# acerbilab/pyvbmc

Measured on AMD Instinct MI355X. Metric: ELBO+entropy evals/sec at D=10, K=50, N=400, Ns=1e6 (1e6-sample-equivalent evals/s), higher is better.
Workload: dtype f64; 1 GPU; BASELINE config 3 per GPU: D=10 K=50 N=400 S=1, Ns=1000000 MC samples per GPU (job Ns=1000000), value+grad _neg_elcbo with soft bounds, eps=philox; parallelism=single GPU

## Files before the change

include/vbmc_hip.h:

```cpp
#ifndef VBMC_HIP_H
#define VBMC_HIP_H

#include <stddef.h>
#include <stdint.h>

#ifdef __cplusplus
extern "C" {
#endif

typedef struct vbmc_ctx vbmc_ctx;

enum {
  VBMC_OK = 0,
  VBMC_E_ARG = -1,
  VBMC_E_HIP = -2,
  VBMC_E_RCCL = -3,
  VBMC_E_NODEV = -4,
  VBMC_E_UNSUP = -5,
  VBMC_E_NONFINITE = -6,
  VBMC_E_NOMEM = -7,
  VBMC_E_NOTPD = -8,
  VBMC_W_GP_CHANGED = 1,
  VBMC_W_NOT_FUSED = 2
};

enum { VBMC_MEAN_ZERO = 0, VBMC_MEAN_CONST = 1, VBMC_MEAN_NEGQUAD = 2 };

enum {
  VBMC_EPS_RESIDENT = 0,
  VBMC_EPS_PHILOX = 1
};


int vbmc_abi_version(void);

int vbmc_device_count(int* n_out);

int vbmc_ctx_create(int device_id, vbmc_ctx** out);
void vbmc_ctx_destroy(vbmc_ctx* ctx);

int vbmc_host_affinity(const vbmc_ctx* ctx, int* bound_out, int* n_cpus_out);

const char* vbmc_last_error(const vbmc_ctx* ctx);

int vbmc_device_info(const vbmc_ctx* ctx, char* name, int name_len, int* cu_count,
                     int* clock_khz, uint64_t* hbm_bytes);

int vbmc_synchronize(vbmc_ctx* ctx);

int vbmc_set_timing(vbmc_ctx* ctx, int on);

int vbmc_last_kernel_ms(vbmc_ctx* ctx, int which, double* ms_out);

int vbmc_last_host_us(const vbmc_ctx* ctx, double out[5]);
int vbmc_last_step_marks(const vbmc_ctx* ctx, double out[4]);
int vbmc_set_release_callback(vbmc_ctx* ctx, void (*fn)(void*), void* user);

int vbmc_set_option(vbmc_ctx* ctx, const char* key, int value);

int vbmc_last_entmc_plan(const vbmc_ctx* ctx, int out[4]);

int vbmc_ws_span_layout(int cus, int pb, int front, int nb, int pad, int K, int64_t* part_lo, int* first_part,
                        int* rows_per_component);

int vbmc_host_checksum(const double* const* ptrs, const int64_t* lens, int n, uint64_t* out);

int vbmc_set_gp_watch(vbmc_ctx* ctx, const double* const* ptrs, const int64_t* lens, int n, uint64_t expected);

int vbmc_armed_stats(const vbmc_ctx* ctx, uint64_t out[6]);

int vbmc_last_elbo_raw(const vbmc_ctx* ctx, double* out, int n);


int vbmc_set_mixture(vbmc_ctx* ctx, int D, int K, const double* mu_KxD,
                     const double* sigma_K, const double* lambd_D, const double* w_K,
                     const double* eta_K);

int vbmc_set_mixture_dk(vbmc_ctx* ctx, int D, int K, const double* mu_DxK,
                        const double* sigma_K, const double* lambd_D, const double* w_K,
                        const double* eta_K);

int vbmc_theta_to_mixture(vbmc_ctx* ctx, const double* theta, int n_theta,
                          int optimize_mask, double* mu_KxD, double* sigma_K,
                          double* lambd_D, double* w_K, double* eta_K);


int vbmc_mixture_pdf(vbmc_ctx* ctx, int64_t n, const double* x_nxD, int log_flag,
                     int grad_flag, double df, double* y_n, double* dy_nxD);


int vbmc_set_eps(vbmc_ctx* ctx, int K, int64_t n_half, int D, const double* eps_half,
                 int64_t row_begin, int64_t row_count);

int vbmc_mt19937_randn(uint32_t* key, int* pos, int* has_gauss, double* gauss, double* out,
                       int64_t n, int n_threads);

int vbmc_mt19937_randn_dev(vbmc_ctx* ctx, uint32_t* key, int* pos, int* has_gauss, double* gauss, double* out,
                           int64_t n);
int vbmc_randn_dev_info(const vbmc_ctx* ctx, int* window_reused);
int vbmc_mt_jump_host(const uint32_t* key_in, uint64_t n_words, uint32_t* key_out);
int vbmc_mt_jump_polys(uint64_t stride_words, int count, uint32_t* out);

int vbmc_set_eps_numpy(vbmc_ctx* ctx, uint32_t* key, int* pos, int* has_gauss, double* gauss, int K,
                       int64_t n_half, int D, int64_t row_begin, int64_t row_count, int n_threads);

int vbmc_entmc(vbmc_ctx* ctx, int64_t ns_per_comp, int eps_mode, uint64_t seed,
               int64_t row_begin, int64_t row_count, int grad_flags, int jacobian_flag,
               double* H, double* dH, double* raw_out);

int vbmc_philox_normals(vbmc_ctx* ctx, int K, int64_t n_half, int D, uint64_t seed, int64_t row_begin,
                        int64_t row_count, double* out);

int vbmc_entmc_finalize(vbmc_ctx* ctx, const double* raw, int grad_flags,
                        int jacobian_flag, double* H, double* dH);

int vbmc_entlb(vbmc_ctx* ctx, int grad_flags, int jacobian_flag, double* H, double* dH);


int vbmc_set_gp(vbmc_ctx* ctx, int N, int D, int S, int P, int mean_kind,
                const double* X_NxD, const double* hyp_SxP, const double* alpha_SxN,
                const double* L_SxNxN, const int32_t* L_chol_S, const double* sW_SxN,
                const double* sn2_mult_S);

int vbmc_gp_posterior(vbmc_ctx* ctx, int N, int D, int S, int P, int mean_kind, const double* X_NxD,
                      const double* y_N, const double* sn2_SxN, const double* sn2_div_S, const double* hyp_SxP,
                      double* alpha_SxN, double* L_SxNxN);

int vbmc_gp_append(vbmc_ctx* ctx, const double* x_D, double y, double* alpha_SxN1, double* L_SxN1xN1);

int vbmc_gp_append_noisy(vbmc_ctx* ctx, const double* x_D, double y, const double* sn2_new_S, double* alpha_SxN1,
                         double* L_SxN1xN1);

int vbmc_gp_fetch(vbmc_ctx* ctx, double* alpha_SxN, double* L_SxNxN);

int vbmc_gp_lml(vbmc_ctx* ctx, int N, int D, int B, int P, int mean_kind, const double* X_NxD, const double* y_N,
                const double* sn2_BxN, const double* sn2_div_B, const double* dsn2_B, const double* hyp_BxP, int want_grad,
                double* lml_B, double* dlml_BxP, int32_t* status_B);

int vbmc_gp_hyp_sample(vbmc_ctx* ctx, int N, int D, int P, int mean_kind, const double* X_NxD, const double* y_N,
                       const double* s2_N, int C, const double* x0_CxP, const double* widths_P, const double* lb_P,
                       const double* ub_P, const double* prior_mu_P, const double* prior_sigma_P, const double* prior_df_P,
                       int n, int thin, int burn_in, uint64_t seed, double* hyp_CxnxP, double* logpost_Cxn,
                       double* logprior_Cxn, int64_t* stats_Cx4, int32_t* invalid_C);

int vbmc_gp_hyp_optimize(vbmc_ctx* ctx, int N, int D, int P, int mean_kind, const double* X_NxD, const double* y_N,
                         const double* s2_N, int R, const double* x0_RxP, const double* lb_P, const double* ub_P,
                         const double* prior_mu_P, const double* prior_sigma_P, const double* prior_df_P, int max_iter, int m,
                         double tol_g, double tol_f, int trace_cap, double* hyp_RxP, double* logpost_R, double* grad_RxP,
                         int64_t* stats_Rx4, int32_t* invalid_R, double* trace_iter, double* trace_eval);

int vbmc_gp_fit(vbmc_ctx* ctx, int N, int D, int P, int mean_kind, const double* X_NxD, const double* y_N,
                const double* s2_N, int H, const double* hyp0_HxP, int init_N, const double* dlb_P, const double* dub_P,
                const double* lb_P, const double* ub_P, const double* prior_mu_P, const double* prior_sigma_P,
                const double* prior_df_P, int opts_N, int max_iter, int m, double tol_g, double tol_f, int n_samples,
                const double* widths_P, int thin, int burn_in, uint64_t seed, double* cand_BxP, double* score_B,
                int32_t* starts_R, double* opt_hyp_RxP, double* opt_logpost_R, int64_t* opt_stats_Rx4,
                int32_t* opt_invalid_R, double* best_P, double* best_logpost, double* hyp_SxP, double* logpost_S,
                double* logprior_S, int64_t* stats_Sx4, double* noise_S, int32_t* status, double* alpha_SxN,
                double* L_SxNxN);


int vbmc_gp_log_joint(vbmc_ctx* ctx, int grad_flags, int avg_flag, int jacobian_flag,
                      int compute_var, double* G, double* dG, double* varG,
                      double* var_ss, double* I_SxK, double* J_SxKxK);


int vbmc_gp_predict(vbmc_ctx* ctx, int64_t M, const double* xs_MxD, int add_noise,
                    int separate_samples, double* fmu, double* fs2);


typedef struct {
  int64_t ns_per_comp;
  int eps_mode;
  uint64_t seed;
  int compute_grad;
  int optimize_mask;
  int64_t row_begin;
  int64_t row_count;
  const double* bnd_lb;
  const double* bnd_ub;
  int n_bnd;
  double tol_con;
  double weight_threshold;
  double weight_penalty;
} vbmc_elbo_opts;

int vbmc_neg_elcbo(vbmc_ctx* ctx, double* theta, int n_theta, const vbmc_elbo_opts* opts,
                   double* F, double* dF, double* G, double* H, double* mu_KxD,
                   double* sigma_K, double* lambd_D, double* w_K, double* eta_K);

typedef struct vbmc_elbo_call {
  double* theta;
  int n_theta;
  const vbmc_elbo_opts* opts;
  double* F;
  double* dF;
  double* G;
  double* H;
  double* mu_KxD;
  double* sigma_K;
  double* lambd_D;
  double* w_K;
  double* eta_K;
} vbmc_elbo_call;
int vbmc_neg_elcbo_call(vbmc_ctx* ctx, const vbmc_elbo_call* c);


int vbmc_neg_elcbo_batch(vbmc_ctx* ctx, const double* thetas_BxN, int B, int n_theta,
                         const vbmc_elbo_opts* opts, double* F_B, double* G_B, double* H_B);


int vbmc_adam_begin(vbmc_ctx* ctx, const double* theta0, int n_theta, const vbmc_elbo_opts* opts,
                    const double* lb, const double* ub, int max_iter, double master_min,
                    double master_max, double master_decay);
int vbmc_adam_run_auto(vbmc_ctx* ctx, int max_iters, double tol_fun, int* n_done, double* y_tab_out,
                       double* x_tab_out, double* G_out, double* H_out);
int vbmc_adam_run(vbmc_ctx* ctx, int n_iters, double* y_tab_out, double* x_tab_out,
                  double* G_out, double* H_out);
int vbmc_adam_end(vbmc_ctx* ctx, double* theta_out, double* mu_KxD, double* sigma_K,
                  double* lambd_D, double* w_K, double* eta_K, int* iterations);


// ... 173 lines not shown
```

pyvbmc_amd/_lib.py:

```python
import ctypes as C
import os
import sys
import threading
from pathlib import Path

import numpy as np

_HERE = Path(__file__).resolve().parent
LIB_PATH = Path(os.environ.get("VBMC_HIP_LIB", _HERE / "libvbmc_hip.so"))

EPS_RESIDENT, EPS_PHILOX = 0, 1
MEAN_ZERO, MEAN_CONST, MEAN_NEGQUAD = 0, 1, 2
E_ARG, E_HIP, E_RCCL, E_NODEV, E_UNSUP, E_NONFINITE = -1, -2, -3, -4, -5, -6
E_NOTPD = -8
W_GP_CHANGED = 1
W_NOT_FUSED = 2
T_ENTMC, T_GLJ, T_PDF, T_PREDICT, T_ELBO, T_PREDICT_VAR, T_GP_POST, T_IS_MCMC, T_GP_LML = range(9)
T_SEARCH_FILL, T_SEARCH_EVAL, T_SEARCH_SORT = 9, 10, 11
T_GP_HYP = 12
T_SEARCH_CMAES = 13
T_GP_OPT = 14
T_SIEVE_FILL, T_SIEVE_SCORE, T_SIEVE_RANK = 15, 16, 17


class VbmcHipError(RuntimeError):
    def __init__(self, code, msg):
        super().__init__(f"libvbmc_hip error {code}: {msg}")
        self.code = code


class NoDeviceError(VbmcHipError):
    pass


class UnsupportedShape(NotImplementedError):
    """VBMC_E_UNSUP: a shape the kernels do not cover (D > 32, a GP too large for the LDS plans ...).  A
    ``NotImplementedError`` -- there is no CPU fallback inside this package -- that ``pyvbmc_amd.patch`` recognises:
    under the drop-in such a call goes back to the reference callable it replaced (pyvbmc_amd/dropin.py)."""


_dp = C.POINTER(C.c_double)
_vp = C.c_void_p


class ElboOpts(C.Structure):
    _fields_ = [
        ("ns_per_comp", C.c_int64),
        ("eps_mode", C.c_int),
        ("seed", C.c_uint64),
        ("compute_grad", C.c_int),
        ("optimize_mask", C.c_int),
        ("row_begin", C.c_int64),
        ("row_count", C.c_int64),
        ("bnd_lb", _dp),
        ("bnd_ub", _dp),
        ("n_bnd", C.c_int),
        ("tol_con", C.c_double),
        ("weight_threshold", C.c_double),
        ("weight_penalty", C.c_double),
    ]


class ElboCall(C.Structure):

    _fields_ = [
        ("theta", _dp),
        ("n_theta", C.c_int),
        ("opts", C.POINTER(ElboOpts)),
        ("F", _dp),
        ("dF", _dp),
        ("G", _dp),
        ("H", _dp),
        ("mu_KxD", _dp),
        ("sigma_K", _dp),
        ("lambd_D", _dp),
        ("w_K", _dp),
        ("eta_K", _dp),
    ]


MTV_HOST, MTV_MIX1, MTV_MIX2 = 0, 1, 2
KDE_SCOTT, KDE_DEGENERATE, KDE_ROOT_STUCK = 1, 4, 8


class MtvSide(C.Structure):

    _fields_ = [
        ("source", C.c_int),
        ("n", C.c_int64),
        ("x_NxD", _dp),
        ("seed", C.c_uint64),
        ("lb_D", _dp),
        ("ub_D", _dp),
    ]


SRC_COPY, SRC_TRANSFORM, SRC_MIXTURE, SRC_AFFINE, SRC_BOX = range(5)
ACQ_IS = 4


class SearchSource(C.Structure):

    _fields_ = [
        ("kind", C.c_int),
        ("rows", C.c_int64),
        ("data", _dp),
        ("df", C.c_double),
        ("seed", C.c_uint64),
    ]


class SieveFillArgs(C.Structure):

    _fields_ = [
        ("D", C.c_int),
        ("K", C.c_int),
        ("K_new", C.c_int),
        ("optimize_mask", C.c_int),
        ("n1", C.c_int64),
        ("n2", C.c_int64),
        ("n3", C.c_int64),
        ("mu0_KxD", _dp),
        ("sigma0_K", _dp),
        ("lambd0_D", _dp),
        ("w0_K", _dp),
        ("mu2_KnxD", _dp),
        ("sigma2_Kn", _dp),
        ("lambd_s_D", _dp),
        ("N_star", C.c_int64),
        ("X_star_NxD", _dp),
        ("v3", C.c_double),
        ("Z_BxS", _dp),
        ("n_slot", C.c_int),
        ("I_BxKn", C.POINTER(C.c_int32)),
        ("seed", C.c_uint64),
    ]


class CmaesOpts(C.Structure):

    _fields_ = [
        ("lam", C.c_int),
        ("max_fevals", C.c_int64),
        ("tol_fun", C.c_double),
        ("tol_x", C.c_double),
        ("seed", C.c_uint64),
    ]


SIGNATURES = {
    "vbmc_abi_version": (C.c_int, []),
    "vbmc_device_count": (C.c_int, [C.POINTER(C.c_int)]),
    "vbmc_ctx_create": (C.c_int, [C.c_int, C.POINTER(_vp)]),
    "vbmc_ctx_destroy": (None, [_vp]),
    "vbmc_last_error": (C.c_char_p, [_vp]),
    "vbmc_device_info": (
        C.c_int,
        [_vp, C.c_char_p, C.c_int, C.POINTER(C.c_int), C.POINTER(C.c_int), C.POINTER(C.c_uint64)],
    ),
    "vbmc_host_affinity": (C.c_int, [_vp, C.POINTER(C.c_int), C.POINTER(C.c_int)]),
    "vbmc_synchronize": (C.c_int, [_vp]),
    "vbmc_set_option": (C.c_int, [_vp, C.c_char_p, C.c_int]),
    "vbmc_last_entmc_plan": (C.c_int, [_vp, C.POINTER(C.c_int)]),
    "vbmc_ws_span_layout": (C.c_int, [C.c_int, C.c_int, C.c_int, C.c_int, C.c_int, C.c_int, C.POINTER(C.c_int64),
                                      C.POINTER(C.c_int), C.POINTER(C.c_int)]),
    "vbmc_last_elbo_raw": (C.c_int, [_vp, _dp, C.c_int]),
    "vbmc_armed_stats": (C.c_int, [_vp, C.POINTER(C.c_uint64)]),
    "vbmc_set_gp_watch": (C.c_int, [_vp, C.POINTER(C.c_void_p), C.POINTER(C.c_int64), C.c_int, C.c_uint64]),
    "vbmc_host_checksum": (C.c_int, [C.POINTER(C.c_void_p), C.POINTER(C.c_int64), C.c_int, C.POINTER(C.c_uint64)]),
    "vbmc_set_timing": (C.c_int, [_vp, C.c_int]),
    "vbmc_last_kernel_ms": (C.c_int, [_vp, C.c_int, _dp]),
    "vbmc_last_host_us": (C.c_int, [_vp, _dp]),
    "vbmc_last_step_marks": (C.c_int, [_vp, _dp]),
    "vbmc_set_release_callback": (C.c_int, [_vp, C.c_void_p, C.c_void_p]),
    "vbmc_set_mixture": (C.c_int, [_vp, C.c_int, C.c_int, _dp, _dp, _dp, _dp, _dp]),
    "vbmc_set_mixture_dk": (C.c_int, [_vp, C.c_int, C.c_int, _dp, _dp, _dp, _dp, _dp]),
    "vbmc_theta_to_mixture": (C.c_int, [_vp, _dp, C.c_int, C.c_int, _dp, _dp, _dp, _dp, _dp]),
    "vbmc_mixture_pdf": (C.c_int, [_vp, C.c_int64, _dp, C.c_int, C.c_int, C.c_double, _dp, _dp]),
    "vbmc_set_eps": (C.c_int, [_vp, C.c_int, C.c_int64, C.c_int, _dp, C.c_int64, C.c_int64]),
    "vbmc_mt19937_randn": (
        C.c_int,
        [C.POINTER(C.c_uint32), C.POINTER(C.c_int), C.POINTER(C.c_int), _dp, _dp, C.c_int64, C.c_int],
    ),
    "vbmc_randn_dev_info": (C.c_int, [_vp, C.POINTER(C.c_int)]),
    "vbmc_mt19937_randn_dev": (
        C.c_int,
        [_vp, C.POINTER(C.c_uint32), C.POINTER(C.c_int), C.POINTER(C.c_int), _dp, _dp, C.c_int64],
    ),
    "vbmc_mt_jump_host": (C.c_int, [C.POINTER(C.c_uint32), C.c_uint64, C.POINTER(C.c_uint32)]),
    "vbmc_mt_jump_polys": (C.c_int, [C.c_uint64, C.c_int, C.POINTER(C.c_uint32)]),
    "vbmc_set_eps_numpy": (
        C.c_int,
        [_vp, C.POINTER(C.c_uint32), C.POINTER(C.c_int), C.POINTER(C.c_int), _dp, C.c_int, C.c_int64, C.c_int,
         C.c_int64, C.c_int64, C.c_int],
    ),
    "vbmc_entmc": (
        C.c_int,
        [_vp, C.c_int64, C.c_int, C.c_uint64, C.c_int64, C.c_int64, C.c_int, C.c_int, _dp, _dp, _dp],
    ),
    "vbmc_philox_normals": (C.c_int, [_vp, C.c_int, C.c_int64, C.c_int, C.c_uint64, C.c_int64, C.c_int64, _dp]),
    "vbmc_entmc_finalize": (C.c_int, [_vp, _dp, C.c_int, C.c_int, _dp, _dp]),
    "vbmc_entlb": (C.c_int, [_vp, C.c_int, C.c_int, _dp, _dp]),
    "vbmc_set_gp": (
        C.c_int,
        [_vp, C.c_int, C.c_int, C.c_int, C.c_int, C.c_int, _dp, _dp, _dp, _dp,
         C.POINTER(C.c_int32), _dp, _dp],
    ),
    "vbmc_gp_posterior": (
        C.c_int,
        [_vp, C.c_int, C.c_int, C.c_int, C.c_int, C.c_int, _dp, _dp, _dp, _dp, _dp, _dp, _dp],
    ),
    "vbmc_gp_append": (C.c_int, [_vp, _dp, C.c_double, _dp, _dp]),
    "vbmc_gp_append_noisy": (C.c_int, [_vp, _dp, C.c_double, _dp, _dp, _dp]),
    "vbmc_gp_fetch": (C.c_int, [_vp, _dp, _dp]),
    "vbmc_gp_lml": (
        C.c_int,
        [_vp, C.c_int, C.c_int, C.c_int, C.c_int, C.c_int, _dp, _dp, _dp, _dp, _dp, _dp, C.c_int, _dp, _dp,
         C.POINTER(C.c_int32)],
    ),
    "vbmc_gp_hyp_sample": (
        C.c_int,
        [_vp, C.c_int, C.c_int, C.c_int, C.c_int, _dp, _dp, _dp, C.c_int, _dp, _dp, _dp, _dp, _dp, _dp, _dp, C.c_int, C.c_int,
         C.c_int, C.c_uint64, _dp, _dp, _dp, C.POINTER(C.c_int64), C.POINTER(C.c_int32)],
    ),
    "vbmc_gp_hyp_optimize": (
        C.c_int,
        [_vp, C.c_int, C.c_int, C.c_int, C.c_int, _dp, _dp, _dp, C.c_int, _dp, _dp, _dp, _dp, _dp, _dp, C.c_int, C.c_int,
         C.c_double, C.c_double, C.c_int, _dp, _dp, _dp, C.POINTER(C.c_int64), C.POINTER(C.c_int32), _dp, _dp],
    ),
    "vbmc_gp_fit": (
        C.c_int,
        [_vp, C.c_int, C.c_int, C.c_int, C.c_int, _dp, _dp, _dp, C.c_int, _dp, C.c_int, _dp, _dp, _dp, _dp, _dp, _dp, _dp,
         C.c_int, C.c_int, C.c_int, C.c_double, C.c_double, C.c_int, _dp, C.c_int, C.c_int, C.c_uint64, _dp, _dp,
         C.POINTER(C.c_int32), _dp, _dp, C.POINTER(C.c_int64), C.POINTER(C.c_int32), _dp, _dp, _dp, _dp, _dp,
         C.POINTER(C.c_int64), _dp, C.POINTER(C.c_int32), _dp, _dp],
    ),
    "vbmc_gp_log_joint": (
        C.c_int,
        [_vp, C.c_int, C.c_int, C.c_int, C.c_int, _dp, _dp, _dp, _dp, _dp, _dp],
    ),
    "vbmc_gp_predict": (C.c_int, [_vp, C.c_int64, _dp, C.c_int, C.c_int, _dp, _dp]),
    "vbmc_neg_elcbo": (
        C.c_int,
        [_vp, _dp, C.c_int, C.POINTER(ElboOpts), _dp, _dp, _dp, _dp, _dp, _dp, _dp, _dp, _dp],
    ),
    "vbmc_neg_elcbo_call": (C.c_int, [_vp, C.POINTER(ElboCall)]),
    "vbmc_neg_elcbo_batch": (
        C.c_int,
        [_vp, _dp, C.c_int, C.c_int, C.POINTER(ElboOpts), _dp, _dp, _dp],
    ),
    "vbmc_adam_begin": (
        C.c_int,
        [_vp, _dp, C.c_int, C.POINTER(ElboOpts), _dp, _dp, C.c_int, C.c_double, C.c_double, C.c_double],
    ),
    "vbmc_adam_run": (C.c_int, [_vp, C.c_int, _dp, _dp, _dp, _dp]),
    "vbmc_adam_run_auto": (C.c_int, [_vp, C.c_int, C.c_double, C.POINTER(C.c_int), _dp, _dp, _dp, _dp]),
    "vbmc_adam_end": (C.c_int, [_vp, _dp, _dp, _dp, _dp, _dp, _dp, C.POINTER(C.c_int)]),
    "vbmc_acq_eval": (
        C.c_int,
        [_vp, C.c_int64, _dp, C.c_int, C.c_double, C.c_double, _dp, _dp, _dp, _dp],
    ),
    "vbmc_acq_is_set": (C.c_int, [_vp, C.c_int64, _dp, C.c_int, _dp, _dp, _dp]),
    "vbmc_acq_is_eval": (C.c_int, [_vp, C.c_int64, _dp, _dp, C.c_double, _dp, _dp]),
    "vbmc_is_proposal": (C.c_int, [_vp, C.c_int64, _dp, C.c_int, _dp, _dp, _dp, _dp, C.c_double, _dp, C.c_int, _dp, _dp,
                                   C.POINTER(C.c_int)]),
    "vbmc_is_box_sample": (C.c_int, [_vp, C.c_int64, C.c_uint64, _dp, _dp]),
    "vbmc_acq_is_build": (C.c_int, [_vp, C.c_int64, _dp, C.c_int, _dp, _dp, _dp, _dp]),
    "vbmc_is_mcmc": (C.c_int, [_vp, C.c_int, C.c_double, _dp, _dp, _dp, _dp, C.c_int, C.c_int, C.c_int, C.c_uint64, _dp, _dp,
                               _dp, _dp, C.POINTER(C.c_int64), C.POINTER(C.c_int)]),
    "vbmc_sq_dist": (C.c_int, [_vp, C.c_int64, C.c_int64, C.c_int, _dp, _dp, _dp, C.POINTER(C.c_int64)]),
    "vbmc_search_fill": (C.c_int, [_vp, C.c_int, C.c_int, C.POINTER(SearchSource), _dp, _dp, C.c_uint32, C.c_int, _dp]),
    "vbmc_search_put": (C.c_int, [_vp, C.c_int64, C.c_int, _dp, C.c_uint32, C.c_int]),
    "vbmc_search_eval": (C.c_int, [_vp, C.c_int, C.c_double, C.c_double, C.c_double, C.c_int64, _dp, _dp, _dp, C.c_int, _dp,
                                   _dp, _dp, C.POINTER(C.c_int64), _dp]),
    "vbmc_search_cmaes": (C.c_int, [_vp, C.c_int, C.c_double, C.c_double, C.c_double, C.c_int64, _dp, _dp, _dp, C.c_int, _dp,
                                    _dp, C.c_int, _dp, _dp, _dp, _dp, C.c_uint32, C.POINTER(CmaesOpts), _dp, _dp, _dp, _dp,
                                    _dp, _dp, C.POINTER(C.c_int64)]),
    "vbmc_sieve_fill": (C.c_int, [_vp, C.POINTER(SieveFillArgs), _dp]),
    "vbmc_sieve_put": (C.c_int, [_vp, C.c_int64, C.c_int, _dp]),
    "vbmc_sieve_eval": (C.c_int, [_vp, C.POINTER(ElboOpts), _dp, _dp, _dp, C.POINTER(C.c_int64), _dp]),
    "vbmc_elcbo_full": (C.c_int, [_vp, _dp, C.c_int, C.c_int, C.c_int64, C.c_int, C.c_uint64, C.c_int, _dp, _dp, _dp]),
    "vbmc_elcbo_prune_trial": (C.c_int, [_vp, C.c_int, C.c_int64, C.c_int, C.c_uint64, _dp]),
    "vbmc_elcbo_prune_accept": (C.c_int, [_vp]),
    "vbmc_elcbo_put": (C.c_int, [_vp, C.c_int, C.c_int, _dp, _dp]),
    "vbmc_elcbo_record_info": (C.c_int, [_vp, C.POINTER(C.c_int64), C.POINTER(C.c_int32)]),
    "vbmc_mixture_sample": (C.c_int, [_vp, C.c_int64, C.c_uint64, C.c_int, _dp, C.POINTER(C.c_int32)]),
    "vbmc_mixture_sample_t": (C.c_int, [_vp, C.c_int64, C.c_uint64, C.c_int, C.c_double, _dp, C.POINTER(C.c_int32)]),
    "vbmc_kl_div_mc": (C.c_int, [_vp, C.c_int64, C.c_uint64, C.c_int, _dp, _dp, _dp, _dp, _dp]),
    "vbmc_set_transformer": (C.c_int, [_vp, C.c_int, C.c_int, _dp, _dp, _dp, _dp, _dp, _dp, _dp]),
    "vbmc_clear_transformer": (C.c_int, [_vp, C.c_int]),
    "vbmc_transform": (C.c_int, [_vp, C.c_int64, C.c_int, _dp, _dp]),
    "vbmc_mixture_sample_orig": (C.c_int, [_vp, C.c_int64, C.c_uint64, C.c_int, C.c_double, _dp, C.POINTER(C.c_int32)]),
    "vbmc_mixture_pdf_orig": (C.c_int, [_vp, C.c_int64, _dp, C.c_int, C.c_int, C.c_double, _dp, _dp]),
    "vbmc_mixture_moments_orig": (C.c_int, [_vp, C.c_int64, C.c_uint64, C.c_int, _dp, _dp]),
    "vbmc_kl_div_mc_orig": (C.c_int, [_vp, C.c_int64, C.c_uint64, C.c_int, _dp, _dp, _dp, _dp, _dp]),
    "vbmc_kde_1d": (C.c_int, [_vp, C.c_int, C.c_int64, _dp, C.c_int, _dp, _dp, _dp, _dp, _dp, C.POINTER(C.c_int64)]),
    "vbmc_mtv": (C.c_int, [_vp, C.c_int, C.POINTER(MtvSide), C.POINTER(MtvSide), C.c_int, _dp, _dp, _dp, _dp, _dp,
                           C.POINTER(C.c_int64)]),
    "vbmc_mixture_mode": (C.c_int, [_vp, C.c_int, C.c_int, C.c_int64, _dp, C.c_uint64, C.c_int, C.c_double, _dp, _dp,
                                    _dp, _dp, _dp]),
    "vbmc_warp_points": (C.c_int, [_vp, C.c_int, C.c_int64, C.c_int, _dp, _dp, _dp, _dp]),
    "vbmc_warp_unscent": (C.c_int, [_vp, C.c_int, C.c_int64, _dp, C.c_int64, _dp, _dp, _dp, _dp]),
    "vbmc_warp_gp": (C.c_int, [_vp, C.c_int, C.c_int, C.c_int, C.c_int, _dp, _dp, _dp, _dp, _dp]),
    "vbmc_warp_box": (C.c_int, [_vp, C.c_int, C.c_int64, C.c_int, _dp, _dp, _dp, C.c_uint64, C.c_int, _dp, _dp]),
    "vbmc_comm_unique_id": (C.c_int, [C.POINTER(C.c_uint8)]),
    "vbmc_comm_init": (C.c_int, [_vp, C.POINTER(C.c_uint8), C.c_int, C.c_int]),
    "vbmc_comm_destroy": (C.c_int, [_vp]),
    "vbmc_comm_info": (C.c_int, [_vp, C.POINTER(C.c_int), C.POINTER(C.c_int)]),
    "vbmc_comm_allreduce_max": (C.c_int, [_vp, _dp]),
    "vbmc_comm_barrier": (C.c_int, [_vp]),
}

_lib = None
_lib_lock = threading.Lock()


def load():
    global _lib
    with _lib_lock:
        if _lib is None:
            if not LIB_PATH.exists():
                raise ImportError(
                    f"{LIB_PATH} not found: build it with `python -m pyvbmc_amd.build` "
                    "(hipcc, gfx950).  pyvbmc_amd has no CPU fallback."
                )
            lib = C.CDLL(str(LIB_PATH), mode=C.RTLD_GLOBAL)
            for name, (res, args) in SIGNATURES.items():
                fn = getattr(lib, name)
                fn.restype = res
                fn.argtypes = args
            _lib = lib
    return _lib


def device_count():
    n = C.c_int(0)
    load().vbmc_device_count(C.byref(n))
    return n.value


def f64(a):
    return np.ascontiguousarray(a, dtype=np.float64)


def ptr(a):
    if a is None:
        return None
    assert a.dtype == np.float64 and a.flags["C_CONTIGUOUS"]
    return a.ctypes.data_as(_dp)


def flags_to_bits(flags):
    if np.isscalar(flags):
        return 15 if flags else 0
    return sum((1 << i) for i, f in enumerate(flags) if f)


class Context:

    def __init__(self, device=None):
        lib = load()
        if device is None:
            device = int(os.environ.get("VBMC_HIP_DEVICE", os.environ.get("LOCAL_RANK", "0")))
        h = _vp()
        rc = lib.vbmc_ctx_create(int(device), C.byref(h))
        if rc != 0:
            msg = (lib.vbmc_last_error(None) or b"").decode()
            raise (NoDeviceError if rc == E_NODEV else VbmcHipError)(rc, msg)
        self._h = h
        self._lib = lib
        self.device = int(device)
        self.rank, self.world = 0, 1

    def close(self):
        if getattr(self, "_h", None):
            self.__dict__.pop("_fused_last", None)
            self.__dict__.pop("_fused_cache", None)
            vo = sys.modules.get(__package__ + ".variational_optimization")
            if vo is not None:
                fs = vo._fast_last[0]
                if fs is not None and fs.ctx is self:
                    vo._fast_last[0] = None
            self._lib.vbmc_ctx_destroy(self._h)
            self._h = None

    def __del__(self):
        try:
            self.close()
        except Exception:
            pass

    def check(self, rc):
        if rc != 0:
            msg = (self._lib.vbmc_last_error(self._h) or b"").decode()
            if rc == E_UNSUP:
                raise UnsupportedShape(msg)
            if rc == E_ARG:
                raise ValueError(msg)
            if rc == E_NODEV:
                raise NoDeviceError(rc, msg)
            if rc == E_NOTPD:
                raise np.linalg.LinAlgError(msg)
            raise VbmcHipError(rc, msg)

    def device_info(self):
        name = C.create_string_buffer(256)
        cu, clk, mem = C.c_int(), C.c_int(), C.c_uint64()
        self.check(self._lib.vbmc_device_info(self._h, name, 256, C.byref(cu), C.byref(clk), C.byref(mem)))
        return {"name": name.value.decode(), "cu_count": cu.value, "clock_khz": clk.value,
                "hbm_bytes": mem.value}

    def host_affinity(self):
        b, n = C.c_int(), C.c_int()
        self.check(self._lib.vbmc_host_affinity(self._h, C.byref(b), C.byref(n)))
        return bool(b.value), n.value

    def synchronize(self):
        self.check(self._lib.vbmc_synchronize(self._h))

    def set_timing(self, on):
        self.check(self._lib.vbmc_set_timing(self._h, int(on) if on else 0))

    def set_option(self, key, value):
        self.check(self._lib.vbmc_set_option(self._h, key.encode(), int(value)))

    def last_entmc_plan(self):
        out = (C.c_int * 4)()
        self.check(self._lib.vbmc_last_entmc_plan(self._h, out))
        return {"kernel": ("valu", "ws", "small", "mfma", "adam_fused", "ws", "ws")[out[0]] if out[0] >= 0 else None, "rg": out[1],
                "chunks": out[2], "resident_draws": bool(out[3] & 1), "roles": bool(out[3] & 2), "span": out[0] in (5, 6), "adam_tail": out[0] == 6}

    def philox_normals(self, K, n_half, D, seed, row_begin=0, row_count=None):
        row_count = n_half - row_begin if row_count is None else row_count
        out = np.empty((K, row_count, D))
        self.check(self._lib.vbmc_philox_normals(self._h, K, n_half, D, C.c_uint64(seed), row_begin, row_count, ptr(out)))
        return out

    def armed_stats(self):
        out = (C.c_uint64 * 6)()
        self.check(self._lib.vbmc_armed_stats(self._h, out))
        return dict(zip(("hits", "cancels", "late", "ident_checked", "ident_bad", "lost"), (int(v) for v in out)))

    def last_elbo_raw(self, D, K):
        out = np.empty(1 + D * K + 2 * K + D)
        self.check(self._lib.vbmc_last_elbo_raw(self._h, ptr(out), out.size))
        return out

    def last_kernel_ms(self, which=T_ENTMC):
        v = C.c_double()
        self.check(self._lib.vbmc_last_kernel_ms(self._h, which, C.byref(v)))
        return v.value

    def last_host_us(self):
        out = np.zeros(5)
        self.check(self._lib.vbmc_last_host_us(self._h, ptr(out)))
        return out

    def last_step_marks(self):
        out = np.zeros(4)
        self.check(self._lib.vbmc_last_step_marks(self._h, ptr(out)))
        return {"gp_word_us": out[0], "entropy_word_us": out[1],
                "gp_sums_in": ("prep launch", "finish launch", "entropy launch")[int(out[2])]}

    def set_mixture(self, mu_DK, sigma, lambd, w, eta):
        mu_DK = np.asarray(mu_DK, dtype=np.float64)
        D, K = mu_DK.shape
        mu_kd = f64(mu_DK.T)
        s, l, ww = f64(np.ravel(sigma)), f64(np.ravel(lambd)), f64(np.ravel(w))
        e = f64(np.ravel(eta)) if eta is not None and np.size(eta) == K else None
        if s.size != K or l.size != D or ww.size != K:
            raise ValueError("mixture attribute shapes do not match (D, K)")
        self.check(self._lib.vbmc_set_mixture(self._h, D, K, ptr(mu_kd), ptr(s), ptr(l), ptr(ww), ptr(e)))
        self.D, self.K = D, K

    def mixture_changed(self, D, K):
        self.__dict__["_vp_args"] = None
        self.D, self.K = int(D), int(K)
        vo = sys.modules.get(__package__ + ".variational_optimization")
        if vo is not None:
            vo.clear_fast_path()

    def set_eps(self, eps_half, row_begin=0, row_count=None):
        eps_half = f64(eps_half)
        K, h, D = eps_half.shape
        if row_count is None:
            row_count = h - row_begin
        self.check(self._lib.vbmc_set_eps(self._h, K, h, D, ptr(eps_half), row_begin, row_count))

    def set_eps_numpy(self, K, n_half, D, row_begin=0, row_count=None, threads=0, view=None):
        if row_count is None:
            row_count = n_half - row_begin
        with NP_STREAM_LOCK:
            left = self.__dict__.get("_np_left")
            fp = view() if view is not None and left is not None else None
            if fp is not None and fp == left and view._words is not None:
                bg, words = view._bg, view._words
                has_gauss, gauss = C.c_int(0), C.c_double(0.0)
                with bg.lock:
                    addr = C.addressof(words)
                    rc = self._lib.vbmc_set_eps_numpy(self._h, C.cast(addr, C.POINTER(C.c_uint32)),
                                                      C.cast(addr + 624 * 4, C.POINTER(C.c_int)), C.byref(has_gauss),
                                                      C.byref(gauss), K, n_half, D, row_begin, row_count,
                                                      threads or host_threads())
                    if has_gauss.value:
                        key = np.array(words[:624], dtype=np.uint32)
                        pos = int(words[624])
                if has_gauss.value:
                    np.random.set_state(("MT19937", key, pos, has_gauss.value, gauss.value))
                    self.__dict__["_np_left"] = None
                else:
                    self.__dict__["_np_left"] = view()
                self.check(rc)
                return True
            st = np.random.get_state(legacy=True)
            if not isinstance(st, tuple) or st[0] != "MT19937":
                return False
            key = np.array(st[1], dtype=np.uint32)
            pos, has_gauss, gauss = C.c_int(int(st[2])), C.c_int(int(st[3])), C.c_double(float(st[4]))
            rc = self._lib.vbmc_set_eps_numpy(self._h, key.ctypes.data_as(C.POINTER(C.c_uint32)), C.byref(pos),
                                              C.byref(has_gauss), C.byref(gauss), K, n_half, D, row_begin, row_count,
                                              threads or host_threads())
            np.random.set_state(("MT19937", key, pos.value, has_gauss.value, gauss.value))
            self.__dict__["_np_left"] = view() if view is not None and has_gauss.value == 0 else None
        self.check(rc)
        return True

    def comm_init(self, uid_bytes, rank, world):
        buf = (C.c_uint8 * 128).from_buffer_copy(uid_bytes)
        self.check(self._lib.vbmc_comm_init(self._h, buf, rank, world))
        self.rank, self.world = rank, world

    def comm_info(self):
        r, w = C.c_int(), C.c_int()
        self.check(self._lib.vbmc_comm_info(self._h, C.byref(r), C.byref(w)))
        return r.value, w.value

    def comm_barrier(self):
        self.check(self._lib.vbmc_comm_barrier(self._h))

    def comm_max(self, value):
        v = C.c_double(value)
        self.check(self._lib.vbmc_comm_allreduce_max(self._h, C.byref(v)))
        return v.value


def comm_unique_id():
    buf = (C.c_uint8 * 128)()
    rc = load().vbmc_comm_unique_id(buf)
    if rc != 0:
        raise VbmcHipError(rc, (load().vbmc_last_error(None) or b"").decode())
    return bytes(buf)


NP_STREAM_LOCK = threading.Lock()


def host_threads():
    try:
        n = len(os.sched_getaffinity(0))
    except (AttributeError, OSError):
        n = os.cpu_count() or 1
    return max(1, min(64, n))


_default_ctx = None


def default_context():
    global _default_ctx
    if _default_ctx is None:
        _default_ctx = Context()
    return _default_ctx


def set_default_context(ctx):
    global _default_ctx
    _default_ctx = ctx
```

pyvbmc_amd/csrc/api_elbo.hip:

```cpp
#include <algorithm>
#include <chrono>
#include <cstdlib>
#include <cmath>
#include <cstring>

#include "common.h"
#include "entropy_args.h"

static double soft_bound_loss(const std::vector<double>& x, const double* lb, const double* ub,
                              double tol_con, std::vector<double>* dy) {
  double y = 0.0;
  if (dy) dy->assign(x.size(), 0.0);
  for (size_t i = 0; i < x.size(); ++i) {
    if (x[i] >= lb[i] && x[i] <= ub[i]) continue;
    const double ell = (ub[i] - lb[i]) * tol_con;
    if (x[i] < lb[i]) {
      const double t = (lb[i] - x[i]) / ell;
      y += 0.5 * t * t;
      if (dy) (*dy)[i] = (x[i] - lb[i]) / (ell * ell);
    }
    if (x[i] > ub[i]) {
      const double t = (x[i] - ub[i]) / ell;
      y += 0.5 * t * t;
      if (dy) (*dy)[i] = (x[i] - ub[i]) / (ell * ell);
// ... 17 lines not shown
  memcpy(out, g_host_stamps, sizeof(g_host_stamps));
  return (int)(g_host_n & 63);
}
extern "C" int vbmc_debug_clock_pair(vbmc_ctx* ctx, int64_t* host_before, int64_t* host_after, unsigned long long* gpu) {
  volatile unsigned long long* f = (volatile unsigned long long*)(ctx->h_done + 6);
  *f = 0;
  (void)hipStreamSynchronize(ctx->stream);
  *host_before = host_ns();
  hipLaunchKernelGGL(clock_stamp_kernel, dim3(1), dim3(64), 0, ctx->stream, (unsigned long long*)(ctx->hd_done + 6));
  while (*f == 0) __builtin_ia32_pause();
  *host_after = host_ns();
  *gpu = *f;
  return 0;
}
#define HSTAMP(i) g_host_stamps[g_host_n & 63][i] = host_ns()
#else
#define HSTAMP(i) (void)0
#endif

static inline uint64_t* ctl_word(vbmc_ctx* ctx, uint64_t seq) { return ctx->d_ctl + (seq & 7); }

void spec_disarm(vbmc_ctx* ctx) {
  vbmc_ctx::ArmedEval& sp = ctx->spec;
  if (!sp.armed) return;
  *(volatile uint64_t*)ctl_word(ctx, sp.seq) = ~(uint64_t)0;
  __builtin_ia32_sfence();
  sp.armed = false;
  ++sp.cancels;
  ctx->gen_cur = sp.gen_cur_before;
  ctx->ahead.valid = sp.ahead_before_valid;
  ctx->ahead.seed = sp.ahead_before_seed;
  ctx->ahead.buf = sp.ahead_before_buf;
  ctx->ahead.frac = sp.ahead_before_frac;
}

extern "C" int vbmc_neg_elcbo(vbmc_ctx* ctx, double* theta, int n_theta,
                              const vbmc_elbo_opts* opts, double* F, double* dF, double* G,
                              double* H, double* mu_KxD, double* sigma_K, double* lambd_D,
                              double* w_K, double* eta_K) {
  if (!ctx || !theta || !opts) return VBMC_E_ARG;
  struct KeepArmed {
    vbmc_ctx* c;
    explicit KeepArmed(vbmc_ctx* c_) : c(c_) { c->spec.keep = true; }
    ~KeepArmed() { c->spec.keep = false; }
  } keep_armed(ctx);
  NEED_DEVICE(ctx);
  if (!ctx->mix_set) return vbmc_fail(ctx, VBMC_E_ARG, "neg_elcbo: mixture (D,K) not set");
  if (!ctx->gp.set) return vbmc_fail(ctx, VBMC_E_ARG, "neg_elcbo: GP not set");
  if (ctx->gp.D != ctx->D) return vbmc_fail(ctx, VBMC_E_ARG, "neg_elcbo: GP/mixture D mismatch");
  using clk = std::chrono::steady_clock;
  const auto t_begin = clk::now();
  HSTAMP(0);
  auto us_since = [](clk::time_point a) {
    return std::chrono::duration<double, std::micro>(clk::now() - a).count();
  };
  const int D = ctx->D, K = ctx->K;
  const int mask = opts->optimize_mask;
  const ThetaMap tm(D, K, mask, n_theta);
  ctx->defer_mix_upload = true;
  int rc = vbmc_theta_to_mixture(ctx, theta, n_theta, mask, mu_KxD, sigma_K, lambd_D, w_K, eta_K);
  ctx->defer_mix_upload = false;
  if (rc) return rc;
  if (tm.o_w()) {
    double* e = theta + (n_theta - K);
    double mx = e[0];
    for (int k = 1; k < K; ++k) mx = e[k] > mx ? e[k] : mx;
    for (int k = 0; k < K; ++k) e[k] -= mx;
  }
  const int grad_flags = opts->compute_grad ? mask : 0;
  const GpState& g = ctx->gp;
  const int S = g.S;
  const int st = 1 + 2 * D;
  const size_t n_res = (size_t)S * K * st;
  const int n_raw = raw_len(D, K);
  const bool mc = opts->ns_per_comp > 0;
  const bool lb_dev = !mc && K > 1;

  int64_t row_begin = opts->row_begin, row_count = opts->row_count;
  if (mc) {
    if (opts->ns_per_comp & 1)
      return vbmc_fail(ctx, VBMC_E_ARG, "neg_elcbo: ns_per_comp must be even");
    rc = resolve_row_slice(ctx, opts, "neg_elcbo", &row_begin, &row_count);
    if (rc) return rc;
  }

  rc = ensure_pinned(ctx, n_res + (size_t)n_raw);
  if (rc) return rc;
  double* hp_dev = ctx->hp_dev;
  double* res_out = hp_dev;
  double* raw_host = hp_dev + n_res;
  const bool multi = ctx_is_multi(ctx);
  double* raw_out = raw_host;
  if (multi && mc) {
    rc = ensure_dev(ctx, &ctx->d_out, &ctx->d_out_cap, (size_t)n_raw);
    if (rc) return rc;
    raw_out = ctx->d_out;
  }

  ctx->host_us[0] = us_since(t_begin);
  const auto t_launch = clk::now();
  const bool can_poll = mc;
  double* stage = nullptr;
  if (can_poll) {
    rc = ensure_dev(ctx, &ctx->d_stage, &ctx->d_stage_cap, n_res + (size_t)n_raw);
    if (rc) return rc;
    stage = ctx->d_stage;
  }
  vbmc_ctx::ArmedEval& sp = ctx->spec;
  constexpr double ARM_MAX_EVAL_US = 1000.0, ARM_LIMIT_MS = 0.3, ARM_DEVICE_WAIT_MS = 0.5;
  const bool arm_allowed = ctx->opt_elbo_arm >= 2 || (ctx->opt_elbo_arm == 1 && vbmc_live_contexts_on(ctx->device) <= 1);
  const bool arm_next = can_poll && !multi && arm_allowed && ctx->opt_mix_bar && !ctx->timing &&
                        opts->eps_mode == VBMC_EPS_PHILOX && ctx->host_us[4] <= ARM_MAX_EVAL_US;
  constexpr double ARM_LATE_SLACK_MS = 0.15;
  const double arm_limit_ms = 1e-3 * ctx->host_us[4] + ARM_LIMIT_MS;
  static_assert(ARM_LIMIT_MS + ARM_LATE_SLACK_MS < ARM_DEVICE_WAIT_MS, "the host's cut-off must come before the device's");

  bool polled = false;
  uint64_t cur_seq = 0;
  bool ident_out_flag = false;
  auto issue = [&](uint64_t seed, bool spin, bool& polled_out, uint64_t& seq_out) -> int {
    int rc2;
    PrepArgs pa;
    glj_fill_prep(ctx, grad_flags != 0, res_out, nullptr, pa);
    EntPlan plan;
    if (mc) {
      rc2 = entmc_plan(ctx, opts->ns_per_comp, opts->eps_mode, seed, row_begin, row_count, grad_flags != 0, plan,
                       pa.n_glj);
      if (rc2) return rc2;
      entmc_fill_prep(ctx, plan, pa);
      rc2 = entmc_pregen(ctx, plan, pa);
      if (rc2) return rc2;
    }
    const bool ahead_ok = can_poll && opts->eps_mode == VBMC_EPS_PHILOX && ctx->opt_elbo_ahead &&
                          plan.a.eps != nullptr && plan.a.eps == ctx->d_epsgen[ctx->gen_cur];
    const bool ws_form = plan.kernel == EntKernel::Ws || plan.kernel == EntKernel::WsSpan || plan.kernel == EntKernel::Mfma;
    if (spin && !(ahead_ok && plan.pregen_hit && ws_form))
      return -1000;
    if (can_poll) {
      pa.done.cnt = ctx->d_done_cnt + 8;
      pa.done.flag = ctx->hd_done + 4;
      pa.done.seq = ++ctx->done_seq;
      pa.done.host_out = res_out;
      pa.done.host_n = (int)n_res;
      pa.res = stage;
    }
    seq_out = ctx->done_seq;
    ident_out_flag = false;
    ctx->gp_where = 0;
    double* fg = nullptr;
    if (can_poll && ctx->opt_mix_bar) fg = spin ? ctx->d_mix_fg : write_pack_to_device(ctx);
    if (spin && !fg) return -1000;
    const bool ident = fg != nullptr && mc;
    if (ident) pa.ident_out = (uint64_t*)(ctx->d_done_cnt + 12);
    if (fg) {
      PrepArgs gp_tail = pa;
      gp_tail.n_table = 0;
      gp_tail.gen = GenSlice();
      gp_tail.mix = ctx->d_mix;
      if (entmc_take_gp(ctx, plan, gp_tail)) {
        pa.n_glj = 0;
        ctx->gp_where = 2;
      }
      if (mc && pa.n_glj > 0 && pa.done.flag != nullptr && ctx->opt_gp_ship && plan.kernel == EntKernel::Mfma) {
        plan.a.ship_src = pa.res;
        plan.a.ship_dst = pa.done.host_out;
        plan.a.ship_n = pa.done.host_n;
        plan.a.ship_flag = pa.done.flag;
        plan.a.ship_seq = pa.done.seq;
        pa.done = DoneSignal();
      }
      pa.mix = fg;
      pa.mix_copy = ctx->d_mix;
      pa.mix_copy_n = ctx->ml.total;
    } else {
      rc2 = upload_packed_mixture(ctx);
      if (rc2) return rc2;
    }
    uint64_t* ctl = nullptr;
    if (spin) {
      ctl = ctl_word(ctx, seq_out);
      *(volatile uint64_t*)ctl = 0;
      __builtin_ia32_sfence();
      pa.go = ctl;
      pa.go_seq = seq_out;
      pa.go_timeout = (uint64_t)(ARM_DEVICE_WAIT_MS * 1e5);
      pa.dead = ctx->hd_done + 5;
      plan.a.cancel = ctl;
    }
    HSTAMP(1);
    rc2 = launch_prep(ctx, pa);
    if (rc2) return rc2;
    polled_out = false;
    if (mc) {
      rc2 = entmc_launch_main(ctx, plan);
      if (rc2) return rc2;
      GenSlice ahead_gen;
      DoneSignal done;
      if (can_poll) {
        if (ahead_ok) ahead_gen = entmc_ahead_slice(ctx, plan);
        done.cnt = ctx->d_done_cnt;
        done.sub = ctx->d_done_sub;
        {
          static const int sub_min = [] { const char* e = getenv("VBMC_FIN_SUB_MIN"); return e ? atoi(e) : 256; }();
          done.sub_min = sub_min;
        }
        done.flag = ctx->hd_done;
        done.seq = seq_out;
        done.host_out = raw_out;
        done.host_n = n_raw;
        done.cancel = ctl;
        if (ident) {
          done.ident_src = (const uint64_t*)(ctx->d_done_cnt + 12);
          done.ident_dst = ctx->hd_done + 1;
          done.ident_seed = seed;
        }
        polled_out = true;
        ident_out_flag = ident;
      }
      const GenSlice* gen_here = ahead_gen.n_blocks > 0 ? &ahead_gen : nullptr;
      if (!multi) {
        rc2 = entmc_launch_finish(ctx, plan, polled_out ? stage + n_res : raw_out, gen_here, polled_out ? &done : nullptr);
        if (rc2) return rc2;
      } else {
        rc2 = entmc_launch_finish(ctx, plan, raw_out, nullptr, nullptr);
        if (rc2) return rc2;
        rc2 = comm_allreduce_sum(ctx, raw_out, n_raw);
        if (rc2) return rc2;
        if (polled_out) {
          done.host_out = raw_host;
          rc2 = entmc_launch_publish(ctx, raw_out, done, gen_here);
          if (rc2) return rc2;
        } else {
          HIP_TRY(ctx, hipMemcpyAsync(ctx->h_pinned + n_res, raw_out, sizeof(double) * n_raw,
                                      hipMemcpyDeviceToHost, ctx->stream));
        }
      }
    } else if (lb_dev) {
      rc2 = launch_entlb(ctx, raw_host);
      if (rc2) return rc2;
    }
    return 0;
  };

  uint64_t want_ck = 0;
  bool check_ident = false;
  bool used_armed = false;
  if (sp.armed) {
    const bool match = can_poll && sp.seed == opts->seed && sp.n_theta == n_theta && sp.mask == mask &&
                       sp.grad_flags == grad_flags && sp.eps_mode == opts->eps_mode &&
                       sp.ns_per_comp == opts->ns_per_comp && sp.row_begin == row_begin && sp.row_count == row_count &&
                       !ctx->timing &&
                       std::chrono::duration<double, std::milli>(clk::now() - sp.t_armed).count() < sp.limit_ms;
    if (match) {
      memcpy(ctx->d_mix_fg, ctx->h_pack, sizeof(double) * (size_t)ctx->ml.total);
      __builtin_ia32_sfence();
      *(volatile uint64_t*)ctl_word(ctx, sp.seq) = sp.seq;
      __builtin_ia32_sfence();
      ctx->pack_valid = true;
      sp.armed = false;
      const bool force_late = ctx->opt_arm_late_test > 0 && --ctx->opt_arm_late_test == 0;
      if (!force_late && std::chrono::duration<double, std::milli>(clk::now() - sp.t_armed).count() < sp.limit_ms + ARM_LATE_SLACK_MS) {
        ++sp.hits;
        used_armed = true;
        polled = true;
        cur_seq = sp.seq;
        check_ident = sp.ident;
        HSTAMP(1);
      } else {
        *(volatile uint64_t*)ctl_word(ctx, sp.seq) = ~(uint64_t)0;
        __builtin_ia32_sfence();
        HIP_TRY(ctx, stream_wait(ctx));
        HIP_TRY(ctx, hipMemsetAsync(ctx->d_done_cnt, 0, sizeof(int) * 16, ctx->stream));
        HIP_TRY(ctx, hipMemsetAsync(ctx->d_done_sub, 0, sizeof(int) * 16 * 64, ctx->stream));
        ctx->gen_cur = sp.gen_cur_before;
        ctx->ahead.valid = sp.ahead_before_valid;
        ctx->ahead.seed = sp.ahead_before_seed;
        ctx->ahead.buf = sp.ahead_before_buf;
        ctx->ahead.frac = sp.ahead_before_frac;
        ++sp.cancels;
        ++sp.late;
      }
    } else {
      spec_disarm(ctx);
    }
  }
  if (!used_armed) {
    rc = issue(opts->seed, false, polled, cur_seq);
    if (rc) return rc;
    check_ident = polled && ident_out_flag;
  }
  if (mc && can_poll && ctx->opt_mix_bar) want_ck = pack_checksum(ctx->h_pack, (size_t)ctx->ml.total);
  ctx->step_marks[2] = (double)ctx->gp_where;
  if (polled && arm_next && ctx->d_ctl && ctx->d_mix_fg) {
    sp.gen_cur_before = ctx->gen_cur;
    sp.ahead_before_valid = ctx->ahead.valid;
    sp.ahead_before_seed = ctx->ahead.seed;
    sp.ahead_before_buf = ctx->ahead.buf;
    sp.ahead_before_frac = ctx->ahead.frac;
    const uint64_t seq_before = ctx->done_seq;
    bool p2 = false;
    uint64_t seq2 = 0;
    const auto t_arm0 = clk::now();
    const int rc2 = issue(opts->seed + 1, true, p2, seq2);
    if (rc2 == 0 && p2) {
      sp.armed = true;
      sp.ident = ident_out_flag;
      sp.limit_ms = arm_limit_ms;
      sp.t_armed = t_arm0;
      sp.seq = seq2;
      sp.seed = opts->seed + 1;
      sp.n_theta = n_theta;
      sp.mask = mask;
      sp.grad_flags = grad_flags;
      sp.eps_mode = opts->eps_mode;
      sp.ns_per_comp = opts->ns_per_comp;
      sp.row_begin = row_begin;
      sp.row_count = row_count;
    } else if (rc2 == -1000) {
      ctx->done_seq = seq_before;
      ctx->gen_cur = sp.gen_cur_before;
      ctx->ahead.valid = sp.ahead_before_valid;
      ctx->ahead.seed = sp.ahead_before_seed;
      ctx->ahead.buf = sp.ahead_before_buf;
      ctx->ahead.frac = sp.ahead_before_frac;
    } else if (rc2 != 0) {
      return rc2;
    }
  }
  if (ctx->release_cb && !ctx->ident_retry) ctx->release_cb(ctx->release_cb_user);
  ElboScratch& sc = ctx->elbo;
  const bool has_bnd = opts->bnd_lb && opts->bnd_ub;
  double F_bnd = 0.0;
  std::vector<double>& dFb = sc.dFb;
  if (has_bnd && grad_flags) dFb.assign((size_t)n_theta, 0.0);
  if (has_bnd) {
    if (tm.n_bnd() != opts->n_bnd)
      return vbmc_fail(ctx, VBMC_E_ARG, "neg_elcbo: bounds length %d != %d", opts->n_bnd, tm.n_bnd());
    std::vector<double>& ext = sc.ext;
    ext.resize((size_t)tm.n_bnd());
    const int sc0 = tm.p_sg;
    for (int i = 0; i < tm.n_bnd(); ++i) ext[i] = tm.bound_coord(i, theta, ctx->sigma.data(), ctx->lambd.data());
    std::vector<double>& dL = sc.dL;
    const double L = soft_bound_loss(ext, opts->bnd_lb, opts->bnd_ub, opts->tol_con,
                                     grad_flags ? &dL : nullptr);
    F_bnd += L;
    if (grad_flags) {
      if (tm.o_mu())
        for (int i = 0; i < D * K; ++i) dFb[i] += dL[i];
      if (tm.o_sg())
        for (int k = 0; k < K; ++k) {
          double a = 0.0;
          for (int d = 0; d < D; ++d) a += dL[sc0 + d * K + k];
          dFb[tm.p_sg + k] += a;
        }
      if (tm.o_lm())
        for (int d = 0; d < D; ++d) {
          double a = 0.0;
          for (int k = 0; k < K; ++k) a += dL[sc0 + d * K + k];
          dFb[tm.p_lm + d] += a;
        }
      if (tm.o_w())
        for (int k = 0; k < K; ++k) dFb[tm.p_w + k] += dL[dL.size() - K + k];
    }
    if (tm.o_w()) {
      const double th = opts->weight_threshold, pen = opts->weight_penalty;
      double a = 0.0;
      std::vector<double>& wg = sc.wpen;
      wg.resize(K);
      for (int k = 0; k < K; ++k) {
        const bool small = ctx->w[k] < th;
        a += small ? ctx->w[k] : th;
        wg[k] = small ? pen : 0.0;
      }
      F_bnd += a * pen;
      if (grad_flags) {
        std::vector<double>& jw = sc.jw;
        jw.resize(K);
        softmax_jacobian_apply(ctx, wg.data(), jw.data());
        for (int k = 0; k < K; ++k) dFb[n_theta - K + k] += jw[k];
      }
    }
  }
  bool gp_changed = false;
  if (!ctx->gp_watch_ptrs.empty()) {
    uint64_t ck = 0;
    vbmc_host_checksum(ctx->gp_watch_ptrs.data(), ctx->gp_watch_lens.data(), (int)ctx->gp_watch_ptrs.size(), &ck);
    gp_changed = ck != ctx->gp_watch_ck;
  }
  ctx->host_us[1] = us_since(t_launch);
  HSTAMP(2);
  const auto t_wait = clk::now();
  auto spin_on = [&](const volatile uint64_t* f, uint64_t want) -> int {
    const volatile uint64_t* dead = ctx->h_done + 5;
    unsigned spins = 0;
    for (;;) {
      if (*f == want) break;
      if (*dead == want) return 1;
      __builtin_ia32_pause();
      if ((++spins & 0xFFFF) == 0 && us_since(t_wait) > 5e6) return 2;
    }
    __atomic_thread_fence(__ATOMIC_ACQUIRE);
    return 0;
  };
  auto redo_unarmed = [&](const char* why) -> int {
    HIP_TRY(ctx, stream_wait(ctx));
    HIP_TRY(ctx, hipMemsetAsync(ctx->d_done_cnt, 0, sizeof(int) * 16, ctx->stream));
        HIP_TRY(ctx, hipMemsetAsync(ctx->d_done_sub, 0, sizeof(int) * 16 * 64, ctx->stream));
    ctx->ahead.valid = false;
    if (ctx->ident_retry) return vbmc_fail(ctx, VBMC_E_HIP, "neg_elcbo: %s, twice in a row", why);
    ctx->ident_retry = true;
    const int arm_was = ctx->opt_elbo_arm;
    ctx->opt_elbo_arm = 0;
    const int rc3 = vbmc_neg_elcbo(ctx, theta, n_theta, opts, F, dF, G, H, mu_KxD, sigma_K, lambd_D, w_K, eta_K);
    ctx->opt_elbo_arm = arm_was;
    ctx->ident_retry = false;
    ctx->spec.keep = true;
    return rc3;
  };
  GljHost& o = sc.glj;
  double Gv = 0.0;
  std::vector<double>&dGv = sc.dG, &dHv = sc.dH;
  auto finalize_gp = [&]() -> int {
    glj_finalize(ctx, ctx->h_pinned, grad_flags != 0, o);
    for (int s = 0; s < S; ++s) Gv += o.G[s];
    Gv /= S;
    dGv.assign((size_t)n_theta, 0.0);
    if (grad_flags) {
      std::vector<double>&mu = sc.mu, &sg = sc.sg, &lm = sc.lm, &wg = sc.wg;
      mu.assign((size_t)K * D, 0.0);
      sg.assign(K, 0.0);
      lm.assign(D, 0.0);
      wg.assign(K, 0.0);
      for (int s = 0; s < S; ++s) {
        for (int i = 0; i < K * D; ++i) mu[i] += o.mu[(size_t)s * K * D + i] / S;
        for (int k = 0; k < K; ++k) sg[k] += o.sigma[(size_t)s * K + k] / S;
        for (int d = 0; d < D; ++d) lm[d] += o.lambd[(size_t)s * D + d] / S;
        for (int k = 0; k < K; ++k) wg[k] += o.w[(size_t)s * K + k] / S;
      }
      const int n = glj_pack(ctx, mu.data(), sg.data(), lm.data(), wg.data(), grad_flags, 1, dGv.data());
      if (n != n_theta) return vbmc_fail(ctx, VBMC_E_ARG, "neg_elcbo: gradient length %d != n_theta %d", n, n_theta);
    }
    return 0;
  };
  bool gp_done = false;
  if (polled) {
    int st_w = spin_on(ctx->h_done + 4, cur_seq);
    HSTAMP(3);
    ctx->step_marks[0] = us_since(t_begin);
    if (st_w == 0) {
      rc = finalize_gp();
      if (rc) return rc;
      gp_done = true;
      st_w = spin_on(ctx->h_done, cur_seq);
    }
    if (st_w != 0) {
      ++sp.lost;
      return redo_unarmed(st_w == 1 ? "the armed launches gave up before the go word reached them"
                                    : "no completion word from the device after 5 s");
    }
    if (check_ident) {
      const volatile uint64_t* id = ctx->h_done + 1;
      ++sp.ident_checked;
      const bool force_bad = ctx->opt_ident_test > 0 && --ctx->opt_ident_test == 0;
      if (force_bad || id[0] != want_ck || id[1] != opts->seed) {
        ++sp.ident_bad;
        return redo_unarmed("the result block does not identify as this evaluation");
      }
    }
  } else {
    HIP_TRY(ctx, stream_wait(ctx));
  }
  ctx->pack_in_flight = false;
  ctx->step_marks[1] = us_since(t_begin);
  if (!polled) ctx->step_marks[0] = ctx->step_marks[1];
  ctx->host_us[2] = us_since(t_wait);
  HSTAMP(4);
  const auto t_fin = clk::now();
  if (!gp_done) {
    rc = finalize_gp();
    if (rc) return rc;
  }
  dHv.assign((size_t)n_theta, 0.0);
  double Hv = 0.0;
  if (mc || lb_dev) {
    const double* r = ctx->h_pinned + n_res;
    entropy_pack(ctx, r[0], r + 1, r + 1 + D * K, r + 1 + D * K + K, r + 1 + D * K + K + D,
                 grad_flags, 1, &Hv, grad_flags ? dHv.data() : nullptr);
  } else {
    rc = vbmc_entlb(ctx, grad_flags, 1, &Hv, grad_flags ? dHv.data() : nullptr);
    if (rc) return rc;
  }
  ctx->last_raw_off = n_res;
  ctx->last_raw_n = mc ? n_raw : 0;
  double Fv = -Gv - Hv;
  std::vector<double>& dFv = sc.dF;
  dFv.assign((size_t)n_theta, 0.0);
  if (grad_flags)
    for (int i = 0; i < n_theta; ++i) dFv[i] = -dGv[i] - dHv[i];

  Fv += F_bnd;
  if (grad_flags && has_bnd)
    for (int i = 0; i < n_theta; ++i) dFv[i] += dFb[i];
  ctx->host_us[3] = us_since(t_fin);
  ctx->host_us[4] = us_since(t_begin);
#ifdef FIN_TIMES
  HSTAMP(5);
  ++g_host_n;
#endif
  if (F) *F = Fv;
  if (G) *G = Gv;
  if (H) *H = Hv;
  if (dF && grad_flags) memcpy(dF, dFv.data(), sizeof(double) * n_theta);
  return gp_changed ? VBMC_W_GP_CHANGED : VBMC_OK;
}

extern "C" int vbmc_neg_elcbo_call(vbmc_ctx* ctx, const vbmc_elbo_call* c) {
  if (!c) return VBMC_E_ARG;
  return vbmc_neg_elcbo(ctx, c->theta, c->n_theta, c->opts, c->F, c->dF, c->G, c->H, c->mu_KxD, c->sigma_K, c->lambd_D, c->w_K,
                        c->eta_K);
}

extern "C" int vbmc_armed_stats(const vbmc_ctx* ctx, uint64_t out[6]) {
  if (!ctx || !out) return VBMC_E_ARG;
  const vbmc_ctx::ArmedEval& sp = ctx->spec;
  out[0] = sp.hits;
  out[1] = sp.cancels;
  out[2] = sp.late;
  out[3] = sp.ident_checked;
  out[4] = sp.ident_bad;
  out[5] = sp.lost;
  return VBMC_OK;
}

extern "C" int vbmc_last_elbo_raw(const vbmc_ctx* ctx, double* out, int n) {
  if (!ctx || !out || ctx->last_raw_n <= 0 || n != ctx->last_raw_n || !ctx->h_pinned) return VBMC_E_ARG;
  memcpy(out, ctx->h_pinned + ctx->last_raw_off, sizeof(double) * (size_t)n);
  return VBMC_OK;
}

extern "C" int vbmc_set_release_callback(vbmc_ctx* ctx, void (*fn)(void*), void* user) {
  if (!ctx) return VBMC_E_ARG;
  ctx->release_cb = fn;
  ctx->release_cb_user = user;
  return VBMC_OK;
}

extern "C" int vbmc_last_step_marks(const vbmc_ctx* ctx, double out[4]) {
  if (!ctx || !out) return VBMC_E_ARG;
  for (int i = 0; i < 4; ++i) out[i] = ctx->step_marks[i];
  return VBMC_OK;
}

extern "C" int vbmc_last_host_us(const vbmc_ctx* ctx, double out[5]) {
  if (!ctx || !out) return VBMC_E_ARG;
  for (int i = 0; i < 5; ++i) out[i] = ctx->host_us[i];
  return VBMC_OK;
}
```

pyvbmc_amd/csrc/common.h:

```cpp
#pragma once
#include <hip/hip_runtime.h>
#include <chrono>

#include <cstdint>
#include <cstdio>
#include <string>
#include <vector>

#include "../../include/vbmc_hip.h"
#include "gp_cand_host.h"
#include "gp_fit_host.h"
#include "scratch.h"
#include "transform.h"

struct ncclComm;

struct MixLayout {
  int D = 0, K = 0;
  int o_mup = 0;
  int o_mu = 0;
  int o_is2 = 0;
  int o_wc = 0;
  int o_rc = 0;
  int o_lrc = 0;
  int o_sig = 0;
  int o_w = 0;
  int o_lam = 0;
  int o_ilam = 0;
  int total = 0;
  void plan(int D_, int K_) {
    D = D_;
    K = K_;
    int o = 0;
    o_mup = o; o += K * D;
    o_mu = o; o += K * D;
    o_is2 = o; o += K;
    o_wc = o; o += K;
    o_rc = o; o += K;
    o_lrc = o; o += K;
    o_sig = o; o += K;
    o_w = o; o += K;
    o_lam = o; o += D;
    o_ilam = o; o += D;
    total = o;
  }
};

struct ThetaMap {
  int D, K;
  int mask;
  __host__ __device__ bool o_mu() const { return mask & 1; }
  __host__ __device__ bool o_sg() const { return mask & 2; }
  __host__ __device__ bool o_lm() const { return mask & 4; }
  __host__ __device__ bool o_w() const { return mask & 8; }
  int p_sg, p_lm, p_w;
  int n_sc;
  __host__ __device__ ThetaMap(int D_, int K_, int mask_) : ThetaMap(D_, K_, mask_, 0) { p_w = n_theta() - K; }
  __host__ __device__ ThetaMap(int D_, int K_, int mask_, int n_theta_)
      : D(D_), K(K_), mask(mask_), p_sg((mask_ & 1) ? D_ * K_ : 0), p_lm(p_sg + ((mask_ & 2) ? K_ : 0)), p_w(n_theta_ - K_),
        n_sc((mask_ & 6) ? D_ * K_ : 0) {}
  __host__ __device__ int n_theta() const { return p_lm + (o_lm() ? D : 0) + (o_w() ? K : 0); }
  __host__ __device__ int n_bnd() const { return p_sg + n_sc + (o_w() ? K : 0); }
  __host__ __device__ bool in_mu(int i) const { return o_mu() && i < D * K; }
  __host__ __device__ bool in_sg(int i) const { return o_sg() && i >= p_sg && i < p_sg + K; }
  __host__ __device__ bool in_lm(int i) const { return o_lm() && i >= p_lm && i < p_lm + D; }
  __host__ __device__ int raw_w() const { return 1 + D * K + K + D; }
  __host__ __device__ int raw_index(int i) const {
    if (o_w() && i >= p_w) return raw_w() + (i - p_w);
    if (o_lm() && i >= p_lm) return 1 + D * K + K + (i - p_lm);
    if (o_sg() && i >= p_sg) return 1 + D * K + (i - p_sg);
    return 1 + i;
  }
  __host__ __device__ double bound_coord(int i, const double* theta, const double* sigma, const double* lambda) const {
    double x;
    if (i < p_sg) {
      x = theta[i];
    } else if (i < p_sg + n_sc) {
      const int q = i - p_sg, k = q / D, d = q - k * D;
      const double ls = o_sg() ? theta[p_sg + k] : log(sigma[k]);
      const double ll = o_lm() ? theta[p_lm + d] : log(lambda[d]);
      x = ll + ls;
    } else {
      x = theta[p_w + (i - p_sg - n_sc)];
    }
    return x;
  }
};

struct GpState {
  bool set = false;
  int N = 0, D = 0, S = 0, P = 0, mean_kind = 0;
  std::vector<double> hyp;
  std::vector<int32_t> L_chol;
  std::vector<double> sn2_eff;
  std::vector<double> sn2_mult;
  double* d_X = nullptr;
  double* d_XT = nullptr;
  double* d_alpha = nullptr;
  double* d_L = nullptr;
  double* d_Linv = nullptr;
  double* d_LinvP = nullptr;
  double* d_sW = nullptr;
  double* d_hyp = nullptr;
  double* d_xc = nullptr;
  double* d_smeta = nullptr;
  size_t cap_X = 0, cap_XT = 0, cap_alpha = 0, cap_L = 0, cap_Linv = 0, cap_LinvP = 0, cap_sW = 0, cap_hyp = 0, cap_xc = 0, cap_smeta = 0;
  std::vector<double> h_small;
  std::vector<double> h_XT;
  bool dev_built = false;
  bool homo = false;
  double* d_y = nullptr;
  double* d_r = nullptr;
  double* d_sn2 = nullptr;
  double* d_sl = nullptr;
  size_t cap_y = 0, cap_r = 0, cap_sn2 = 0, cap_sl = 0;
  std::vector<double> h_X, h_y, h_sl;
  std::vector<double> h_sn2;
};

struct GljHost {
  std::vector<double> G;
  std::vector<double> I_sk;
  std::vector<double> mu;
  std::vector<double> sigma;
  std::vector<double> lambd;
  std::vector<double> w;
};

struct ElboScratch {
  GljHost glj;
  std::vector<double> dG, dH, dF, dFb, mu, sg, lm, wg, ext, dL, wpen, jw;
};

enum TimingPair { T_ENTMC = 0, T_GLJ, T_PDF, T_PREDICT, T_ELBO, T_PREDICT_VAR, T_GP_POST, T_IS_MCMC, T_GP_LML, T_SEARCH_FILL,
                  T_SEARCH_EVAL, T_SEARCH_SORT, T_GP_HYP, T_SEARCH_CMAES, T_GP_OPT, T_SIEVE_FILL, T_SIEVE_SCORE, T_SIEVE_RANK, T_COUNT };

struct vbmc_ctx {
  int device = 0;
  hipStream_t stream = nullptr;
  hipEvent_t ev[2 * T_COUNT] = {};
  bool ev_valid[T_COUNT] = {};
  std::string err;
  hipDeviceProp_t prop;

  bool mix_set = false;
  int D = 0, K = 0;
  std::vector<double> mu, sigma, lambd, w, eta;
  MixLayout ml;
  double* d_mix = nullptr;
  struct ArmedEval {
    bool armed = false;
    bool keep = false;
    uint64_t seq = 0;
    uint64_t seed = 0;
    int n_theta = 0, mask = 0, grad_flags = 0, eps_mode = 0;
    int64_t ns_per_comp = 0, row_begin = 0, row_count = 0;
    int gen_cur_before = 0;
    bool ahead_before_valid = false;
    uint64_t ahead_before_seed = 0;
    int ahead_before_buf = 0;
    double ahead_before_frac = 1.0;
    uint64_t hits = 0, cancels = 0, late = 0, ident_checked = 0, ident_bad = 0, lost = 0;
    bool ident = false;
    double limit_ms = 1.0;
    std::chrono::steady_clock::time_point t_armed;
  } spec;
  uint64_t* d_ctl = nullptr;
  double* d_stage = nullptr;
  size_t d_stage_cap = 0;
  double* d_mix_fg = nullptr;
  std::vector<double> mu_scratch;
  std::vector<double> t2m_mu, t2m_sg, t2m_lm, t2m_w, t2m_eta;
  double* d_acq_fg = nullptr;
  bool acq_fg_failed = false;
  uint64_t acq_seq = 0;
  size_t d_mix_fg_cap = 0;
  bool mix_fg_failed = false;
  size_t d_mix_cap = 0;

  double* d_epsgen[2] = {nullptr, nullptr};
  size_t d_epsgen_cap[2] = {0, 0};
  int gen_cur = 0;
  struct AheadDraws {
    bool valid = false;
    uint64_t seed = 0;
    int K = 0, D = 0, buf = 0;
    int64_t rows = 0, n_half = 0, row_begin = 0;
    double frac = 1.0;
  } ahead;
  uint64_t* h_done = nullptr;
  uint64_t* hd_done = nullptr;
  int* d_done_cnt = nullptr;
  int* d_done_sub = nullptr;
  uint64_t done_seq = 0;

  double* d_eps = nullptr;
  size_t d_eps_cap = 0;
  int eps_K = 0, eps_D = 0;
  int64_t eps_rows = 0, eps_row_begin = 0, eps_n_half = 0;

  double* d_scratch = nullptr;
  size_t d_scratch_cap = 0;
  double* d_out = nullptr;
  size_t d_out_cap = 0;
  double* d_ptick = nullptr;
  size_t d_ptick_cap = 0;
  double* h_pinned = nullptr;
  double* h_eps = nullptr;
  size_t h_eps_cap = 0;
  size_t h_pinned_cap = 0;
  double* h_pack = nullptr;
  size_t h_pack_cap = 0;
  bool pack_in_flight = false;
  bool pack_valid = false;
  bool defer_mix_upload = false;
  double* hp_dev = nullptr;
  int timing = 0;
  double host_us[5] = {0, 0, 0, 0, 0};
  double step_marks[4] = {0, 0, 0, 0};
  int gp_where = 0;
  int opt_entmc_valu = 0;
  int opt_gp_ship = 1;
  int opt_entmc_mfma = 1;
  int opt_elbo_pregen = 1;
  int opt_elbo_ahead = 1;
  int opt_predict_dma = 1;
  int opt_predict_fused = 1;
  int opt_arm_late_test = 0;
  int opt_acq_poll = 1;
  int opt_is_mcmc_threads = 512;
  int opt_gp_lml_chunk = 0;
  int opt_gp_hyp_rounds = 4;
  int opt_gp_opt_rounds = 4;
  int opt_cmaes_rounds = 8;
  void (*release_cb)(void*) = nullptr;
  void* release_cb_user = nullptr;
  int opt_adam_fused = 1;
  int opt_adam_tail = 1;
  int opt_ident_test = 0;
  bool ident_retry = false;
  int opt_elbo_arm = 1;
  bool counted = false;
  int opt_ws_span = 1;
  int opt_ws_front = 0;
  int opt_ws_pad = -1;
  int opt_ws_roles = 1;
  int opt_mix_bar = 1;
  double* h_pack_dev = nullptr;
  double* h_pack_dev_of = nullptr;
  std::vector<double> exp_eta;
  double exp_eta_sum = 0.0;
  bool exp_eta_valid = false;
  int last_plan[4] = {-1, 0, 0, 0};
  size_t last_raw_off = 0;
  int last_raw_n = 0;

  GpState gp;
  GpState gp_next;
  double* d_post_ws = nullptr;
  size_t d_post_ws_cap = 0;

  ncclComm* comm = nullptr;
  int rank = 0, world = 1;

  std::vector<const double*> gp_watch_ptrs;
  std::vector<int64_t> gp_watch_lens;
  uint64_t gp_watch_ck = 0;

  ElboScratch elbo;
  void* adam = nullptr;
  void* acq_is = nullptr;
  bool host_bound = false;
  int host_cpus = 0;
  void* randn_dev = nullptr;
  int randn_last_reused = 0;
  int opt_randn_dev = 1;
  void* xf = nullptr;
  void* search = nullptr;
  void* sieve = nullptr;
  void* elcbo = nullptr;
  uint64_t stream_waits = 0;
  uint64_t gp_launches = 0;
};
inline int ctx_cus(const vbmc_ctx* ctx) { return ctx->prop.multiProcessorCount > 0 ? ctx->prop.multiProcessorCount : 256; }
int vbmc_live_contexts_on(int device);
void adam_free(vbmc_ctx* ctx);
void acq_is_free(vbmc_ctx* ctx);
void randn_dev_free(vbmc_ctx* ctx);
void xf_free(vbmc_ctx* ctx);
void search_free(vbmc_ctx* ctx);
void sieve_free(vbmc_ctx* ctx);
void elcbo_free(vbmc_ctx* ctx);
int randn_device(vbmc_ctx* ctx, uint32_t* key, int* pos, int* has_gauss, double* gauss, double* d_out, int64_t n);

int vbmc_fail(vbmc_ctx* ctx, int code, const char* fmt, ...);
extern thread_local std::string g_create_err;

#define HIP_TRY(ctx, call)                                                            \
  do {                                                                                \
    hipError_t e_ = (call);                                                           \
    if (e_ != hipSuccess)                                                             \
      return vbmc_fail((ctx), VBMC_E_HIP, "%s failed: %s (%s:%d)", #call,             \
                       hipGetErrorString(e_), __FILE__, __LINE__);                    \
  } while (0)

#define VBMC_DISPATCH_DP(D, CALL)   \
  do {                              \
    if ((D) <= 2) CALL(2);          \
    else if ((D) <= 4) CALL(4);     \
    else if ((D) <= 6) CALL(6);     \
    else if ((D) <= 8) CALL(8);     \
    else if ((D) <= 10) CALL(10);   \
    else if ((D) <= 12) CALL(12);   \
    else if ((D) <= 16) CALL(16);   \
    else if ((D) <= 20) CALL(20);   \
    else if ((D) <= 24) CALL(24);   \
    else CALL(32);                  \
  } while (0)

void spec_disarm(vbmc_ctx* ctx);
#define NEED_DEVICE(ctx)                                                                     \
  do {                                                                                       \
    if ((ctx)->device < 0)                                                                   \
      return vbmc_fail((ctx), VBMC_E_NODEV,                                                  \
                       "host-only context: this entry point needs a gfx950 device "          \
                       "(libvbmc_hip has no CPU fallback)");                                 \
    if ((ctx)->spec.armed && !(ctx)->spec.keep) spec_disarm(ctx);                            \
  } while (0)

void write_mixture_pack(const MixLayout& ml, const double* mu_KxD, const double* sigma,
                        const double* lambd, const double* w, double* p);
int make_mixture2(vbmc_ctx* ctx, const char* who, int err, int D, int K2, const double* mu2_KxD, const double* sigma2_K,
                  const double* lambd2_D, const double* w2_K, MixLayout& ml2, std::vector<double>& pack2);
int theta_to_arrays(int D, int K, const double* theta, int n_theta, int optimize_mask, double* mu,
                    double* sg, double* lm, double* w, double* eta);
void ctx_pack_aux(const vbmc_ctx* ctx, double* dst);
void ctx_unpack_aux(vbmc_ctx* ctx, const double* src);
int resolve_row_slice(vbmc_ctx* ctx, const vbmc_elbo_opts* opts, const char* who, int64_t* row_begin, int64_t* row_count);
int upload_packed_mixture(vbmc_ctx* ctx);
double* write_pack_to_device(vbmc_ctx* ctx);
int set_mixture_host(vbmc_ctx* ctx, int D, int K, const double* mu_KxD, const double* sigma_K,
                     const double* lambd_D, const double* w_K, const double* eta_K, bool skip_if_same);

int ensure_dev(vbmc_ctx* ctx, double** p, size_t* cap, size_t n_doubles);
int ensure_pinned(vbmc_ctx* ctx, size_t n_doubles);
int reserve_in(vbmc_ctx* ctx, double** p, size_t* cap, Scratch& sc);
int reserve(vbmc_ctx* ctx, Scratch& sc);
int download_chunked(vbmc_ctx* ctx, const double* d_src, double* dst, size_t n);
int fetch_vectors(vbmc_ctx* ctx, int k, const double* const* d_src, double* const* dst, size_t count, size_t stride, size_t o);
int randn_with_progress(uint32_t* key, int* pos, int* has_gauss, double* gauss, double* out, int64_t n, int n_threads,
                        void (*progress)(void*, int64_t), void* user);

static inline int raw_len(int D, int K) { return 1 + D * K + 2 * K + D; }

struct DoneSignal {
  int* cnt = nullptr;
  int* sub = nullptr;
  int sub_min = 256;
  uint64_t* flag = nullptr;
  uint64_t seq = 0;
  double* host_out = nullptr;
  int host_n = 0;
  const uint64_t* cancel = nullptr;
  const uint64_t* ident_src = nullptr;
  uint64_t* ident_dst = nullptr;
  uint64_t ident_seed = 0;
  int dev = 0;
};

__host__ __device__ inline uint64_t pack_ck_term(double v, uint32_t i) {
  uint64_t b;
  __builtin_memcpy(&b, &v, 8);
  return b * (0x9E3779B97F4A7C15ull + 2ull * i);
}
inline uint64_t pack_checksum(const double* p, size_t n) {
  uint64_t s0 = 0, s1 = 0, s2 = 0, s3 = 0;
  size_t i = 0;
  for (; i + 4 <= n; i += 4) {
    s0 += pack_ck_term(p[i], (uint32_t)i);
    s1 += pack_ck_term(p[i + 1], (uint32_t)i + 1);
    s2 += pack_ck_term(p[i + 2], (uint32_t)i + 2);
    s3 += pack_ck_term(p[i + 3], (uint32_t)i + 3);
  }
  for (; i < n; ++i) s0 += pack_ck_term(p[i], (uint32_t)i);
  return (s0 + s1) + (s2 + s3);
}

#ifdef __HIPCC__
__device__ __forceinline__ void staged_copy_to_host(const double* __restrict__ src, double* __restrict__ dst, int n) {
  for (int base = 0; base < n; base += 256 * 8) {
    double v[8];
#pragma unroll
    for (int u = 0; u < 8; ++u) {
// ... 354 lines not shown
```

pyvbmc_amd/csrc/ctx.hip:

```cpp
#include <algorithm>
#include <cmath>
#include <cstdarg>
#include <cstdlib>
#include <cstring>

#include <sched.h>

#include <cctype>
#include <cstdio>

#include "common.h"

thread_local std::string g_create_err;

int vbmc_fail(vbmc_ctx* ctx, int code, const char* fmt, ...) {
  char buf[1024];
  va_list ap;
  va_start(ap, fmt);
  vsnprintf(buf, sizeof buf, fmt, ap);
  va_end(ap);
  if (ctx)
    ctx->err = buf;
  else
    g_create_err = buf;
  return code;
}

int ensure_dev(vbmc_ctx* ctx, double** p, size_t* cap, size_t n) {
  if (*cap >= n && *p) return 0;
  if (*p) {
    HIP_TRY(ctx, stream_wait(ctx));
    HIP_TRY(ctx, hipFree(*p));
    *p = nullptr;
    *cap = 0;
  }
  size_t want = n + n / 4 + 64;
  HIP_TRY(ctx, hipMalloc((void**)p, want * sizeof(double)));
  *cap = want;
  return 0;
}

int ensure_pinned(vbmc_ctx* ctx, size_t n) {
  if (ctx->h_pinned_cap >= n && ctx->h_pinned) return 0;
  if (ctx->h_pinned) {
    HIP_TRY(ctx, stream_wait(ctx));
    HIP_TRY(ctx, hipHostFree(ctx->h_pinned));
    ctx->h_pinned = nullptr;
    ctx->h_pinned_cap = 0;
  }
  size_t want = n + n / 4 + 64;
  HIP_TRY(ctx, hipHostMalloc((void**)&ctx->h_pinned, want * sizeof(double), hipHostMallocDefault));
  ctx->h_pinned_cap = want;
  HIP_TRY(ctx, hipHostGetDevicePointer((void**)&ctx->hp_dev, ctx->h_pinned, 0));
  return 0;
}

int reserve_in(vbmc_ctx* ctx, double** p, size_t* cap, Scratch& sc) {
  const int rc = ensure_dev(ctx, p, cap, sc.total);
  if (rc) return rc;
  sc.base = *p;
  return 0;
}
int reserve(vbmc_ctx* ctx, Scratch& sc) { return reserve_in(ctx, &ctx->d_scratch, &ctx->d_scratch_cap, sc); }

int download_chunked(vbmc_ctx* ctx, const double* d_src, double* dst, size_t n) {
  const size_t chunk = (size_t)1 << 20;
  int rc = ensure_pinned(ctx, n < chunk ? n : chunk);
  if (rc) return rc;
  for (size_t o = 0; o < n; o += chunk) {
    const size_t m = (n - o) < chunk ? (n - o) : chunk;
    HIP_TRY(ctx, hipMemcpyAsync(ctx->h_pinned, d_src + o, sizeof(double) * m, hipMemcpyDeviceToHost, ctx->stream));
    HIP_TRY(ctx, stream_wait(ctx));
    memcpy(dst + o, ctx->h_pinned, sizeof(double) * m);
  }
  return 0;
}

int fetch_vectors(vbmc_ctx* ctx, int k, const double* const* d_src, double* const* dst, size_t count, size_t stride, size_t o) {
  for (int i = 0; i < k; ++i)
    if (!dst || dst[i])
      HIP_TRY(ctx, hipMemcpyAsync(ctx->h_pinned + i * stride, d_src[i], sizeof(double) * count, hipMemcpyDeviceToHost, ctx->stream));
  HIP_TRY(ctx, stream_wait(ctx));
  for (int i = 0; dst && i < k; ++i)
    if (dst[i]) memcpy(dst[i] + o, ctx->h_pinned + i * stride, sizeof(double) * count);
  return 0;
}

#include <atomic>
static std::atomic<int> g_live_ctx[64];
int vbmc_live_contexts_on(int device) { return device >= 0 && device < 64 ? g_live_ctx[device].load() : 2; }

static void options_from_env(vbmc_ctx* c) {
  const char* e = getenv("VBMC_ENTMC_KERNEL");
  c->opt_entmc_valu = (e && e[0] == 'v') ? 1 : 0;
  e = getenv("VBMC_ELBO_PREGEN");
  c->opt_elbo_pregen = !(e && e[0] == '0');
  e = getenv("VBMC_ELBO_AHEAD");
  c->opt_elbo_ahead = !(e && e[0] == '0');
  e = getenv("VBMC_ELBO_ARM");
  c->opt_elbo_arm = e ? atoi(e) : 1;
  e = getenv("VBMC_ACQ_POLL");
  c->opt_acq_poll = !(e && e[0] == '0');
  e = getenv("VBMC_ADAM_FUSED");
  c->opt_adam_fused = e ? atoi(e) : 1;
  e = getenv("VBMC_RANDN_DEVICE");
  c->opt_randn_dev = e ? (e[0] == '0' ? 0 : e[0] == '2' ? 2 : 1) : 1;
  e = getenv("VBMC_ADAM_TAIL");
  c->opt_adam_tail = e ? atoi(e) : 1;
  e = getenv("VBMC_WS_SPAN");
  c->opt_ws_span = !(e && e[0] == '0');
  e = getenv("VBMC_WS_FRONT");
  if (e) c->opt_ws_front = atoi(e);
  e = getenv("VBMC_WS_PAD");
  if (e) c->opt_ws_pad = atoi(e);
  e = getenv("VBMC_WS_ROLES");
  c->opt_ws_roles = !(e && e[0] == '0');
  e = getenv("VBMC_MIX_BAR");
  c->opt_mix_bar = !(e && e[0] == '0');
  e = getenv("VBMC_PREDICT_DMA");
  c->opt_predict_dma = !(e && e[0] == '0');
  e = getenv("VBMC_PREDICT_FUSED_FINISH");
  if (e) c->opt_predict_fused = atoi(e);
  e = getenv("VBMC_GP_SHIP");
  c->opt_gp_ship = !(e && e[0] == '0');
}

extern "C" {

int vbmc_abi_version(void) { return 2; }

int vbmc_device_count(int* n_out) {
  int n = 0;
  hipError_t e = hipGetDeviceCount(&n);
  if (e != hipSuccess) {
    n = 0;
    (void)hipGetLastError();
  }
  if (n_out) *n_out = n;
  return VBMC_OK;
}

}

static void bind_host_thread(vbmc_ctx* ctx) {
  const char* e = getenv("VBMC_HOST_AFFINITY");
  if (e && e[0] == '0') return;
  char bus[64] = {0};
  if (hipDeviceGetPCIBusId(bus, (int)sizeof(bus) - 1, ctx->device) != hipSuccess) {
    (void)hipGetLastError();
    return;
  }
  for (char* c = bus; *c; ++c) *c = (char)tolower((unsigned char)*c);
  char path[160];
  snprintf(path, sizeof(path), "/sys/bus/pci/devices/%s/local_cpulist", bus);
  FILE* f = fopen(path, "r");
  if (!f) return;
  char list[1024] = {0};
  const bool got = fgets(list, sizeof(list), f) != nullptr;
  fclose(f);
  if (!got) return;
  cpu_set_t local, cur, both;
  CPU_ZERO(&local);
  for (char* p = list; *p;) {
    char* end = nullptr;
    const long a = strtol(p, &end, 10);
    if (end == p) break;
    long b = a;
    p = end;
    if (*p == '-') {
      b = strtol(p + 1, &end, 10);
      if (end == p + 1) break;
      p = end;
    }
    for (long c = a; c <= b && c < CPU_SETSIZE; ++c)
      if (c >= 0) CPU_SET((int)c, &local);
    while (*p == ',' || *p == ' ' || *p == '\n') ++p;
  }
  if (CPU_COUNT(&local) == 0 || sched_getaffinity(0, sizeof(cur), &cur) != 0) return;
  CPU_AND(&both, &cur, &local);
  const int n_both = CPU_COUNT(&both), n_cur = CPU_COUNT(&cur);
  ctx->host_cpus = n_cur;
  if (n_both == 0 || n_both == n_cur) return;
  if (sched_setaffinity(0, sizeof(both), &both) == 0) {
    ctx->host_bound = true;
    ctx->host_cpus = n_both;
  }
}

extern "C" {

int vbmc_host_affinity(const vbmc_ctx* ctx, int* bound_out, int* n_cpus_out) {
  if (!ctx) return VBMC_E_ARG;
  if (bound_out) *bound_out = ctx->host_bound ? 1 : 0;
  if (n_cpus_out) *n_cpus_out = ctx->host_cpus;
  return VBMC_OK;
}

int vbmc_ctx_create(int device_id, vbmc_ctx** out) {
  if (!out) return vbmc_fail(nullptr, VBMC_E_ARG, "vbmc_ctx_create: out is NULL");
  *out = nullptr;
  if (device_id == -1) {
    vbmc_ctx* h = new vbmc_ctx();
    h->device = -1;
    options_from_env(h);
    *out = h;
    return VBMC_OK;
  }
  int n = 0;
  hipError_t e = hipGetDeviceCount(&n);
  if (e != hipSuccess || n <= 0) {
    (void)hipGetLastError();
    return vbmc_fail(nullptr, VBMC_E_NODEV,
                     "no HIP device visible (%s); libvbmc_hip has no CPU fallback",
                     e == hipSuccess ? "device count 0" : hipGetErrorString(e));
  }
  if (device_id < 0 || device_id >= n)
    return vbmc_fail(nullptr, VBMC_E_ARG, "device_id %d out of range [0,%d)", device_id, n);
  vbmc_ctx* ctx = new vbmc_ctx();
  ctx->device = device_id;
  options_from_env(ctx);
  e = hipSetDevice(device_id);
  if (e == hipSuccess) e = hipGetDeviceProperties(&ctx->prop, device_id);
  if (e == hipSuccess) bind_host_thread(ctx);
  if (e == hipSuccess) e = hipStreamCreateWithFlags(&ctx->stream, hipStreamNonBlocking);
  for (int i = 0; i < 2 * T_COUNT && e == hipSuccess; ++i) e = hipEventCreate(&ctx->ev[i]);
  if (e == hipSuccess) e = hipHostMalloc((void**)&ctx->h_done, 64, hipHostMallocDefault);
  if (e == hipSuccess) {
    for (int i = 0; i < 8; ++i) ctx->h_done[i] = 0;
    e = hipHostGetDevicePointer((void**)&ctx->hd_done, ctx->h_done, 0);
  }
  if (e == hipSuccess) e = hipMalloc((void**)&ctx->d_done_cnt, 64);
  if (e == hipSuccess) e = hipMemset(ctx->d_done_cnt, 0, 64);
  if (e == hipSuccess) e = hipMalloc((void**)&ctx->d_done_sub, 16 * 64 * sizeof(int));
  if (e == hipSuccess) e = hipMemset(ctx->d_done_sub, 0, 16 * 64 * sizeof(int));
  if (e != hipSuccess) {
    int rc = vbmc_fail(nullptr, VBMC_E_HIP, "context setup failed: %s", hipGetErrorString(e));
    delete ctx;
    return rc;
  }
  if (strncmp(ctx->prop.gcnArchName, "gfx950", 6) != 0) {
    int rc = vbmc_fail(nullptr, VBMC_E_NODEV, "device %d is %s; this library is built for gfx950 only",
                       device_id, ctx->prop.gcnArchName);
    vbmc_ctx_destroy(ctx);
    return rc;
  }
  if (device_id < 64) g_live_ctx[device_id].fetch_add(1);
  ctx->counted = true;
  *out = ctx;
  return VBMC_OK;
}

void vbmc_ctx_destroy(vbmc_ctx* ctx) {
  if (!ctx) return;
  if (ctx->device < 0) {
    delete ctx;
    return;
  }
  if (ctx->counted && ctx->device < 64) g_live_ctx[ctx->device].fetch_sub(1);
  (void)hipSetDevice(ctx->device);
  spec_disarm(ctx);
  if (getenv("VBMC_DEBUG_ARM")) fprintf(stderr, "[vbmc] armed evaluations: %llu used, %llu cancelled\n", (unsigned long long)ctx->spec.hits, (unsigned long long)ctx->spec.cancels);
  if (ctx->stream) (void)hipStreamSynchronize(ctx->stream);
  if (ctx->d_ctl) (void)hipFree(ctx->d_ctl);
  vbmc_comm_destroy(ctx);
  adam_free(ctx);
  acq_is_free(ctx);
  randn_dev_free(ctx);
  xf_free(ctx);
  search_free(ctx);
  sieve_free(ctx);
  elcbo_free(ctx);
  gp_post_free(ctx);
  double* bufs[] = {ctx->d_mix, ctx->d_mix_fg, ctx->d_acq_fg, ctx->d_stage, ctx->d_eps, ctx->d_scratch, ctx->d_out, ctx->d_ptick, ctx->gp.d_X, ctx->gp.d_XT,
                    ctx->gp.d_alpha, ctx->gp.d_L, ctx->gp.d_Linv, ctx->gp.d_LinvP, ctx->gp.d_sW, ctx->gp.d_hyp,
                    ctx->gp.d_xc, ctx->gp.d_smeta};
  for (double* b : bufs)
    if (b) (void)hipFree(b);
  for (double* b : ctx->d_epsgen)
    if (b) (void)hipFree(b);
  if (ctx->h_done) (void)hipHostFree(ctx->h_done);
  if (ctx->d_done_cnt) (void)hipFree(ctx->d_done_cnt);
  if (ctx->d_done_sub) (void)hipFree(ctx->d_done_sub);
  if (ctx->h_pinned) (void)hipHostFree(ctx->h_pinned);
  if (ctx->h_eps) (void)hipHostFree(ctx->h_eps);
  if (ctx->h_pack) (void)hipHostFree(ctx->h_pack);

  for (hipEvent_t e : ctx->ev)
    if (e) (void)hipEventDestroy(e);
  if (ctx->stream) (void)hipStreamDestroy(ctx->stream);
  delete ctx;
}

const char* vbmc_last_error(const vbmc_ctx* ctx) {
  return ctx ? ctx->err.c_str() : g_create_err.c_str();
}

int vbmc_device_info(const vbmc_ctx* ctx, char* name, int name_len, int* cu_count,
                     int* clock_khz, uint64_t* hbm_bytes) {
  if (!ctx) return VBMC_E_ARG;
  if (ctx->device < 0) return vbmc_fail(const_cast<vbmc_ctx*>(ctx), VBMC_E_NODEV, "host-only context");
  if (name && name_len > 0) {
    snprintf(name, (size_t)name_len, "%s (%s)", ctx->prop.name, ctx->prop.gcnArchName);
  }
  if (cu_count) *cu_count = ctx->prop.multiProcessorCount;
  if (clock_khz) *clock_khz = ctx->prop.clockRate;
  if (hbm_bytes) *hbm_bytes = (uint64_t)ctx->prop.totalGlobalMem;
  return VBMC_OK;
}

int vbmc_synchronize(vbmc_ctx* ctx) {
  if (!ctx) return VBMC_E_ARG;
  if (ctx->device < 0) return VBMC_OK;
  HIP_TRY(ctx, hipSetDevice(ctx->device));
  HIP_TRY(ctx, stream_wait(ctx));
  return VBMC_OK;
}

int vbmc_set_option(vbmc_ctx* ctx, const char* key, int value) {
  if (!ctx || !key) return VBMC_E_ARG;
  if (!strcmp(key, "arm_late_test")) {
    ctx->opt_arm_late_test = value;
    return VBMC_OK;
  }
  if (!strcmp(key, "ident_test")) {
    ctx->opt_ident_test = value;
    return VBMC_OK;
  }
  spec_disarm(ctx);
  if (!strcmp(key, "entmc_kernel")) ctx->opt_entmc_valu = value == 1;
  else if (!strcmp(key, "entmc_mfma")) ctx->opt_entmc_mfma = value != 0;
  else if (!strcmp(key, "gp_ship")) ctx->opt_gp_ship = value != 0;
  else if (!strcmp(key, "elbo_pregen")) ctx->opt_elbo_pregen = value != 0;
  else if (!strcmp(key, "elbo_ahead")) ctx->opt_elbo_ahead = value != 0;
  else if (!strcmp(key, "predict_dma")) ctx->opt_predict_dma = value != 0;
  else if (!strcmp(key, "predict_fused")) ctx->opt_predict_fused = value < 0 ? 0 : value > 2 ? 2 : value;
  else if (!strcmp(key, "mix_bar")) ctx->opt_mix_bar = value != 0;
  else if (!strcmp(key, "ws_span")) ctx->opt_ws_span = value != 0;
  else if (!strcmp(key, "ws_roles")) ctx->opt_ws_roles = value != 0;
  else if (!strcmp(key, "ws_pad")) ctx->opt_ws_pad = value > 8 ? 8 : value;
  else if (!strcmp(key, "ws_front")) ctx->opt_ws_front = value < 0 ? 0 : value > 990 ? 990 : value;
  else if (!strcmp(key, "elbo_arm")) ctx->opt_elbo_arm = value < 0 ? 0 : value > 2 ? 2 : value;
  else if (!strcmp(key, "acq_poll")) ctx->opt_acq_poll = value != 0;
  else if (!strcmp(key, "is_mcmc_threads")) ctx->opt_is_mcmc_threads = value <= 256 ? 256 : value >= 768 ? 768 : 512;
  else if (!strcmp(key, "gp_lml_chunk")) ctx->opt_gp_lml_chunk = value < 0 ? 0 : value;
  else if (!strcmp(key, "gp_hyp_rounds")) ctx->opt_gp_hyp_rounds = value < 1 ? 4 : value > 4096 ? 4096 : value;
  else if (!strcmp(key, "gp_opt_rounds")) ctx->opt_gp_opt_rounds = value < 1 ? 4 : value > 4096 ? 4096 : value;
  else if (!strcmp(key, "cmaes_rounds")) ctx->opt_cmaes_rounds = value < 1 ? 8 : value > 4096 ? 4096 : value;
  else if (!strcmp(key, "randn_device")) ctx->opt_randn_dev = value < 0 ? 0 : value > 3 ? 3 : value;
  else if (!strcmp(key, "adam_tail")) ctx->opt_adam_tail = value;
  else if (!strcmp(key, "adam_fused")) ctx->opt_adam_fused = value;
  else return vbmc_fail(ctx, VBMC_E_ARG, "vbmc_set_option: unknown key '%s'", key);
  return VBMC_OK;
}

int vbmc_set_gp_watch(vbmc_ctx* ctx, const double* const* ptrs, const int64_t* lens, int n, uint64_t expected) {
  if (!ctx || n < 0 || (n > 0 && (!ptrs || !lens))) return VBMC_E_ARG;
  ctx->gp_watch_ptrs.assign(ptrs, ptrs + n);
  ctx->gp_watch_lens.assign(lens, lens + n);
  ctx->gp_watch_ck = expected;
  return VBMC_OK;
}

int vbmc_host_checksum(const double* const* ptrs, const int64_t* lens, int n, uint64_t* out) {
  if (!ptrs || !lens || n < 0 || !out) return VBMC_E_ARG;
  uint64_t s = 0;
  for (int a = 0; a < n; ++a) {
    if (!ptrs[a] || lens[a] < 0) return VBMC_E_ARG;
    s += (pack_checksum(ptrs[a], (size_t)lens[a]) + (uint64_t)lens[a]) * (0xD1B54A32D192ED03ull + 2ull * (uint64_t)a);
  }
  *out = s;
  return VBMC_OK;
}

int vbmc_last_entmc_plan(const vbmc_ctx* ctx, int out[4]) {
  if (!ctx || !out) return VBMC_E_ARG;
  for (int i = 0; i < 4; ++i) out[i] = ctx->last_plan[i];
  return VBMC_OK;
}

int vbmc_set_timing(vbmc_ctx* ctx, int on) {
  if (!ctx) return VBMC_E_ARG;
  ctx->timing = on < 0 ? 0 : on > 2 ? 2 : on;
  return VBMC_OK;
}

int vbmc_last_kernel_ms(vbmc_ctx* ctx, int which, double* ms_out) {
  if (!ctx || which < 0 || which >= T_COUNT || !ms_out) return VBMC_E_ARG;
  NEED_DEVICE(ctx);
  if (!ctx->ev_valid[which])
    return vbmc_fail(ctx, VBMC_E_ARG, which == T_PREDICT_VAR ? "no timed launch recorded for 5 (gp_predict's product alone is timed at vbmc_set_timing(ctx, 2) only)"
                                                 : "no timed launch recorded for %d", which);
  HIP_TRY(ctx, hipEventSynchronize(ctx->ev[2 * which + 1]));
  float ms = 0.f;
  HIP_TRY(ctx, hipEventElapsedTime(&ms, ctx->ev[2 * which], ctx->ev[2 * which + 1]));
  *ms_out = (double)ms;
  return VBMC_OK;
}

}

void write_mixture_pack(const MixLayout& ml, const double* mu_KxD, const double* sigma,
                        const double* lambd, const double* w, double* p) {
  const int D = ml.D, K = ml.K;
  double prod_lam = 1.0;
  for (int d = 0; d < D; ++d) prod_lam *= lambd[d];
  const double nconst = 1.0 / std::pow(2.0 * M_PI, 0.5 * D) / prod_lam;
  const double l2n = std::log2(nconst);
  for (int k = 0; k < K; ++k) {
    for (int d = 0; d < D; ++d) {
      p[ml.o_mu + k * D + d] = mu_KxD[(size_t)k * D + d];
      p[ml.o_mup + k * D + d] = mu_KxD[(size_t)k * D + d] / lambd[d];
    }
    const double s = sigma[k];
    double sD = 1.0, b = s;
    for (int e = D; e > 0; e >>= 1) {
      if (e & 1) sD *= b;
      b *= b;
    }
    p[ml.o_is2 + k] = 1.0 / (s * s);
    p[ml.o_rc + k] = nconst / sD;
    p[ml.o_lrc + k] = l2n - D * std::log2(s);
    p[ml.o_wc + k] = w[k] * nconst / sD;
    p[ml.o_sig + k] = s;
    p[ml.o_w + k] = w[k];
  }
  for (int d = 0; d < D; ++d) {
    p[ml.o_lam + d] = lambd[d];
    p[ml.o_ilam + d] = 1.0 / lambd[d];
  }
}

int make_mixture2(vbmc_ctx* ctx, const char* who, int err, int D, int K2, const double* mu2_KxD, const double* sigma2_K,
                  const double* lambd2_D, const double* w2_K, MixLayout& ml2, std::vector<double>& pack2) {
  for (int k = 0; k < K2; ++k)
    if (!(sigma2_K[k] > 0.0) || !std::isfinite(sigma2_K[k]))
      return vbmc_fail(ctx, err, "%s: sigma2[%d] must be finite and > 0", who, k);
  ml2.plan(D, K2);
  pack2.resize((size_t)ml2.total);
  write_mixture_pack(ml2, mu2_KxD, sigma2_K, lambd2_D, w2_K, pack2.data());
  return 0;
}

int theta_to_arrays(int D, int K, const double* theta, int n_theta, int optimize_mask, double* mu,
                    double* sg, double* lm, double* w, double* eta) {
  const ThetaMap tm(D, K, optimize_mask);
  if (n_theta != tm.n_theta()) return -1;
  for (int i = 0; i < n_theta; ++i)
    if (!std::isfinite(theta[i])) return -2;
  if (tm.o_mu())
    for (int i = 0; i < D * K; ++i) mu[i] = theta[i];
  if (tm.o_sg())
    for (int k = 0; k < K; ++k) sg[k] = std::exp(theta[tm.p_sg + k]);
  if (tm.o_lm())
    for (int d = 0; d < D; ++d) lm[d] = std::exp(theta[tm.p_lm + d]);
  if (tm.o_w()) {
    const double* e = theta + tm.p_w;
    double mx = e[0];
    for (int k = 1; k < K; ++k) mx = e[k] > mx ? e[k] : mx;
    for (int k = 0; k < K; ++k) {
      eta[k] = e[k] - mx;
      w[k] = std::exp(eta[k]);
    }
  }
  double s2 = 0.0;
  for (int d = 0; d < D; ++d) s2 += lm[d] * lm[d];
  const double nl = std::sqrt(s2 / D);
  for (int d = 0; d < D; ++d) lm[d] /= nl;
  for (int k = 0; k < K; ++k) sg[k] *= nl;
  if (tm.o_w()) {
    double ws = 0.0;
    for (int k = 0; k < K; ++k) ws += w[k];
    for (int k = 0; k < K; ++k) w[k] /= ws;
  }
  return 0;
}

void ctx_pack_aux(const vbmc_ctx* ctx, double* dst) {
  for (const std::vector<double>* v : {&ctx->mu, &ctx->sigma, &ctx->lambd, &ctx->w, &ctx->eta}) dst = std::copy(v->begin(), v->end(), dst);
}

void ctx_unpack_aux(vbmc_ctx* ctx, const double* src) {
  for (std::vector<double>* v : {&ctx->mu, &ctx->sigma, &ctx->lambd, &ctx->w, &ctx->eta}) {
    std::copy(src, src + v->size(), v->begin());
    src += v->size();
  }
}

int resolve_row_slice(vbmc_ctx* ctx, const vbmc_elbo_opts* opts, const char* who, int64_t* row_begin, int64_t* row_count) {
  const int64_t n_half = opts->ns_per_comp / 2;
  *row_begin = opts->row_begin;
  *row_count = opts->row_count;
  if (*row_count < 0) {
    *row_begin = n_half * ctx->rank / ctx->world;
    *row_count = n_half * (ctx->rank + 1) / ctx->world - *row_begin;
  }
  if (*row_begin < 0 || *row_begin + *row_count > n_half) return vbmc_fail(ctx, VBMC_E_ARG, "%s: bad row slice", who);
  if (opts->eps_mode == VBMC_EPS_RESIDENT &&
      (!ctx->d_eps || ctx->eps_K != ctx->K || ctx->eps_D != ctx->D || ctx->eps_n_half != n_half ||
       ctx->eps_row_begin != *row_begin || ctx->eps_rows != *row_count))
    return vbmc_fail(ctx, VBMC_E_ARG, "%s: resident eps does not match the request", who);
  return 0;
}

static int pack_mixture(vbmc_ctx* ctx) {
  const int D = ctx->D, K = ctx->K;
  ctx->ml.plan(D, K);
  const MixLayout& ml = ctx->ml;
  if (ctx->device < 0) return 0;
  if (ctx->h_pack_cap < (size_t)ml.total) {
    if (ctx->h_pack) {
      HIP_TRY(ctx, stream_wait(ctx));
      HIP_TRY(ctx, hipHostFree(ctx->h_pack));
      ctx->h_pack = nullptr;
    }
    const size_t want = (size_t)ml.total * 2 + 64;
    HIP_TRY(ctx, hipHostMalloc((void**)&ctx->h_pack, want * sizeof(double), hipHostMallocDefault));
    ctx->h_pack_cap = want;
  }
  if (ctx->pack_in_flight) {
    HIP_TRY(ctx, stream_wait(ctx));
    ctx->pack_in_flight = false;
  }
  write_mixture_pack(ml, ctx->mu.data(), ctx->sigma.data(), ctx->lambd.data(), ctx->w.data(), ctx->h_pack);
  return ensure_dev(ctx, &ctx->d_mix, &ctx->d_mix_cap, (size_t)ml.total);
}

namespace {
__global__ void mix_upload_kernel(const double* __restrict__ src, double* __restrict__ dst, int n) {
  const int i = blockIdx.x * blockDim.x + threadIdx.x;
  if (i < n) dst[i] = src[i];
}
}

double* write_pack_to_device(vbmc_ctx* ctx) {
  if (ctx->device < 0 || ctx->mix_fg_failed) return nullptr;
  const size_t n = (size_t)ctx->ml.total;
  if (ctx->d_mix_fg_cap < n) {
    if (ctx->d_mix_fg) {
      (void)hipStreamSynchronize(ctx->stream);
      (void)hipFree(ctx->d_mix_fg);
      ctx->d_mix_fg = nullptr;
    }
    const size_t want = n * 2 + 64;
    int large_bar = 0;
    if (hipDeviceGetAttribute(&large_bar, hipDeviceAttributeIsLargeBar, ctx->device) != hipSuccess || !large_bar) {
      (void)hipGetLastError();
      ctx->mix_fg_failed = true;
      return nullptr;
    }
    if (hipExtMallocWithFlags((void**)&ctx->d_mix_fg, want * sizeof(double), hipDeviceMallocFinegrained) != hipSuccess) {
      (void)hipGetLastError();
      ctx->d_mix_fg = nullptr;
      ctx->d_mix_fg_cap = 0;
      ctx->mix_fg_failed = true;
      return nullptr;
    }
    ctx->d_mix_fg_cap = want;
  }
  if (!ctx->d_ctl) {
    if (hipExtMallocWithFlags((void**)&ctx->d_ctl, 64, hipDeviceMallocFinegrained) != hipSuccess) {
      (void)hipGetLastError();
      ctx->d_ctl = nullptr;
    } else {
      memset(ctx->d_ctl, 0, 64);
      __builtin_ia32_sfence();
    }
  }
  memcpy(ctx->d_mix_fg, ctx->h_pack, n * sizeof(double));
  __builtin_ia32_sfence();
  ctx->pack_valid = true;
  return ctx->d_mix_fg;
}

int upload_packed_mixture(vbmc_ctx* ctx) {
  if (ctx->device < 0) return 0;
  if (ctx->spec.armed) spec_disarm(ctx);
  {
    double* src = nullptr;
    if (ctx->h_pack_dev_of != ctx->h_pack) {
      HIP_TRY(ctx, hipHostGetDevicePointer((void**)&ctx->h_pack_dev, ctx->h_pack, 0));
      ctx->h_pack_dev_of = ctx->h_pack;
    }
    src = ctx->h_pack_dev;
    const int n = ctx->ml.total;
    hipLaunchKernelGGL(mix_upload_kernel, dim3((n + 255) / 256), dim3(256), 0, ctx->stream, (const double*)src,
                       ctx->d_mix, n);
    HIP_TRY(ctx, hipGetLastError());
  }
  ctx->pack_in_flight = true;
  ctx->pack_valid = true;
  return 0;
}

int set_mixture_host(vbmc_ctx* ctx, int D, int K, const double* mu_KxD, const double* sigma_K,
                     const double* lambd_D, const double* w_K, const double* eta_K, bool skip_if_same) {
  if (D < 1 || K < 1) return vbmc_fail(ctx, VBMC_E_ARG, "set_mixture: bad D=%d K=%d", D, K);
  if (skip_if_same && ctx->mix_set && ctx->pack_valid && ctx->D == D && ctx->K == K &&
      memcmp(ctx->mu.data(), mu_KxD, sizeof(double) * K * D) == 0 &&
      memcmp(ctx->sigma.data(), sigma_K, sizeof(double) * K) == 0 &&
      memcmp(ctx->lambd.data(), lambd_D, sizeof(double) * D) == 0 &&
      memcmp(ctx->w.data(), w_K, sizeof(double) * K) == 0) {
    if (eta_K) ctx->eta.assign(eta_K, eta_K + K);
    ctx->exp_eta_valid = false;
    return 0;
  }
  ctx->pack_valid = false;
  ctx->D = D;
  ctx->K = K;
  ctx->mu.assign(mu_KxD, mu_KxD + (size_t)K * D);
  ctx->sigma.assign(sigma_K, sigma_K + K);
  ctx->lambd.assign(lambd_D, lambd_D + D);
  ctx->w.assign(w_K, w_K + K);
  if (eta_K)
    ctx->eta.assign(eta_K, eta_K + K);
  else
    ctx->eta.assign((size_t)K, 0.0);
  ctx->exp_eta_valid = false;
  for (int k = 0; k < K; ++k)
    if (!(ctx->sigma[k] > 0.0) || !std::isfinite(ctx->sigma[k]))
      return vbmc_fail(ctx, VBMC_E_NONFINITE, "set_mixture: sigma[%d]=%g must be finite and > 0", k,
                       ctx->sigma[k]);
  for (int d = 0; d < D; ++d)
    if (!(ctx->lambd[d] > 0.0) || !std::isfinite(ctx->lambd[d]))
      return vbmc_fail(ctx, VBMC_E_NONFINITE, "set_mixture: lambd[%d]=%g must be finite and > 0", d,
                       ctx->lambd[d]);
  ctx->mix_set = true;
  int rc = pack_mixture(ctx);
  if (rc || ctx->defer_mix_upload) return rc;
  return upload_packed_mixture(ctx);
}

extern "C" {

int vbmc_set_mixture(vbmc_ctx* ctx, int D, int K, const double* mu_KxD, const double* sigma_K,
                     const double* lambd_D, const double* w_K, const double* eta_K) {
  if (!ctx || !mu_KxD || !sigma_K || !lambd_D || !w_K) return VBMC_E_ARG;
  if (ctx->device >= 0) HIP_TRY(ctx, hipSetDevice(ctx->device));
  return set_mixture_host(ctx, D, K, mu_KxD, sigma_K, lambd_D, w_K, eta_K, true);
}

int vbmc_set_mixture_dk(vbmc_ctx* ctx, int D, int K, const double* mu_DxK, const double* sigma_K,
                        const double* lambd_D, const double* w_K, const double* eta_K) {
  if (!ctx || !mu_DxK || !sigma_K || !lambd_D || !w_K || D < 1 || K < 1) return VBMC_E_ARG;
  if (ctx->device >= 0) HIP_TRY(ctx, hipSetDevice(ctx->device));
  std::vector<double>& t = ctx->mu_scratch;
  t.resize((size_t)D * K);
  for (int d = 0; d < D; ++d)
    for (int k = 0; k < K; ++k) t[(size_t)k * D + d] = mu_DxK[(size_t)d * K + k];
  return set_mixture_host(ctx, D, K, t.data(), sigma_K, lambd_D, w_K, eta_K, true);
}

int vbmc_theta_to_mixture(vbmc_ctx* ctx, const double* theta, int n_theta, int optimize_mask,
                          double* mu_KxD, double* sigma_K, double* lambd_D, double* w_K,
                          double* eta_K) {
  if (!ctx || !theta) return VBMC_E_ARG;
  if (!ctx->mix_set) return vbmc_fail(ctx, VBMC_E_ARG, "theta_to_mixture: mixture (D,K) not set");
  if (ctx->device >= 0) HIP_TRY(ctx, hipSetDevice(ctx->device));
  const int D = ctx->D, K = ctx->K;
  std::vector<double>&mu = ctx->t2m_mu, &sg = ctx->t2m_sg, &lm = ctx->t2m_lm, &w = ctx->t2m_w, &eta = ctx->t2m_eta;
  mu = ctx->mu;
  sg = ctx->sigma;
  lm = ctx->lambd;
  w = ctx->w;
  eta = ctx->eta;
  const int st = theta_to_arrays(D, K, theta, n_theta, optimize_mask, mu.data(), sg.data(), lm.data(),
                                 w.data(), eta.data());
  if (st == -1)
    return vbmc_fail(ctx, VBMC_E_ARG, "theta length %d does not match D=%d K=%d mask=%d", n_theta, D, K,
                     optimize_mask);
  if (st == -2) return vbmc_fail(ctx, VBMC_E_NONFINITE, "theta has a non-finite entry");
  int rc = set_mixture_host(ctx, D, K, mu.data(), sg.data(), lm.data(), w.data(), eta.data(), false);
  if (rc) return rc;
  if (mu_KxD) memcpy(mu_KxD, mu.data(), sizeof(double) * D * K);
  if (sigma_K) memcpy(sigma_K, sg.data(), sizeof(double) * K);
  if (lambd_D) memcpy(lambd_D, lm.data(), sizeof(double) * D);
  if (w_K) memcpy(w_K, w.data(), sizeof(double) * K);
  if (eta_K) memcpy(eta_K, eta.data(), sizeof(double) * K);
  return VBMC_OK;
}

static int upload_eps(vbmc_ctx* ctx, int K, int64_t n_half, int D, const double* eps_half, int64_t row_begin,
                      int64_t row_count) {
  HIP_TRY(ctx, hipSetDevice(ctx->device));
  size_t n = (size_t)K * (size_t)row_count * (size_t)D;
  int rc = ensure_dev(ctx, &ctx->d_eps, &ctx->d_eps_cap, n ? n : 1);
  if (rc) return rc;
  if (row_begin == 0 && row_count == n_half && n > 0) {
    HIP_TRY(ctx, hipMemcpyAsync(ctx->d_eps, eps_half, sizeof(double) * n, hipMemcpyHostToDevice, ctx->stream));
  } else {
    for (int j = 0; j < K && row_count > 0; ++j) {
      const double* src = eps_half + ((size_t)j * (size_t)n_half + (size_t)row_begin) * D;
      double* dst = ctx->d_eps + (size_t)j * (size_t)row_count * D;
      HIP_TRY(ctx, hipMemcpyAsync(dst, src, sizeof(double) * (size_t)row_count * D,
                                  hipMemcpyHostToDevice, ctx->stream));
    }
  }
  HIP_TRY(ctx, stream_wait(ctx));
  ctx->eps_K = K;
  ctx->eps_D = D;
  ctx->eps_rows = row_count;
  ctx->eps_row_begin = row_begin;
  ctx->eps_n_half = n_half;
  return VBMC_OK;
}

int vbmc_set_eps(vbmc_ctx* ctx, int K, int64_t n_half, int D, const double* eps_half,
                 int64_t row_begin, int64_t row_count) {
  if (!ctx || !eps_half || K < 1 || D < 1 || n_half < 0) return VBMC_E_ARG;
  if (row_begin < 0 || row_count < 0 || row_begin + row_count > n_half)
    return vbmc_fail(ctx, VBMC_E_ARG, "set_eps: rows [%lld,+%lld) outside [0,%lld)",
                     (long long)row_begin, (long long)row_count, (long long)n_half);
  NEED_DEVICE(ctx);
  return upload_eps(ctx, K, n_half, D, eps_half, row_begin, row_count);
}

int vbmc_set_eps_numpy(vbmc_ctx* ctx, uint32_t* key, int* pos, int* has_gauss, double* gauss, int K,
                       int64_t n_half, int D, int64_t row_begin, int64_t row_count, int n_threads) {
  if (!ctx || !key || !pos || !has_gauss || !gauss || K < 1 || D < 1 || n_half < 0) return VBMC_E_ARG;
// ... 70 lines not shown
```

pyvbmc_amd/csrc/entropy.hip:

```cpp
#include <cstdlib>

#include <algorithm>

#include "common.h"
#include "fastmath.h"
#include "entropy_args.h"
#include "philox.h"
#ifdef FIN_TIMES
__device__ unsigned long long g_glj_stamp;
#define GLJ_STAMP() (g_glj_stamp = wall_clock64())
#endif
#include "glj_block.h"

namespace {

constexpr int WG = 256;
constexpr int WAVES = WG / 64;

__device__ inline double wave_sum(double v) {
  return fm::wave_sum_dpp(v);
}


template <int DP>
// ... 314 lines not shown
}

template <int DP>
int launch_entmc_dp(vbmc_ctx* ctx, const EntArgs& a) {
  const int K = a.ml.K;
  size_t lds = sizeof(double) * ((size_t)K * DP + 4 * K + WAVES * (2 * DP + 1) + (size_t)WAVES * K);
  dim3 grid(a.chunks, K);
  hipLaunchKernelGGL(entmc_valu_kernel<DP>, grid, dim3(WG), lds, ctx->stream, a);
  return 0;
}

}

static bool use_ws_kernel(const vbmc_ctx* ctx, int D, int K) {
  if (ctx->opt_entmc_valu) return false;
  return D <= 32 && K <= 128;
}

static int ws_front_default(int DP, int KT) {
  if (DP <= 12) return 660;
  if (DP == 16) return KT <= 8 ? 0 : 570;
  return 660;
}

int entmc_plan(vbmc_ctx* ctx, int64_t ns_per_comp, int eps_mode, uint64_t seed, int64_t row_begin,
               int64_t row_count, int want_grad, EntPlan& p, int gp_items, int gp_per_slot) {
  const int D = ctx->D, K = ctx->K;
  p.DP = padded_d(D);
  if (p.DP < 0) return vbmc_fail(ctx, VBMC_E_UNSUP, "entmc: D=%d > 32 not supported", D);
  EntArgs& a = p.a;
  a.mix = ctx->d_mix;
  a.ml = ctx->ml;
  a.eps = ctx->d_eps;
  a.eps_rows = ctx->eps_rows;
  a.n_half = ns_per_comp / 2;
  a.row_begin = row_begin;
  a.row_count = row_count;
  a.seed = seed;
  a.eps_mode = eps_mode;
  a.want_grad = want_grad;
  const bool ws = use_ws_kernel(ctx, D, K);
  const int cus = ctx_cus(ctx);
  p.inv_ns = 1.0 / (double)ns_per_comp;
  int rows_per_wg = WG;
  a.rg = 1;
  size_t n_table = 0;
  if (ws) {
    const int64_t total_rows = row_count * K;
    int64_t rg = (total_rows + 64 * 2 * cus - 1) / (64 * 2 * cus);
    if (rg < 1) rg = 1;
    if (rg > 16) rg = 16;
    a.rg = (int)rg;
    rows_per_wg = 64 * a.rg;
    n_table = (size_t)K * (size_t)ws_table_rows(K) * (size_t)(p.DP + 6);
  }
  a.chunks = (int)((row_count + rows_per_wg - 1) / rows_per_wg);
  if (a.chunks < 1) a.chunks = 1;
  if (ws) {
    const int64_t slots = (int64_t)cus * ws_min_waves(p.DP, ws_ktmax_for(K), want_grad != 0);
    const int64_t fit = slots / K;
    if (fit >= 1 && a.chunks > fit && (int64_t)K * (a.chunks - 1) <= slots) {
      const int64_t rg2 = (row_count + 64 * fit - 1) / (64 * fit);
      if (rg2 <= 24) {
        a.rg = (int)rg2;
        rows_per_wg = 64 * a.rg;
        a.chunks = (int)((row_count + rows_per_wg - 1) / rows_per_wg);
      }
    }
  }
  a.roles = ws && ctx->opt_ws_roles ? 1 : 0;
  a.pair_cus = 0;
  if (ws) {
    const int64_t total = (int64_t)K * a.chunks;
    if (ws_min_waves(p.DP, ws_ktmax_for(K), want_grad != 0) == 2 && total > cus && total <= 2 * (int64_t)cus)
      a.pair_cus = cus;
  }
  EntArgs at_launch = a;
  {
    const size_t n_eps = (size_t)K * (size_t)row_count * D;
    if (eps_mode == VBMC_EPS_PHILOX && ctx->opt_elbo_pregen && n_eps > 0 && n_eps <= ((size_t)1 << 28)) {
      at_launch.eps_mode = VBMC_EPS_RESIDENT;
      at_launch.eps = (const double*)ctx;
    }
    if (at_launch.eps_mode == VBMC_EPS_RESIDENT && at_launch.eps == nullptr) at_launch.eps = (const double*)ctx;
  }
  p.kernel = !ws                                                          ? EntKernel::Valu
             : entmc_small_applies(at_launch, p.DP)                       ? EntKernel::Small
             : ctx->opt_entmc_mfma && entmc_mfma_applies(at_launch, p.DP) ? EntKernel::Mfma
                                                                          : EntKernel::Ws;
  a.sp = WsSpan();
  a.gp_wgs = 0;
  p.gp_in_ws = false;
  if (p.kernel == EntKernel::Ws && ctx->opt_ws_span) {
    const int waves = ws_min_waves(p.DP, ws_ktmax_for(K), want_grad != 0);
    WsSpan sp;
    sp.cus = cus;
    sp.nb = (int)((row_count + 63) >> 6);
    sp.pad = ctx->opt_ws_pad >= 0 ? ctx->opt_ws_pad : 3;
    sp.T = (int64_t)K * sp.nbv();
    sp.front = ctx->opt_ws_front > 0 ? ctx->opt_ws_front : ws_front_default(p.DP, ws_ktmax_for(K));
    static const int slots_env = [] {
      const char* e = getenv("VBMC_WS_GP_SLOTS");
      return e ? atoi(e) : 0;
    }();
    int WS_GP_SLOTS = 10;
    constexpr int WS_GP_PER = 5;
    int gp_wgs = 0;
    bool gp_here = false;
    if (gp_per_slot > 0) {
      gp_wgs = (gp_items + gp_per_slot - 1) / gp_per_slot;
      WS_GP_SLOTS = std::max(10, gp_wgs + 1);
      gp_here = waves == 2 && gp_wgs > 0 && WS_GP_SLOTS <= cus / 2;
      if (!gp_here) {
        WS_GP_SLOTS = 10;
        gp_wgs = 0;
      }
    } else {
      static const int per_env = [] {
        const char* e = getenv("VBMC_WS_GP_PER");
        return e ? atoi(e) : 0;
      }();
      const int per = per_env > 0 ? per_env : WS_GP_PER;
      if (slots_env > 0) WS_GP_SLOTS = slots_env;
      else if (gp_items > 10 * per && gp_items <= 100 * per) WS_GP_SLOTS = (gp_items + per - 1) / per;
      if (WS_GP_SLOTS > cus / 2) WS_GP_SLOTS = cus / 2;
      gp_wgs = gp_items > 0 ? std::min(WS_GP_SLOTS, (gp_items + per - 1) / per) : 0;
      gp_here = waves == 2 && gp_wgs > 0 && gp_items <= (per + 1) * WS_GP_SLOTS;
    }
    sp.pb = waves == 2 ? cus - WS_GP_SLOTS : 0;
    if (sp.pb == 0) sp.front = 1000;
    const int64_t min_part = sp.front > 0 ? (sp.pb > 0 ? 1000 - sp.front : sp.front) * sp.T / sp.W() : 0;
    if (min_part >= (gp_per_slot > 0 ? 2 : 3) && sp.T < ((int64_t)1 << 40)) {
      int R = 1;
      int longest = 0;
      for (int j = 0; j < K; ++j) {
        const int n = sp.part_of((int64_t)j * sp.nbv() + sp.nb - 1) - sp.part_of((int64_t)j * sp.nbv()) + 1;
        R = n > R ? n : R;
      }
      for (int u = 0; u < sp.n_parts(); ++u) longest = std::max(longest, (int)(sp.lo(u + 1) - sp.lo(u)));
      sp.R = R;
      a.sp = sp;
      a.chunks = R;
      a.rg = longest;
      a.pair_cus = 0;
      p.kernel = EntKernel::WsSpan;
      if (gp_here) {
        a.gp_wgs = gp_wgs;
        p.gp_in_ws = true;
      }
    }
  }
  a.stride = 2 + 2 * D + K;
  const size_t n_part = (size_t)K * a.chunks * a.stride;
  int rc = ensure_dev(ctx, &ctx->d_scratch, &ctx->d_scratch_cap, n_part + n_table);
  if (rc) return rc;
  a.partial = ctx->d_scratch;
  p.table = ws ? ctx->d_scratch + n_part : nullptr;
  return 0;
}

bool entmc_take_gp(const vbmc_ctx* ctx, EntPlan& p, const PrepArgs& gp) {
  if (gp.n_glj <= 0) return false;
  EntArgs& a = p.a;
  bool in_ws = false;
  if (p.kernel == EntKernel::WsSpan) {
    in_ws = p.gp_in_ws;
  } else if (p.kernel == EntKernel::Ws || p.kernel == EntKernel::Mfma) {
    const int slots = ctx_cus(ctx) * ws_min_waves(p.DP, ws_ktmax_for(ctx->K), a.want_grad != 0);
    const int free_slots = slots - ctx->K * a.chunks;
    in_ws = free_slots >= a.chunks && gp.n_glj <= 6 * a.chunks;
  }
  if (!in_ws) return false;
  a.gp = gp;
  a.gp_items = gp.n_glj;
  if (p.kernel == EntKernel::Mfma) p.kernel = EntKernel::Ws;
  return true;
}

extern "C" int vbmc_ws_span_layout(int cus, int pb, int front, int nb, int pad, int K, int64_t* part_lo, int* first_part,
                                   int* rows_per_component) {
  if (cus <= 0 || pb < 0 || pb > cus || front <= 0 || front >= 1000 + (pb == 0) || nb <= 0 || pad < 0 || K <= 0 || !part_lo ||
      !first_part || !rows_per_component)
    return VBMC_E_ARG;
  WsSpan sp;
  sp.cus = cus;
  sp.pb = pb;
  sp.front = front;
  sp.nb = nb;
  sp.pad = pad;
  sp.T = (int64_t)K * sp.nbv();
  for (int u = 0; u <= sp.n_parts(); ++u) part_lo[u] = sp.lo(u);
  int R = 1;
  for (int j = 0; j < K; ++j) {
    first_part[j] = sp.part_of((int64_t)j * sp.nbv());
    R = std::max(R, sp.part_of((int64_t)j * sp.nbv() + nb - 1) - first_part[j] + 1);
  }
  *rows_per_component = R;
  return VBMC_OK;
}

void entmc_fill_prep(const vbmc_ctx* ctx, const EntPlan& p, PrepArgs& a) {
  a.mix = ctx->d_mix;
  a.ml = ctx->ml;
  if (p.tabled()) {
    a.n_table = ctx->K;
    a.DP = p.DP;
    a.K4 = ws_table_rows(ctx->K);
    a.table = p.table;
  }
}

int entmc_pregen(vbmc_ctx* ctx, EntPlan& p, PrepArgs& pa) {
  const bool on = ctx->opt_elbo_pregen != 0;
  const int D = ctx->D, K = ctx->K;
  const size_t n_eps = (size_t)K * (size_t)p.a.row_count * D;
  if (!on || p.a.eps_mode != VBMC_EPS_PHILOX || n_eps == 0 || n_eps > ((size_t)1 << 28)) return 0;
  vbmc_ctx::AheadDraws& ah = ctx->ahead;
  int cur;
  if (ah.valid && ah.seed == p.a.seed && ah.K == K && ah.D == D && ah.rows == p.a.row_count &&
      ah.n_half == p.a.n_half && ah.row_begin == p.a.row_begin) {
    cur = ah.buf;
    p.pregen_hit = true;
    if (ah.frac < 1.0)
      pa.gen = make_gen_slice(ctx->d_epsgen[cur], K, D, p.a.row_count, p.a.n_half, p.a.row_begin, p.a.seed, nullptr, ah.frac, 1.0);
  } else {
    cur = ah.valid ? 1 - ah.buf : 0;
    int rc = ensure_dev(ctx, &ctx->d_epsgen[cur], &ctx->d_epsgen_cap[cur], n_eps);
    if (rc) return rc;
    pa.gen = make_gen_slice(ctx->d_epsgen[cur], K, D, p.a.row_count, p.a.n_half, p.a.row_begin, p.a.seed, nullptr, 0.0, 1.0);
  }
  ah.valid = false;
  ctx->gen_cur = cur;
  p.a.eps_mode = VBMC_EPS_RESIDENT;
  p.a.eps = ctx->d_epsgen[cur];
  p.a.eps_rows = p.a.row_count;
  return 0;
}

GenSlice entmc_ahead_slice(vbmc_ctx* ctx, const EntPlan& p) {
  const double frac_end = 1.0;
  const EntArgs& a = p.a;
  GenSlice none;
  if (!ctx->opt_elbo_ahead || a.eps == nullptr || a.eps != ctx->d_epsgen[ctx->gen_cur]) return none;
  const int D = ctx->D, K = ctx->K, other = 1 - ctx->gen_cur;
  const size_t n_eps = (size_t)K * (size_t)a.row_count * D;
  if (ctx->d_epsgen_cap[other] < n_eps || !ctx->d_epsgen[other]) {
    if (ctx->d_epsgen[other]) return none;
    if (ensure_dev(ctx, &ctx->d_epsgen[other], &ctx->d_epsgen_cap[other], n_eps)) return none;
  }
  vbmc_ctx::AheadDraws& ah = ctx->ahead;
  ah.seed = a.seed + 1;
  ah.K = K;
  ah.D = D;
  ah.rows = a.row_count;
  ah.n_half = a.n_half;
  ah.row_begin = a.row_begin;
  ah.buf = other;
  ah.frac = frac_end;
  ah.valid = true;
  return make_gen_slice(ctx->d_epsgen[other], K, D, a.row_count, a.n_half, a.row_begin, ah.seed, nullptr, 0.0, frac_end);
}

int entmc_launch_main(vbmc_ctx* ctx, const EntPlan& p) {
  const EntArgs& a = p.a;
  hipEvent_t e0 = ctx->timing ? ctx->ev[2 * T_ENTMC] : nullptr, e1 = ctx->timing ? ctx->ev[2 * T_ENTMC + 1] : nullptr;
  ctx->last_plan[0] = (int)p.kernel;
  ctx->last_plan[1] = a.rg;
  ctx->last_plan[2] = a.chunks;
  ctx->last_plan[3] = (a.eps_mode == VBMC_EPS_RESIDENT ? 1 : 0) | ((p.kernel == EntKernel::Ws || p.kernel == EntKernel::WsSpan) && a.roles ? 2 : 0);
  const bool bracket = ctx->timing && (p.kernel == EntKernel::Valu || p.kernel == EntKernel::Small);
  if (bracket) HIP_TRY(ctx, hipEventRecord(ctx->ev[2 * T_ENTMC], ctx->stream));
  switch (p.kernel) {
    case EntKernel::Small: launch_entmc_small(ctx->stream, a, p.DP, p.table); break;
    case EntKernel::Mfma: launch_entmc_mfma(ctx->stream, a, p.DP, p.table, e0, e1); break;
    case EntKernel::Ws:
    case EntKernel::WsSpan:
      switch (p.DP) {
#define VBMC_CASE_WS(dp) case dp: launch_entmc_ws_dp##dp(ctx->stream, a, p.table, e0, e1); break;
        VBMC_WS_DPS(VBMC_CASE_WS)
#undef VBMC_CASE_WS
      }
      break;
    case EntKernel::Valu:
      switch (p.DP) {
#define VBMC_CASE_VALU(dp) case dp: launch_entmc_dp<dp>(ctx, a); break;
        VBMC_WS_DPS(VBMC_CASE_VALU)
#undef VBMC_CASE_VALU
      }
      break;
    default: return vbmc_fail(ctx, VBMC_E_ARG, "entmc: plan names no entropy kernel (%d)", (int)p.kernel);
  }
  if (ctx->timing) {
    if (bracket) HIP_TRY(ctx, hipEventRecord(ctx->ev[2 * T_ENTMC + 1], ctx->stream));
    ctx->ev_valid[T_ENTMC] = true;
  }
  HIP_TRY(ctx, hipGetLastError());
  return 0;
}

namespace {
__global__ __launch_bounds__(256) void eps_gen_kernel(GenSlice g) { gen_slice_block(g, blockIdx.x, threadIdx.x); }
}

GenSlice make_gen_slice(double* eps, int K, int D, int64_t rows, int64_t n_half, int64_t row_begin,
                        uint64_t seed, const int* seed_add, double frac_begin, double frac_end) {
  GenSlice g;
  g.eps = eps;
  g.K = K;
  g.D = D;
  g.rows = rows;
  g.n_half = n_half;
  g.row_begin = row_begin;
  g.seed = seed;
  g.seed_add = seed_add;
  g.nb = (D + 3) / 4;
  auto magic = [](uint64_t d) { return (uint32_t)std::min<uint64_t>(d ? 0x100000000ull / d : 0, 0xFFFFFFFFull); };
  g.nb_magic = magic((uint64_t)g.nb);
  g.rows_magic = magic((uint64_t)rows);
  const int64_t total = (int64_t)K * rows * g.nb;
  const int64_t b = (int64_t)(frac_begin * (double)total), e = frac_end >= 1.0 ? total : (int64_t)(frac_end * (double)total);
  g.item_begin = b;
  g.item_count = e > b ? e - b : 0;
  g.n_blocks = (int)((g.item_count + 255) / 256);
  return g;
}

namespace {
__global__ __launch_bounds__(256) void entmc_publish_kernel(const double* __restrict__ src, DoneSignal done, GenSlice gen) {
  if (blockIdx.x > 0) {
    gen_slice_block(gen, blockIdx.x - 1, threadIdx.x);
    return;
  }
  if (done.ident_dst && threadIdx.x == 255) {
    __hip_atomic_store(done.ident_dst, *done.ident_src, __ATOMIC_RELAXED, __HIP_MEMORY_SCOPE_SYSTEM);
    __hip_atomic_store(done.ident_dst + 1, done.ident_seed, __ATOMIC_RELAXED, __HIP_MEMORY_SCOPE_SYSTEM);
  }
  staged_copy_to_host(src, done.host_out, done.host_n);
  __syncthreads();
  if (threadIdx.x == 0) __hip_atomic_store(done.flag, done.seq, __ATOMIC_RELAXED, __HIP_MEMORY_SCOPE_SYSTEM);
}
}

int entmc_launch_publish(vbmc_ctx* ctx, const double* d_raw, const DoneSignal& done, const GenSlice* gen) {
  const GenSlice g = gen ? *gen : GenSlice();
  hipLaunchKernelGGL(entmc_publish_kernel, dim3(1 + g.n_blocks), dim3(256), 0, ctx->stream, d_raw, done, g);
  HIP_TRY(ctx, hipGetLastError());
  return 0;
}

int launch_eps_gen(vbmc_ctx* ctx, hipStream_t st, const GenSlice& g) {
  if (g.n_blocks <= 0) return 0;
  hipLaunchKernelGGL(eps_gen_kernel, dim3((unsigned)g.n_blocks), dim3(256), 0, st, g);
  HIP_TRY(ctx, hipGetLastError());
  return 0;
}

int entmc_launch_finish(vbmc_ctx* ctx, const EntPlan& p, double* raw_out, const GenSlice* gen,
                        const DoneSignal* done) {
  const int n_out = raw_len(ctx->D, ctx->K);
  if ((uint64_t)ctx->K * (uint64_t)p.a.chunks * (uint64_t)p.a.stride >= ((uint64_t)1 << 31))
    return vbmc_fail(ctx, VBMC_E_UNSUP, "entropy: partial block of %d x %d rows too large", ctx->K, p.a.chunks);
  const GenSlice g = gen ? *gen : GenSlice();
  DoneSignal ds = done ? *done : DoneSignal();
  ds.sub_min = std::max(ds.sub_min, FIN_SUB_COUNTERS);
  hipLaunchKernelGGL(entmc_finish_kernel, dim3((n_out + 3) / 4 + g.n_blocks), dim3(256), 0, ctx->stream,
                     p.a.partial, p.a.chunks, p.a.stride, ctx->d_mix, ctx->ml, p.inv_ns,
                     p.a.want_grad, p.tabled() ? 1 : 0, raw_out, g, ds);
  HIP_TRY(ctx, hipGetLastError());
  return 0;
}

int launch_entmc(vbmc_ctx* ctx, int64_t ns_per_comp, int eps_mode, uint64_t seed,
                 int64_t row_begin, int64_t row_count, int want_grad, double* d_raw) {
  EntPlan p;
  int rc = entmc_plan(ctx, ns_per_comp, eps_mode, seed, row_begin, row_count, want_grad, p);
  if (rc) return rc;
  PrepArgs pa;
  entmc_fill_prep(ctx, p, pa);
  rc = entmc_pregen(ctx, p, pa);
  if (rc) return rc;
  rc = launch_prep(ctx, pa);
  if (rc) return rc;
  rc = entmc_launch_main(ctx, p);
  if (rc) return rc;
  return entmc_launch_finish(ctx, p, d_raw);
}

int launch_entlb(vbmc_ctx* ctx, double* d_res) {
  const int D = ctx->D, K = ctx->K;
  const size_t n_part = (size_t)K + (size_t)K * D, n_G = (size_t)K * K;
  int rc = ensure_dev(ctx, &ctx->d_scratch, &ctx->d_scratch_cap, n_part + n_G + K);
  if (rc) return rc;
  double* part = ctx->d_scratch;
  double* Gm = part + n_part;
  double* gsum = Gm + n_G;
  hipLaunchKernelGGL(entlb_rows_kernel, dim3(K), dim3(256), 0, ctx->stream, ctx->d_mix, ctx->ml, Gm,
                     gsum);
  size_t lds = sizeof(double) * (size_t)(WAVES * (2 * D + 2));
  hipLaunchKernelGGL(entlb_kernel, dim3(K), dim3(256), lds, ctx->stream, ctx->d_mix, ctx->ml, 1,
                     (const double*)Gm, (const double*)gsum, d_res, part);
  hipLaunchKernelGGL(entlb_finish_kernel, dim3((1 + D + 3) / 4), dim3(256), 0, ctx->stream,
                     ctx->d_mix, ctx->ml, 1, (const double*)part, d_res);
  HIP_TRY(ctx, hipGetLastError());
  return 0;
}
```

pyvbmc_amd/csrc/entropy_args.h:

```cpp
#pragma once
#include "common.h"

struct WsSpan {
  int cus = 0;
  int pb = 0;
  int front = 0;
  int nb = 0;
  int pad = 0;
  int R = 0;
  int64_t T = 0;
  __host__ __device__ int nbv() const { return nb + pad; }
  __host__ __device__ int n_parts() const { return cus + pb; }
  __host__ __device__ int64_t W() const { return (int64_t)pb * 1000 + (int64_t)(cus - pb) * front; }
  __host__ __device__ int64_t cw(int u) const {
    return u < 2 * pb ? (int64_t)(u >> 1) * 1000 + (int64_t)(u & 1) * front : (int64_t)pb * 1000 + (int64_t)(u - 2 * pb) * front;
  }
  __host__ __device__ int64_t lo(int u) const { return cw(u) * T / W(); }
  __host__ __device__ int part_of(int64_t g) const {
    const int64_t c = ((g + 1) * W() - 1) / T;
    int u;
    if (c < (int64_t)pb * 1000) {
      const int p = (int)(c / 1000);
      u = 2 * p + ((c - (int64_t)p * 1000) >= front ? 1 : 0);
    } else {
      u = 2 * pb + (int)((c - (int64_t)pb * 1000) / front);
    }
    return u < n_parts() ? u : n_parts() - 1;
  }
  __host__ __device__ int part_of_block(int b) const { return b < cus ? (b < pb ? 2 * b : 2 * pb + (b - pb)) : 2 * (b - cus) + 1; }
};

struct EntArgs {
  const double* mix;
  MixLayout ml;
  const double* eps;
  int64_t eps_rows;
  int64_t n_half;
  int64_t row_begin;
  int64_t row_count;
  uint64_t seed;
  int eps_mode;
  int want_grad;
  double* partial;
  int chunks;
  int stride;
  int rg;
  const void* extra = nullptr;
  int extra_lds = 0;
  int gp_items = 0;
  PrepArgs gp;
  int pair_cus = 0;
  WsSpan sp;
  int gp_wgs = 0;
  int roles = 0;
  const uint64_t* cancel = nullptr;
  const double* ship_src = nullptr;
  double* ship_dst = nullptr;
  int ship_n = 0;
  uint64_t* ship_flag = nullptr;
  uint64_t ship_seq = 0;
};

constexpr int ws_ktmax_for(int K) {
  const int KT = (K + 3) / 4;
  return KT <= 4 ? 4 : KT <= 8 ? 8 : KT <= 10 ? 10 : KT <= 13 ? 13 : KT <= 16 ? 16 : KT <= 20 ? 20 : KT <= 25 ? 25 : 32;
}
constexpr int ws_table_rows(int K) { return 4 * ws_ktmax_for(K); }
constexpr int ws_kt_role(int K, int r) { return K > r ? (K - r + 3) / 4 : 0; }
constexpr int ws_ktmin_for(int ktmax) {
  return ktmax <= 4 ? 1 : ktmax <= 8 ? 4 : ktmax <= 10 ? 8 : ktmax <= 13 ? 10 : ktmax <= 16 ? 13 : ktmax <= 20 ? 16 : ktmax <= 25 ? 20 : 25;
}
constexpr bool ws_kt_roles_cover(int kmax) {
  for (int K = 1; K <= kmax; ++K) {
    if (K >= 4 && ws_kt_role(K, 3) < ws_ktmin_for(ws_ktmax_for(K))) return false;
    if (ws_kt_role(K, 0) + ws_kt_role(K, 1) + ws_kt_role(K, 2) + ws_kt_role(K, 3) != K) return false;
    if (ws_kt_role(K, 0) > ws_ktmax_for(K) || ws_kt_role(K, 3) > ws_kt_role(K, 2) || ws_kt_role(K, 2) > ws_kt_role(K, 1)) return false;
  }
  return true;
}
static_assert(ws_kt_roles_cover(128), "the four roles own every component once, each at least ws_ktmin_for; roles 2 and 3 are the lightest");
constexpr int ws_min_waves(int dp, int ktmax, bool grad) {
#ifdef VBMC_WS_FORCE_WAVES
  return VBMC_WS_FORCE_WAVES;
#else
  return (grad && 4 * dp + 3 * ktmax > 95) ? 1 : 2;
#endif
}

enum class EntKernel : int { Valu = 0, Ws = 1, Small = 2, Mfma = 3, AdamFused = 4, WsSpan = 5, AdamTail = 6 };

struct EntPlan {
  EntArgs a;
  EntKernel kernel = EntKernel::Valu;
  bool gp_in_ws = false;
  bool pregen_hit = false;
  int DP = 0;
  double inv_ns = 0.0;
  double* table = nullptr;
  bool tabled() const { return kernel != EntKernel::Valu; }
};

#define VBMC_WS_DPS(X) X(2) X(4) X(6) X(8) X(10) X(12) X(16) X(20) X(24) X(32)
inline int padded_d(int D) {
#define VBMC_PAD_D(dp) if (D <= dp) return dp;
  VBMC_WS_DPS(VBMC_PAD_D)
#undef VBMC_PAD_D
  return -1;
}
#define VBMC_DECL_WS(dp) \
  void launch_entmc_ws_dp##dp(hipStream_t st, const EntArgs& a, const double* d_table, hipEvent_t e0, hipEvent_t e1);
VBMC_WS_DPS(VBMC_DECL_WS)
#undef VBMC_DECL_WS

bool entmc_mfma_applies(const EntArgs& a, int DP);
void launch_entmc_mfma(hipStream_t st, const EntArgs& a, int DP, const double* d_table, hipEvent_t e0, hipEvent_t e1);

bool entmc_small_applies(const EntArgs& a, int DP);
void launch_entmc_small(hipStream_t st, const EntArgs& a, int DP, const double* d_table);
```

pyvbmc_amd/csrc/entropy_ws.hip:

```cpp
#include <hip/hip_ext.h>

#include <type_traits>

#include "adam_dev.h"
#include "common.h"
#include "entropy_args.h"
#include "fastmath.h"
#include "glj_block.h"

#ifndef WS_EXP2_N
#define WS_EXP2_N VBMC_ENT_EXP2_N
#endif
constexpr int EN = WS_EXP2_N;
__device__ __forceinline__ double exp2_vc(double x, const double (&c)[EN]) {
  const double t = __builtin_rint(x);
  const double f = x - t;
  const int n = (int)t;
  double p = c[EN - 1];
#pragma unroll
  for (int i = EN - 2; i >= 0; --i) p = fma(p, f, c[i]);
  p = fma(p, f, 1.0);
  return __builtin_amdgcn_ldexp(p, n);
}
__device__ __forceinline__ void exp2_vc2(double x1, double x2, const double (&c)[EN], double& r1,
                                         double& r2) {
  const double t1 = __builtin_rint(x1), t2 = __builtin_rint(x2);
  const double f1 = x1 - t1, f2 = x2 - t2;
  const int n1 = (int)t1, n2 = (int)t2;
  double p1 = c[EN - 1], p2 = c[EN - 1];
#pragma unroll
  for (int i = EN - 2; i >= 0; --i) {
    p1 = fma(p1, f1, c[i]);
    p2 = fma(p2, f2, c[i]);
  }
  p1 = fma(p1, f1, 1.0);
  p2 = fma(p2, f2, 1.0);
  r1 = __builtin_amdgcn_ldexp(p1, n1);
  r2 = __builtin_amdgcn_ldexp(p2, n2);
}
#if WS_EXP2_N == VBMC_ENT_EXP2_N
__device__ const double kExp2C[EN] = VBMC_ENT_EXP2_COEFFS;
#elif WS_EXP2_N == 10
__device__ const double kExp2C[10] = {0x1.62e42fefa3a19p-1, 0x1.ebfbdff82c598p-3, 0x1.c6b08d703ce49p-5, 0x1.3b2ab6fba1ddap-7, 0x1.5d87fe9d7a584p-10, 0x1.430913096fd9fp-13, 0x1.ffcb54062e698p-17, 0x1.62bfd47773353p-20, 0x1.b675bca4eeebbp-24, 0x1.e6063f7217bc6p-28};
#elif WS_EXP2_N == 9
__device__ const double kExp2C[9] = {0x1.62e42fefa39f7p-1, 0x1.ebfbdff8149f2p-3, 0x1.c6b08d7044119p-5, 0x1.3b2ab72b175eep-7, 0x1.5d87fe908f88ap-10, 0x1.43088e257f341p-13, 0x1.ffcb76789860fp-17, 0x1.63ef969a64d3cp-20, 0x1.b6571de2f2351p-24};
#endif

#include "philox.h"

#ifndef VBMC_DP
#error "compile with -DVBMC_DP=<padded D>"
#endif

namespace {

constexpr int WG = 256;
constexpr int WAVES = WG / 64;

__device__ __forceinline__ double wave_sum(double v) { return fm::wave_sum_dpp(v); }

constexpr int ws_dmin(int dp) { return dp <= 12 ? dp - 1 : dp == 16 ? 13 : dp == 20 ? 17 : dp == 24 ? 21 : 25; }

constexpr int ws_epi_cap_doubles(int dp, int ktmax, bool grad) { return (ws_min_waves(dp, ktmax, grad) >= 2 ? 44 : 100) * 1024 / 8; }
constexpr int ws_epi_nq(int dp, int ktmax, bool grad) {
  if (!grad) return 0;
  const int ni = 1 + 2 * dp + ktmax;
  for (int nq = 1; nq <= 3; ++nq)
    if (WAVES * ni * ((64 >> nq) + 1) <= ws_epi_cap_doubles(dp, ktmax, grad)) return nq;
  return 0;
}
constexpr int ws_epi_doubles(int dp, int ktmax, bool grad) {
  const int nq = ws_epi_nq(dp, ktmax, grad);
  return nq == 0 ? 0 : WAVES * (1 + 2 * dp + ktmax) * ((64 >> nq) + 1);
}

template <int KK, int KTMIN, int KTMAX, class F>
__device__ __forceinline__ void ws_for_owned(int kt, F&& f) {
  if constexpr (KK < KTMAX) {
    if constexpr (KK >= KTMIN)
      if (KK == kt) return;
    f(std::integral_constant<int, KK>());
    ws_for_owned<KK + 1, KTMIN, KTMAX>(kt, f);
  }
}
template <int N>
__device__ __forceinline__ void ws_keep(const double (&r)[N]) {
#pragma unroll
  for (int i = 0; i < N; ++i) asm volatile("" : : "s"(r[i]));
}

#if defined(WS_TIMES) && VBMC_DP == 10
__device__ unsigned long long g_ws_times[1024 * 4];
#define WS_STAMP(i) do { if (threadIdx.x == 0) g_ws_times[(blockIdx.y * gridDim.x + blockIdx.x) * 4 + (i)] = wall_clock64(); } while (0)
#else
#define WS_STAMP(i) (void)0
#endif
constexpr int ws_dprev(int dp) { return dp <= 12 ? dp - 2 : dp == 16 ? 12 : dp == 20 ? 16 : dp == 24 ? 20 : 24; }
template <int DP, int KTMAX, bool GRAD, bool PHILOX, int STAGE = 0>
__global__ __launch_bounds__(WG, ws_min_waves(DP, KTMAX, GRAD)) void entmc_ws_kernel(
    EntArgs a, const double* __restrict__ T) {
  constexpr int TS = DP + 6;
  __shared__ double sQ[2][WAVES][2][64];
  constexpr int GB = 4;
  __shared__ __attribute__((aligned(16))) double sE[PHILOX ? GB : 2][DP][64];
  __shared__ double sRed[WAVES][2 * DP + 1];
  __shared__ int sSimd[WAVES];
  extern __shared__ double dyn[];
  constexpr int EPI = ws_epi_doubles(DP, KTMAX, GRAD);
  double* sW = dyn + EPI;

  constexpr bool EXTRA_ROW = GRAD && !PHILOX;
  const bool span = a.sp.cus > 0;
  if constexpr (EXTRA_ROW) {
    if (a.extra != nullptr && (span ? (int)blockIdx.x == a.sp.n_parts() + (a.gp_items > 0 ? a.gp_wgs : 0) : blockIdx.y == 0)) {
      if (span || blockIdx.x == 0) {
        const adam_dev::AdamDev& pa = *(const adam_dev::AdamDev*)a.extra;
        if (a.gp_items > 0 && a.gp.done.dev) {
          if (threadIdx.x == 0) {
            const unsigned long long t0 = wall_clock64();
            while (__hip_atomic_load(a.gp.done.flag, __ATOMIC_RELAXED, __HIP_MEMORY_SCOPE_AGENT) != a.gp.done.seq) {
              if (wall_clock64() - t0 > 2000000ull) {
                atomicOr(pa.status, 8);
                break;
              }
              __builtin_amdgcn_s_sleep(8);
            }
            __builtin_amdgcn_fence(__ATOMIC_ACQUIRE, "agent");
          }
          __syncthreads();
        }
        if (a.extra_lds > 0) adam_dev::adam_pre_body<true>(pa, dyn, &sRed[0][0], pa.pre);
        else adam_dev::adam_pre_body<false>(pa, nullptr, &sRed[0][0], pa.pre);
      }
      return;
    }
  }
  if (a.cancel != nullptr && __hip_atomic_load(a.cancel, __ATOMIC_RELAXED, __HIP_MEMORY_SCOPE_SYSTEM) == ~(uint64_t)0) return;
  if (a.gp_items > 0 && (span ? (int)blockIdx.x >= a.sp.n_parts() && (int)blockIdx.x < a.sp.n_parts() + a.gp_wgs : blockIdx.y == gridDim.y - 1)) {
    const int first = span ? (int)blockIdx.x - a.sp.n_parts() : (int)blockIdx.x, step = span ? a.gp_wgs : (int)gridDim.x;
    if (a.gp.x_lds) {
      if (first < a.gp_items) glj_stage_x(a.gp, dyn);
      for (int it = first; it < a.gp_items; it += step) {
        glj_block<true, DP, ws_dmin(DP), true>(a.gp, it, dyn);
        __syncthreads();
      }
    } else {
      for (int it = first; it < a.gp_items; it += step) {
        glj_block<false, DP, ws_dmin(DP), true>(a.gp, it, dyn);
        __syncthreads();
      }
    }
    return;
  }
  const int D = a.ml.D;
  constexpr int KT = KTMAX, K4 = KT * 4;
  int64_t g_lo, g_hi;
  int nb, part = 0, chunk_slot = 0, j_chunk = 0;
  int nbv;
  bool filler = false;
  if (span) {
    nb = a.sp.nb;
    nbv = a.sp.nbv();
    filler = (int)blockIdx.x >= a.sp.cus;
    part = a.sp.part_of_block((int)blockIdx.x);
    g_lo = a.sp.lo(part);
    g_hi = a.sp.lo(part + 1);
  } else {
    int j = (EXTRA_ROW && a.extra != nullptr) ? blockIdx.y - 1 : blockIdx.y, chunk = blockIdx.x;
    if (a.pair_cus > 0) {
      const int total = a.ml.K * a.chunks, b = j * a.chunks + chunk;
      const int paired = total - a.pair_cus;
      filler = b >= a.pair_cus;
      if (paired > 0 && b < 2 * a.pair_cus) {
        const int m = b < a.pair_cus ? b : b - a.pair_cus;
        const int item = m < paired ? 2 * m + (b >= a.pair_cus ? 1 : 0) : paired + m;
        j = item / a.chunks;
        chunk = item - j * a.chunks;
      }
    }
    nb = (int)((a.row_count + 63) >> 6);
    nbv = nb;
    chunk_slot = chunk;
    j_chunk = j;
    const int64_t i0 = (int64_t)chunk * a.rg;
    g_lo = (int64_t)j * nb + (i0 < nb ? i0 : nb);
    g_hi = (int64_t)j * nb + (i0 + a.rg < nb ? i0 + a.rg : nb);
  }
  const int tid = threadIdx.x, lane = tid & 63;
  const int wave = __builtin_amdgcn_readfirstlane(tid >> 6);
  int role = wave;
  if (a.roles) {
    const int simd = (int)__builtin_amdgcn_s_getreg(4 | (4 << 6) | (1 << 11));
    if (lane == 0) sSimd[wave] = simd;
    __syncthreads();
    const int seen = (1 << sSimd[0]) | (1 << sSimd[1]) | (1 << sSimd[2]) | (1 << sSimd[3]);
    role = __builtin_amdgcn_readfirstlane(seen == 0xF ? (simd + (filler ? 2 : 0)) & 3 : wave);
  }
  constexpr int KTMIN = ws_ktmin_for(KTMAX);
  const int kt_own = ws_kt_role(a.ml.K, role);
  const int kt_r = __builtin_amdgcn_readfirstlane(a.roles ? (kt_own > KTMIN ? kt_own : KTMIN) : KTMAX);
  WS_STAMP(0);
  constexpr bool eps_exact = !PHILOX && STAGE != 0;

  double ec[EN];
  {
    int vz;
    asm volatile("v_mov_b32 %0, 0" : "=v"(vz));
#pragma unroll
    for (int i = 0; i < EN; ++i) ec[i] = kExp2C[i + vz];
  }
  WS_STAMP(1);
  bool first_stretch = true;
  for (int64_t g = g_lo; g < g_hi || (first_stretch && !span);) {
  first_stretch = false;
  const int j = span ? (int)(g / nbv) : j_chunk;
  const int ib0 = (int)(g - (int64_t)j * nbv);
  if (span && ib0 >= nb) {
    g = (int64_t)(j + 1) * nbv;
    continue;
  }
  const int n_it = g < g_hi ? (int)((g_hi - g < nb - ib0) ? g_hi - g : nb - ib0) : 0;
  const int slot = span ? part - a.sp.part_of((int64_t)j * nbv) : chunk_slot;
  const double sig_j = a.mix[a.ml.o_sig + j];
  const double sj2 = sig_j * sig_j;
  const double two_sj = 2.0 * sig_j;
  const double* Tj = T + (size_t)j * K4 * TS;
  double slog_acc = 0.0;
  double mu_acc[DP], lam_acc[DP], Wacc[KTMAX];
#pragma unroll
  for (int d = 0; d < DP; ++d) mu_acc[d] = lam_acc[d] = 0.0;
#pragma unroll
  for (int kk = 0; kk < KTMAX; ++kk) Wacc[kk] = 0.0;

  auto ws_fill = [&](int ib, int buf) {
    if constexpr (!PHILOX && STAGE == 1) {
      const char* base = (const char*)(a.eps + ((int64_t)j * a.eps_rows + ((int64_t)ib << 6)) * DP);
      const int64_t left = (a.row_count - ((int64_t)ib << 6)) * (DP * 8) - 16;
      const unsigned last = (unsigned)(left < 64 * DP * 8 - 16 ? left : 64 * DP * 8 - 16);
#pragma unroll
      for (int c = 0; c < DP / 2; ++c) {
        if ((c & 3) != wave) continue;
        unsigned voff = (unsigned)(c * 1024 + lane * 16);
        voff = voff < last ? voff : last;
        const unsigned dst = (unsigned)(uintptr_t)&sE[buf][0][0] + (unsigned)(c * 1024);
        asm volatile("s_mov_b32 m0, %2\n\ts_nop 0\n\tglobal_load_lds_dwordx4 %0, %1" : : "v"(voff), "s"(base), "s"(dst) : "memory");
      }
    } else if constexpr (!PHILOX && STAGE == 2) {
      const char* base = (const char*)(a.eps + ((int64_t)j * a.eps_rows + ((int64_t)ib << 6)) * D);
      const int64_t left = (a.row_count - ((int64_t)ib << 6)) * (int64_t)(D * 8);
      const int blk = 64 * D * 8;
      if ((((uintptr_t)base) & 15) == 0 && (left >= blk || (left >= 16 && (left & 15) == 0))) {
        const unsigned last = (unsigned)((left < blk ? left : blk) - 16);
        for (int c = wave; c < (D + 1) / 2; c += WAVES) {
          unsigned voff = (unsigned)(c * 1024 + lane * 16);
          voff = voff < last ? voff : last;
          const unsigned dst = (unsigned)__builtin_amdgcn_readfirstlane((int)((unsigned)(uintptr_t)&sE[buf][0][0] + (unsigned)(c * 1024)));
          asm volatile("s_mov_b32 m0, %2\n\ts_nop 0\n\tglobal_load_lds_dwordx4 %0, %1" : : "v"(voff), "s"(base), "s"(dst) : "memory");
        }
      } else {
        const unsigned last = (unsigned)((left < blk ? left : blk) - 4);
        for (int c = wave; c < 2 * D; c += WAVES) {
          unsigned voff = (unsigned)(c * 256 + lane * 4);
          voff = voff < last ? voff : last;
          const unsigned dst = (unsigned)__builtin_amdgcn_readfirstlane((int)((unsigned)(uintptr_t)&sE[buf][0][0] + (unsigned)(c * 256)));
          asm volatile("s_mov_b32 m0, %2\n\ts_nop 0\n\tglobal_load_lds_dword %0, %1" : : "v"(voff), "s"(base), "s"(dst) : "memory");
        }
      }
    }
  };
  (void)ws_fill;
  if (eps_exact && n_it > 0) {
    ws_fill(ib0, 0);
    asm volatile("s_waitcnt vmcnt(0)" ::: "memory");
    __syncthreads();
  }
  constexpr int LOGB = 8;
  double lmant = 1.0;
  int lexp = 0;

  for (int it = 0; it < n_it; ++it) {
    const int64_t i_loc = ((int64_t)(ib0 + it) << 6) + lane;
    const bool valid = i_loc < a.row_count;

    double e[DP];
#pragma unroll
    for (int d = 0; d < DP; ++d) e[d] = 0.0;
    if (!PHILOX) {
      if constexpr (eps_exact) {
        if (it + 1 < n_it) ws_fill(ib0 + it + 1, (it + 1) & 1);
        if constexpr (STAGE == 1) {
          const double2* rp = (const double2*)&sE[it & 1][0][0] + lane * (DP / 2);
#pragma unroll
          for (int d = 0; d < DP / 2; ++d) {
            const double2 v = rp[d];
            e[2 * d] = v.x;
            e[2 * d + 1] = v.y;
          }
        } else {
          const double* rp = &sE[it & 1][0][0] + lane * D;
#pragma unroll
          for (int d = 0; d < DP; ++d) e[d] = rp[d];
#pragma unroll
          for (int d = ws_dprev(DP) + 1; d < DP; ++d) e[d] = d < D ? e[d] : 0.0;
        }
      } else if (valid) {
        const double* rp = a.eps + ((int64_t)j * a.eps_rows + i_loc) * D;
#pragma unroll
        for (int d = 0; d < DP; ++d)
          if (d < D) e[d] = rp[d];
      }
    } else {
      constexpr int NP = DP / 2;
      const int nbk = (D + 3) / 4;
      if ((it % GB) == 0) {
        const int nb = min(GB, n_it - it);
        __syncthreads();
        for (int q = wave; q < nb * nbk; q += WAVES) {
          const int bq = q / nbk, blk = q - bq * nbk;
          const int64_t il = ((int64_t)(ib0 + it + bq) << 6) + lane;
          const uint64_t grow = (uint64_t)j * (uint64_t)a.n_half + (uint64_t)(a.row_begin + il);
          double z[4];
          philox_normal_quad(grow, (uint32_t)blk, a.seed, z);
#pragma unroll
          for (int c = 0; c < 4; ++c)
            if (4 * blk + c < DP) sE[bq][4 * blk + c][lane] = z[c];
        }
        __syncthreads();
      }
      (void)NP;
#pragma unroll
      for (int d = 0; d < DP; ++d)
        if (valid && d < D) e[d] = sE[it % GB][d][lane];
    }
    double e2 = 0.0;
#pragma unroll
    for (int d = 0; d < DP; ++d) e2 = fma(e[d], e[d], e2);
    const double b = sj2 * e2;

    int zoff;
    asm volatile("s_mov_b32 %0, 0" : "=s"(zoff));
    const double* Tw = Tj + (size_t)role * TS + zoff;

    double qp = 0.0, qm = 0.0;
    double rp_[KTMAX], rm_[KTMAX];
    constexpr int NR1 = DP + 3;
    double cur[NR1];
    {
      const double* tr = Tw;
#pragma unroll
      for (int i = 0; i < NR1; ++i) cur[i] = tr[i];
    }
    int kt1;
    asm volatile("s_mov_b32 %0, %1" : "=s"(kt1) : "s"(kt_r));
    ws_for_owned<0, KTMIN, KTMAX>(kt1, [&](auto kc) __attribute__((always_inline)) {
      constexpr int kk = decltype(kc)::value;
      double nxt[NR1];
      {
        __builtin_amdgcn_s_waitcnt(0xC07F);
        __builtin_amdgcn_sched_barrier(0);
        if (kk + 1 < KTMAX) {
          const double* tn = Tw + (size_t)(4 * (kk + 1)) * TS;
#pragma unroll
          for (int i = 0; i < NR1; ++i) nxt[i] = tn[i];
        }
        __builtin_amdgcn_sched_barrier(0);
        double c = 0.0;
#pragma unroll
        for (int d = 0; d < DP; ++d) c = fma(cur[d], e[d], c);
        const double sp = fma(two_sj, c, b);
        const double sm = fma(-two_sj, c, b);
        double rp, rm;
        exp2_vc2(fma(cur[DP + 1], sp, cur[DP + 0]), fma(cur[DP + 1], sm, cur[DP + 0]), ec, rp, rm);
        rp_[kk] = rp;
        rm_[kk] = rm;
        qp = fma(cur[DP + 2], rp, qp);
        qm = fma(cur[DP + 2], rm, qm);
#pragma unroll
        for (int i = 0; i < NR1; ++i) cur[i] = nxt[i];
        if (kk + 1 < KTMAX && kk + 1 >= KTMIN) ws_keep(cur);
      }
    });
    const int buf = it & 1;
    sQ[buf][role][0][lane] = qp;
    sQ[buf][role][1][lane] = qm;
    if constexpr (eps_exact) asm volatile("s_waitcnt vmcnt(0)" ::: "memory");
    __syncthreads();
    qp = (sQ[buf][0][0][lane] + sQ[buf][1][0][lane]) + (sQ[buf][2][0][lane] + sQ[buf][3][0][lane]);
    qm = (sQ[buf][0][1][lane] + sQ[buf][1][1][lane]) + (sQ[buf][2][1][lane] + sQ[buf][3][1][lane]);

    if (role >= 2) {
      const double qv = valid ? (role == 2 ? qp : qm) : 1.0;
      lmant *= __builtin_amdgcn_frexp_mant(qv);
      lexp += __builtin_amdgcn_frexp_exp(qv);
      if ((it & (LOGB - 1)) == LOGB - 1 || it + 1 == n_it) {
        slog_acc += fma((double)lexp, 0x1.62e42fefa39efp-1, fm::log_fast(lmant));
        lmant = 1.0;
        lexp = 0;
      }
    }
    if (GRAD) {
      const double ip = valid ? fm::rcp_fast(qp) : 0.0;
      const double im = valid ? fm::rcp_fast(qm) : 0.0;
      double sgs = 0.0, sgd = 0.0;
      double Td[DP];
#pragma unroll
      for (int d = 0; d < DP; ++d) Td[d] = 0.0;
      constexpr int NR2 = DP + 4;
      double c2[NR2];
      {
        const double* tr = Tw;
#pragma unroll
        for (int d = 0; d < DP; ++d) c2[d] = tr[d];
        c2[DP + 3] = tr[DP + 3];
      }
      int kt2;
      asm volatile("s_mov_b32 %0, %1" : "=s"(kt2) : "s"(kt_r));
      ws_for_owned<0, KTMIN, KTMAX>(kt2, [&](auto kc) __attribute__((always_inline)) {
        constexpr int kk = decltype(kc)::value;
        double n2[NR2];
        {
          __builtin_amdgcn_s_waitcnt(0xC07F);
          __builtin_amdgcn_sched_barrier(0);
          if (kk + 1 < KTMAX) {
            const double* tn = Tw + (size_t)(4 * (kk + 1)) * TS;
#pragma unroll
            for (int d = 0; d < DP; ++d) n2[d] = tn[d];
            n2[DP + 3] = tn[DP + 3];
          }
          __builtin_amdgcn_sched_barrier(0);
          const double t2 = rm_[kk] * im;
          const double ts = fma(rp_[kk], ip, t2), td = fma(rp_[kk], ip, -t2);
          Wacc[kk] += ts;
          sgs = fma(ts, c2[DP + 3], sgs);
          const double gd = td * c2[DP + 3];
          sgd += gd;
#pragma unroll
          for (int d = 0; d < DP; ++d) Td[d] = fma(gd, c2[d], Td[d]);
#pragma unroll
          for (int d = 0; d < DP; ++d) c2[d] = n2[d];
          c2[DP + 3] = n2[DP + 3];
          if (kk + 1 < KTMAX && kk + 1 >= KTMIN) {
#pragma unroll
            for (int d = 0; d < DP; ++d) asm volatile("" : : "s"(c2[d]));
            asm volatile("" : : "s"(c2[DP + 3]));
          }
        }
      });
      const double cs = sig_j * sgs, cd = sig_j * sgd;
#pragma unroll
      for (int d = 0; d < DP; ++d) {
        mu_acc[d] = fma(e[d], cd, mu_acc[d]);
        lam_acc[d] = fma(e[d], fma(e[d], cs, Td[d]), lam_acc[d]);
      }
    }
  }

  WS_STAMP(2);
  if constexpr (EPI > 0) {
    constexpr int NQ = ws_epi_nq(DP, KTMAX, GRAD);
    constexpr int GL = 1 << NQ, NV = 64 / GL;
    constexpr int NI = 1 + 2 * DP + KTMAX, RS = NV + 1;
    static_assert(NQ >= 1 && NQ <= 3 && WAVES * NI * RS == EPI, "epilogue buffer");
    auto group = [](double v) {
      v += fm::dpp_get<0xB1, 0xf>(v);
      if constexpr (NQ >= 2) v += fm::dpp_get<0x4E, 0xf>(v);
      if constexpr (NQ >= 3) v += fm::dpp_get<0x141, 0xf>(v);
      return v;
    };
    {
      double* mine = dyn + (size_t)role * NI * RS + (lane / GL);
      const bool wr = (lane & (GL - 1)) == 0;
      double v = group(slog_acc);
      if (wr) mine[0] = v;
#pragma unroll
      for (int d = 0; d < DP; ++d) {
        v = group(mu_acc[d]);
        if (wr) mine[(1 + d) * RS] = v;
        v = group(lam_acc[d]);
        if (wr) mine[(1 + DP + d) * RS] = v;
      }
#pragma unroll
      for (int kk = 0; kk < KTMAX; ++kk) {
        v = group(Wacc[kk]);
        if (wr) mine[(1 + 2 * DP + kk) * RS] = v;
      }
    }
    __syncthreads();
    for (int r = tid; r < WAVES * NI; r += WG) {
      const int wv = r / NI, it = r - wv * NI;
      const double* row = dyn + (size_t)r * RS;
      double x[NV];
#pragma unroll
      for (int l = 0; l < NV; ++l) x[l] = row[l];
      double s0 = 0.0, s1 = 0.0, s2 = 0.0, s3 = 0.0;
#pragma unroll
      for (int l = 0; l < NV; l += 4) {
        s0 += x[l];
        s1 += x[l + 1];
        s2 += x[l + 2];
        s3 += x[l + 3];
      }
      const double sum = (s0 + s1) + (s2 + s3);
      if (it <= 2 * DP) {
        sRed[wv][it] = sum;
      } else {
        const int kk = it - 1 - 2 * DP;
        sW[4 * kk + wv] = sum;
      }
    }
    __syncthreads();
  } else {
    {
      const double v = wave_sum(slog_acc);
      if (lane == 0) sRed[role][0] = v;
    }
    if (GRAD) {
#pragma unroll
      for (int d = 0; d < DP; ++d) {
        const double vmu = wave_sum(mu_acc[d]);
        const double vlam = wave_sum(lam_acc[d]);
        if (lane == 0) {
          sRed[role][1 + d] = vmu;
          sRed[role][1 + DP + d] = vlam;
        }
      }
#pragma unroll
      for (int kk = 0; kk < KTMAX; ++kk)
        {
          const double v = wave_sum(Wacc[kk]);
          if (lane == 0) sW[4 * kk + role] = v;
        }
    }
    __syncthreads();
  }

  WS_STAMP(3);
  double* out = a.partial + ((int64_t)j * a.chunks + slot) * a.stride;
  for (int t = tid; t < a.stride; t += WG) {
    double v = 0.0;
    if (t == 0) {
      for (int wv = 0; wv < WAVES; ++wv) v += sRed[wv][0];
    } else if (GRAD) {
      if (t <= D) {
        for (int wv = 0; wv < WAVES; ++wv) v += sRed[wv][t];
      } else if (t == D + 1) {
        for (int d = 0; d < D; ++d)
          for (int wv = 0; wv < WAVES; ++wv) v += sRed[wv][1 + DP + d];
      } else if (t < 2 * D + 2) {
        const int d = t - (D + 2);
        for (int wv = 0; wv < WAVES; ++wv) v += sRed[wv][1 + DP + d];
      } else {
        v = sW[t - (2 * D + 2)];
      }
    }
    out[t] = v;
  }
  if (span) {
    if (ib0 + n_it == nb)
      for (int t = tid; t < (a.chunks - 1 - slot) * a.stride; t += WG) out[a.stride + t] = 0.0;
    __syncthreads();
  }
  g += n_it;
  if (!span) break;
  }
}

template <int DP, int KTMAX>
void launch_one(hipStream_t st, const EntArgs& a_in, const double* d_table, hipEvent_t e0, hipEvent_t e1) {
  EntArgs a = a_in;
  const int K = a.ml.K;
  const int K4 = 4 * KTMAX;
  size_t lds = sizeof(double) * ((size_t)K4 + ws_epi_doubles(DP, KTMAX, a.want_grad != 0));
  const bool philox = a.eps_mode == VBMC_EPS_PHILOX;
  const bool extra_row = a.extra != nullptr && a.want_grad && !philox;
  const dim3 grid = a.sp.cus > 0 ? dim3(a.sp.n_parts() + (a.gp_items > 0 ? a.gp_wgs : 0) + (extra_row ? 1 : 0))
                                 : dim3(a.chunks, K + (extra_row ? 1 : 0) + (a.gp_items > 0 ? 1 : 0));
  const dim3 block(WG);
  if (extra_row && sizeof(double) * (size_t)a.extra_lds > lds) lds = sizeof(double) * (size_t)a.extra_lds;
  if (a.gp_items > 0 && glj_block_lds(a.ml.D, a.gp.N) > lds) lds = glj_block_lds(a.ml.D, a.gp.N);
  {
    static const bool x_lds_on = [] {
      const char* e = getenv("VBMC_GLJ_X_LDS");
      return !(e && e[0] == '0');
    }();
    a.gp.x_lds = (x_lds_on && a.gp_items > 0 && glj_block_lds_x(a.ml.D, a.gp.N) <= lds) ? 1 : 0;
  }
  int dev = 0;
  if (lds > 32 * 1024) (void)hipGetDevice(&dev);
#define VBMC_LAUNCH_WS(G, P, X)                                                                           \
  do {                                                                                                    \
    auto kern = entmc_ws_kernel<DP, KTMAX, G, P, X>;                                                      \
    static size_t lds_limit[64] = {};                \
    if (lds > 32 * 1024 && lds > lds_limit[dev & 63]) {                                                   \
      (void)hipFuncSetAttribute((const void*)kern, hipFuncAttributeMaxDynamicSharedMemorySize, (int)lds); \
      lds_limit[dev & 63] = lds;                                                                          \
    }                                                                                                     \
    hipExtLaunchKernelGGL(kern, grid, block, (std::uint32_t)lds, st, e0, e1, 0u, a, d_table);             \
  } while (0)
  const bool exact = !philox && a.ml.D == DP && (DP % 2) == 0 && ((uintptr_t)a.eps & 15) == 0;
  if (a.want_grad) {
    if (philox) VBMC_LAUNCH_WS(true, true, 0); else if (exact) VBMC_LAUNCH_WS(true, false, 1); else VBMC_LAUNCH_WS(true, false, 2);
  } else {
    if (philox) VBMC_LAUNCH_WS(false, true, 0); else if (exact) VBMC_LAUNCH_WS(false, false, 1); else VBMC_LAUNCH_WS(false, false, 2);
  }
#undef VBMC_LAUNCH_WS
}

}

#define VBMC_CAT2(a, b) a##b
#define VBMC_CAT(a, b) VBMC_CAT2(a, b)

void VBMC_CAT(launch_entmc_ws_dp, VBMC_DP)(hipStream_t st, const EntArgs& a, const double* d_table, hipEvent_t e0,
                                            hipEvent_t e1) {
  switch (ws_ktmax_for(a.ml.K)) {
    case 4: launch_one<VBMC_DP, 4>(st, a, d_table, e0, e1); break;
    case 8: launch_one<VBMC_DP, 8>(st, a, d_table, e0, e1); break;
    case 10: launch_one<VBMC_DP, 10>(st, a, d_table, e0, e1); break;
    case 13: launch_one<VBMC_DP, 13>(st, a, d_table, e0, e1); break;
    case 16: launch_one<VBMC_DP, 16>(st, a, d_table, e0, e1); break;
    case 20: launch_one<VBMC_DP, 20>(st, a, d_table, e0, e1); break;
    case 25: launch_one<VBMC_DP, 25>(st, a, d_table, e0, e1); break;
    default: launch_one<VBMC_DP, 32>(st, a, d_table, e0, e1); break;
  }
}

#if defined(WS_TIMES) && VBMC_DP == 10
extern "C" int vbmc_debug_ws_times(unsigned long long* out, int n) {
  return (int)hipMemcpyFromSymbol(out, HIP_SYMBOL(g_ws_times), sizeof(unsigned long long) * n);
}
#endif
```

pyvbmc_amd/csrc/ws_table.h:

```cpp
#pragma once
#include "common.h"

__device__ __forceinline__ void ws_table_row_block(const double* mix, const MixLayout& ml, int j, int DP, int K4,
                                                   double* table, double* lds) {
  const int D = ml.D, K = ml.K, tid = threadIdx.x, TS = DP + 6;
  const double* mup = mix + ml.o_mup;
  double* sV2 = lds;
  const int kt = min(tid, K - 1);
  const double t_is2 = mix[ml.o_is2 + kt], t_w = mix[ml.o_w + kt], t_lrc = mix[ml.o_lrc + kt];
  constexpr int U = 8;
  for (int base = 0; base < K4 * DP; base += U * 256) {
    double vj[U], vk[U];
#pragma unroll
    for (int u = 0; u < U; ++u) {
      if (base + u * 256 >= K4 * DP) break;
      const int idx = base + u * 256 + tid;
      const int k = idx / DP, d = idx - k * DP;
      vj[u] = mup[j * D + min(d, D - 1)];
      vk[u] = mup[min(k, K - 1) * D + min(d, D - 1)];
    }
#pragma unroll
    for (int u = 0; u < U; ++u) {
      if (base + u * 256 >= K4 * DP) break;
      const int idx = base + u * 256 + tid;
      const int k = idx / DP, d = idx - k * DP;
      if (idx < K4 * DP) {
        const double v = (d < D && k < K) ? (vj[u] - vk[u]) : 0.0;
        table[((size_t)j * K4 + k) * TS + d] = v;
        sV2[idx] = v * v;
      }
    }
  }
  __syncthreads();
  for (int k = tid; k < K4; k += 256) {
    double* row = table + ((size_t)j * K4 + k) * TS;
    double s = 0.0;
    for (int d = 0; d < DP; ++d) s += sV2[k * DP + d];
    if (k < K) {
      const bool pre = k == tid;
      const double is2 = pre ? t_is2 : mix[ml.o_is2 + k];
      const double w = pre ? t_w : mix[ml.o_w + k];
      const double ak = -0.5 * 0x1.71547652b82fep+0 * is2;
      row[DP + 0] = fma(ak, s, pre ? t_lrc : mix[ml.o_lrc + k]);
      row[DP + 1] = ak;
      row[DP + 2] = w;
      row[DP + 3] = w * is2;
    } else {
      row[DP + 0] = -2000.0; row[DP + 1] = 0.0; row[DP + 2] = 0.0; row[DP + 3] = 0.0;
    }
    row[DP + 4] = 0.0;
    row[DP + 5] = 0.0;
  }
}
```

Before: 12490 evals/s.

## Fuse armed-prep table build into entropy kernel with per-row ready flags

When a speculative armed evaluation is issued, the separate prep kernel is no longer launched. The GP-row workgroups of the WS entropy kernel now wait on the host go flag, copy the mixture pack, and build the per-component distance table rows. Each finished row is published through a per-row flag that the entropy workgroups spin on before they use it. The GP/GLJ work may also be folded into extra grid rows when enough slots are free. This removes a kernel launch and the serialisation between prep and entropy, at the cost of device-side spin waits, extra LDS, atomic table stores, and possible deadlock or timeout risk if the workgroups are not co-resident.

```diff
diff --git a/include/vbmc_hip.h b/include/vbmc_hip.h
--- a/include/vbmc_hip.h
+++ b/include/vbmc_hip.h
@@ -68,6 +68,7 @@
 int vbmc_set_gp_watch(vbmc_ctx* ctx, const double* const* ptrs, const int64_t* lens, int n, uint64_t expected);
 
 int vbmc_armed_stats(const vbmc_ctx* ctx, uint64_t out[6]);
+int vbmc_armed_fused_hits(const vbmc_ctx* ctx, uint64_t* out);
 
 int vbmc_last_elbo_raw(const vbmc_ctx* ctx, double* out, int n);
 
diff --git a/pyvbmc_amd/_lib.py b/pyvbmc_amd/_lib.py
--- a/pyvbmc_amd/_lib.py
+++ b/pyvbmc_amd/_lib.py
@@ -166,6 +166,7 @@
                                       C.POINTER(C.c_int), C.POINTER(C.c_int)]),
     "vbmc_last_elbo_raw": (C.c_int, [_vp, _dp, C.c_int]),
     "vbmc_armed_stats": (C.c_int, [_vp, C.POINTER(C.c_uint64)]),
+    "vbmc_armed_fused_hits": (C.c_int, [_vp, C.POINTER(C.c_uint64)]),
     "vbmc_set_gp_watch": (C.c_int, [_vp, C.POINTER(C.c_void_p), C.POINTER(C.c_int64), C.c_int, C.c_uint64]),
     "vbmc_host_checksum": (C.c_int, [C.POINTER(C.c_void_p), C.POINTER(C.c_int64), C.c_int, C.POINTER(C.c_uint64)]),
     "vbmc_set_timing": (C.c_int, [_vp, C.c_int]),
@@ -428,7 +429,7 @@
         out = (C.c_int * 4)()
         self.check(self._lib.vbmc_last_entmc_plan(self._h, out))
         return {"kernel": ("valu", "ws", "small", "mfma", "adam_fused", "ws", "ws")[out[0]] if out[0] >= 0 else None, "rg": out[1],
-                "chunks": out[2], "resident_draws": bool(out[3] & 1), "roles": bool(out[3] & 2), "span": out[0] in (5, 6), "adam_tail": out[0] == 6}
+                "chunks": out[2], "resident_draws": bool(out[3] & 1), "roles": bool(out[3] & 2), "armed_fused": bool(out[3] & 4), "span": out[0] in (5, 6), "adam_tail": out[0] == 6}
 
     def philox_normals(self, K, n_half, D, seed, row_begin=0, row_count=None):
         row_count = n_half - row_begin if row_count is None else row_count
@@ -439,7 +440,11 @@
     def armed_stats(self):
         out = (C.c_uint64 * 6)()
         self.check(self._lib.vbmc_armed_stats(self._h, out))
-        return dict(zip(("hits", "cancels", "late", "ident_checked", "ident_bad", "lost"), (int(v) for v in out)))
+        st = dict(zip(("hits", "cancels", "late", "ident_checked", "ident_bad", "lost"), (int(v) for v in out)))
+        fh = C.c_uint64()
+        self.check(self._lib.vbmc_armed_fused_hits(self._h, C.byref(fh)))
+        st["fused_hits"] = int(fh.value)
+        return st
 
     def last_elbo_raw(self, D, K):
         out = np.empty(1 + D * K + 2 * K + D)
diff --git a/pyvbmc_amd/csrc/api_elbo.hip b/pyvbmc_amd/csrc/api_elbo.hip
--- a/pyvbmc_amd/csrc/api_elbo.hip
+++ b/pyvbmc_amd/csrc/api_elbo.hip
@@ -193,8 +193,9 @@
     if (spin && !fg) return -1000;
     const bool ident = fg != nullptr && mc;
     if (ident) pa.ident_out = (uint64_t*)(ctx->d_done_cnt + 12);
+    PrepArgs gp_tail;
     if (fg) {
-      PrepArgs gp_tail = pa;
+      gp_tail = pa;
       gp_tail.n_table = 0;
       gp_tail.gen = GenSlice();
       gp_tail.mix = ctx->d_mix;
@@ -228,9 +229,43 @@
       pa.dead = ctx->hd_done + 5;
       plan.a.cancel = ctl;
     }
+    ctx->issued_fused = false;
+    if (spin && ctx->opt_arm_fused && mc && ident && ctx->d_row_flag && pa.gen.n_blocks == 0 && pa.n_table > 0 &&
+        (plan.kernel == EntKernel::Ws || plan.kernel == EntKernel::WsSpan) && plan.a.eps_mode == VBMC_EPS_RESIDENT && K <= 128 &&
+        ws_armed2_built(plan.DP, ws_ktmax_for(K), plan.a.want_grad != 0) &&
+        ws_armed_build_doubles(ctx->ml, plan.DP, ws_table_rows(K)) <= WS_ARMED_BUILD_CAP) {
+      if (plan.a.gp_items == 0 && pa.n_glj > 0 && plan.kernel == EntKernel::Ws) {
+        const int slots = ctx_cus(ctx) * ws_min_waves(plan.DP, ws_ktmax_for(K), plan.a.want_grad != 0);
+        const int rows = (pa.n_glj + 6 * plan.a.chunks - 1) / (6 * plan.a.chunks);
+        if (slots - K * plan.a.chunks >= rows * plan.a.chunks) {
+          plan.a.gp_rows = rows;
+          plan.a.gp = gp_tail;
+          plan.a.gp_items = pa.n_glj;
+          pa.n_glj = 0;
+          ctx->gp_where = 2;
+        }
+      }
+      if (plan.a.gp_items > 0 && pa.n_glj == 0) {
+        EntArgs& ea = plan.a;
+        ea.row_flag = ctx->d_row_flag;
+        ea.go = pa.go;
+        ea.go_seq = pa.go_seq;
+        ea.go_timeout = pa.go_timeout;
+        ea.dead = pa.dead;
+        ea.pack = fg;
+        ea.mix_copy = pa.mix_copy;
+        ea.mix_copy_n = pa.mix_copy_n;
+        ea.ident_out = pa.ident_out;
+        ea.table_w = plan.table;
+        ea.gp.mix = fg;
+        ctx->issued_fused = true;
+      }
+    }
     HSTAMP(1);
-    rc2 = launch_prep(ctx, pa);
-    if (rc2) return rc2;
+    if (!ctx->issued_fused) {
+      rc2 = launch_prep(ctx, pa);
+      if (rc2) return rc2;
+    }
     polled_out = false;
     if (mc) {
       rc2 = entmc_launch_main(ctx, plan);
@@ -302,6 +337,7 @@
       const bool force_late = ctx->opt_arm_late_test > 0 && --ctx->opt_arm_late_test == 0;
       if (!force_late && std::chrono::duration<double, std::milli>(clk::now() - sp.t_armed).count() < sp.limit_ms + ARM_LATE_SLACK_MS) {
         ++sp.hits;
+        if (sp.fused) ++sp.fused_hits;
         used_armed = true;
         polled = true;
         cur_seq = sp.seq;
@@ -346,6 +382,7 @@
     if (rc2 == 0 && p2) {
       sp.armed = true;
       sp.ident = ident_out_flag;
+      sp.fused = ctx->issued_fused;
       sp.limit_ms = arm_limit_ms;
       sp.t_armed = t_arm0;
       sp.seq = seq2;
@@ -573,6 +610,12 @@
   return VBMC_OK;
 }
 
+extern "C" int vbmc_armed_fused_hits(const vbmc_ctx* ctx, uint64_t* out) {
+  if (!ctx || !out) return VBMC_E_ARG;
+  *out = ctx->spec.fused_hits;
+  return VBMC_OK;
+}
+
 extern "C" int vbmc_last_elbo_raw(const vbmc_ctx* ctx, double* out, int n) {
   if (!ctx || !out || ctx->last_raw_n <= 0 || n != ctx->last_raw_n || !ctx->h_pinned) return VBMC_E_ARG;
   memcpy(out, ctx->h_pinned + ctx->last_raw_off, sizeof(double) * (size_t)n);
diff --git a/pyvbmc_amd/csrc/common.h b/pyvbmc_amd/csrc/common.h
--- a/pyvbmc_amd/csrc/common.h
+++ b/pyvbmc_amd/csrc/common.h
@@ -162,10 +162,13 @@
     double ahead_before_frac = 1.0;
     uint64_t hits = 0, cancels = 0, late = 0, ident_checked = 0, ident_bad = 0, lost = 0;
     bool ident = false;
+    bool fused = false;
+    uint64_t fused_hits = 0;
     double limit_ms = 1.0;
     std::chrono::steady_clock::time_point t_armed;
   } spec;
   uint64_t* d_ctl = nullptr;
+  uint64_t* d_row_flag = nullptr;
   double* d_stage = nullptr;
   size_t d_stage_cap = 0;
   double* d_mix_fg = nullptr;
@@ -239,6 +242,8 @@
   int opt_adam_tail = 1;
   int opt_ident_test = 0;
   bool ident_retry = false;
+  int opt_arm_fused = 1;
+  bool issued_fused = false;
   int opt_elbo_arm = 1;
   bool counted = false;
   int opt_ws_span = 1;
diff --git a/pyvbmc_amd/csrc/ctx.hip b/pyvbmc_amd/csrc/ctx.hip
--- a/pyvbmc_amd/csrc/ctx.hip
+++ b/pyvbmc_amd/csrc/ctx.hip
@@ -99,6 +99,8 @@
   c->opt_elbo_ahead = !(e && e[0] == '0');
   e = getenv("VBMC_ELBO_ARM");
   c->opt_elbo_arm = e ? atoi(e) : 1;
+  e = getenv("VBMC_ARM_FUSED");
+  c->opt_arm_fused = !(e && e[0] == '0');
   e = getenv("VBMC_ACQ_POLL");
   c->opt_acq_poll = !(e && e[0] == '0');
   e = getenv("VBMC_ADAM_FUSED");
@@ -262,6 +264,7 @@
   if (getenv("VBMC_DEBUG_ARM")) fprintf(stderr, "[vbmc] armed evaluations: %llu used, %llu cancelled\n", (unsigned long long)ctx->spec.hits, (unsigned long long)ctx->spec.cancels);
   if (ctx->stream) (void)hipStreamSynchronize(ctx->stream);
   if (ctx->d_ctl) (void)hipFree(ctx->d_ctl);
+  if (ctx->d_row_flag) (void)hipFree(ctx->d_row_flag);
   vbmc_comm_destroy(ctx);
   adam_free(ctx);
   acq_is_free(ctx);
@@ -340,6 +343,7 @@
   else if (!strcmp(key, "ws_pad")) ctx->opt_ws_pad = value > 8 ? 8 : value;
   else if (!strcmp(key, "ws_front")) ctx->opt_ws_front = value < 0 ? 0 : value > 990 ? 990 : value;
   else if (!strcmp(key, "elbo_arm")) ctx->opt_elbo_arm = value < 0 ? 0 : value > 2 ? 2 : value;
+  else if (!strcmp(key, "elbo_arm_fused")) ctx->opt_arm_fused = value != 0;
   else if (!strcmp(key, "acq_poll")) ctx->opt_acq_poll = value != 0;
   else if (!strcmp(key, "is_mcmc_threads")) ctx->opt_is_mcmc_threads = value <= 256 ? 256 : value >= 768 ? 768 : 512;
   else if (!strcmp(key, "gp_lml_chunk")) ctx->opt_gp_lml_chunk = value < 0 ? 0 : value;
@@ -564,6 +568,12 @@
     } else {
       memset(ctx->d_ctl, 0, 64);
       __builtin_ia32_sfence();
+    }
+  }
+  if (!ctx->d_row_flag) {
+    if (hipMalloc((void**)&ctx->d_row_flag, 128 * sizeof(uint64_t)) != hipSuccess || hipMemset(ctx->d_row_flag, 0, 128 * sizeof(uint64_t)) != hipSuccess) {
+      (void)hipGetLastError();
+      ctx->d_row_flag = nullptr;
     }
   }
   memcpy(ctx->d_mix_fg, ctx->h_pack, n * sizeof(double));
diff --git a/pyvbmc_amd/csrc/entropy.hip b/pyvbmc_amd/csrc/entropy.hip
--- a/pyvbmc_amd/csrc/entropy.hip
+++ b/pyvbmc_amd/csrc/entropy.hip
@@ -490,10 +490,11 @@
   }
   a.stride = 2 + 2 * D + K;
   const size_t n_part = (size_t)K * a.chunks * a.stride;
-  int rc = ensure_dev(ctx, &ctx->d_scratch, &ctx->d_scratch_cap, n_part + n_table);
+  const size_t table_at = (n_part + 15) & ~(size_t)15;
+  int rc = ensure_dev(ctx, &ctx->d_scratch, &ctx->d_scratch_cap, table_at + n_table);
   if (rc) return rc;
   a.partial = ctx->d_scratch;
-  p.table = ws ? ctx->d_scratch + n_part : nullptr;
+  p.table = ws ? ctx->d_scratch + table_at : nullptr;
   return 0;
 }
 
@@ -605,7 +606,8 @@
   ctx->last_plan[0] = (int)p.kernel;
   ctx->last_plan[1] = a.rg;
   ctx->last_plan[2] = a.chunks;
-  ctx->last_plan[3] = (a.eps_mode == VBMC_EPS_RESIDENT ? 1 : 0) | ((p.kernel == EntKernel::Ws || p.kernel == EntKernel::WsSpan) && a.roles ? 2 : 0);
+  ctx->last_plan[3] = (a.eps_mode == VBMC_EPS_RESIDENT ? 1 : 0) | ((p.kernel == EntKernel::Ws || p.kernel == EntKernel::WsSpan) && a.roles ? 2 : 0) |
+                      (a.row_flag != nullptr ? 4 : 0);
   const bool bracket = ctx->timing && (p.kernel == EntKernel::Valu || p.kernel == EntKernel::Small);
   if (bracket) HIP_TRY(ctx, hipEventRecord(ctx->ev[2 * T_ENTMC], ctx->stream));
   switch (p.kernel) {
diff --git a/pyvbmc_amd/csrc/entropy_args.h b/pyvbmc_amd/csrc/entropy_args.h
--- a/pyvbmc_amd/csrc/entropy_args.h
+++ b/pyvbmc_amd/csrc/entropy_args.h
@@ -52,6 +52,7 @@
   int pair_cus = 0;
   WsSpan sp;
   int gp_wgs = 0;
+  int gp_rows = 1;
   int roles = 0;
   const uint64_t* cancel = nullptr;
   const double* ship_src = nullptr;
@@ -59,7 +60,24 @@
   int ship_n = 0;
   uint64_t* ship_flag = nullptr;
   uint64_t ship_seq = 0;
+  uint64_t* row_flag = nullptr;
+  uint64_t* go = nullptr;
+  uint64_t go_seq = 0;
+  uint64_t go_timeout = 0;
+  uint64_t* dead = nullptr;
+  const double* pack = nullptr;
+  double* mix_copy = nullptr;
+  int mix_copy_n = 0;
+  uint64_t* ident_out = nullptr;
+  double* table_w = nullptr;
 };
+constexpr uint64_t WS_ROW_CANCEL = (uint64_t)1 << 63;
+inline size_t ws_armed_build_doubles(const MixLayout& ml, int DP, int K4) { return (size_t)ml.total + (size_t)K4 * DP + 16 + 1; }
+constexpr size_t WS_ARMED_BUILD_CAP = 4096;
+constexpr bool ws_armed2_built(int dp, int ktmax, bool grad) {
+  const int s = 4 * dp + 3 * ktmax;
+  return dp <= 12 && (!grad || s <= 80 || s > 95);
+}
 
 constexpr int ws_ktmax_for(int K) {
   const int KT = (K + 3) / 4;
diff --git a/pyvbmc_amd/csrc/entropy_ws.hip b/pyvbmc_amd/csrc/entropy_ws.hip
--- a/pyvbmc_amd/csrc/entropy_ws.hip
+++ b/pyvbmc_amd/csrc/entropy_ws.hip
@@ -7,6 +7,7 @@
 #include "entropy_args.h"
 #include "fastmath.h"
 #include "glj_block.h"
+#include "ws_table.h"
 
 #ifndef WS_EXP2_N
 #define WS_EXP2_N VBMC_ENT_EXP2_N
@@ -90,11 +91,125 @@
 }
 
 #if defined(WS_TIMES) && VBMC_DP == 10
-__device__ unsigned long long g_ws_times[1024 * 4];
-#define WS_STAMP(i) do { if (threadIdx.x == 0) g_ws_times[(blockIdx.y * gridDim.x + blockIdx.x) * 4 + (i)] = wall_clock64(); } while (0)
+constexpr int WS_NSTAMP = 6;
+__device__ unsigned long long g_ws_times[2 * 1024 * WS_NSTAMP];
+#define WS_STAMP(i) do { if (threadIdx.x == 0) g_ws_times[((a.go_seq & 1) * 1024 + blockIdx.y * gridDim.x + blockIdx.x) * WS_NSTAMP + (i)] = wall_clock64(); } while (0)
 #else
 #define WS_STAMP(i) (void)0
 #endif
+
+__device__ __noinline__ int ws_armed_build(uint64_t* go, uint64_t go_seq, uint64_t go_timeout, uint64_t* dead, uint64_t* row_flag,
+                                           const double* pack, int ml_D, int ml_K, int ml_mup, int ml_is2, int ml_w, int ml_lrc,
+                                           int ml_total, int DP, int K4, double* table, double* mix_copy, uint64_t* ident_out, int b,
+                                           int n_bld, double* dyn) {
+  MixLayout ml;
+  ml.D = ml_D;
+  ml.K = ml_K;
+  ml.o_mup = ml_mup;
+  ml.o_is2 = ml_is2;
+  ml.o_w = ml_w;
+  ml.o_lrc = ml_lrc;
+  ml.total = ml_total;
+  const int tid = threadIdx.x, n = ml.total;
+  double* sV2 = dyn + n;
+  unsigned long long* s_ck = (unsigned long long*)(sV2 + K4 * DP);
+  int* s_st = (int*)(s_ck + 16);
+  if (tid == 0) {
+    const unsigned long long t0 = wall_clock64();
+    int st = 0;
+    for (;;) {
+      const uint64_t v = __hip_atomic_load(go, __ATOMIC_RELAXED, __HIP_MEMORY_SCOPE_SYSTEM);
+      if (v == go_seq) { st = 1; break; }
+      if (v == ~(uint64_t)0) break;
+      if (wall_clock64() - t0 > go_timeout) {
+        if (b == 0) {
+          __hip_atomic_store(go, ~(uint64_t)0, __ATOMIC_RELAXED, __HIP_MEMORY_SCOPE_SYSTEM);
+          __hip_atomic_store(dead, go_seq, __ATOMIC_RELAXED, __HIP_MEMORY_SCOPE_SYSTEM);
+        }
+        break;
+      }
+      __builtin_amdgcn_s_sleep(2);
+    }
+    *s_st = st;
+  }
+  __syncthreads();
+  if (*s_st == 0) {
+    for (int j = b + tid * n_bld; j < ml.K; j += 256 * n_bld)
+      __hip_atomic_store(row_flag + j, go_seq | WS_ROW_CANCEL, __ATOMIC_RELAXED, __HIP_MEMORY_SCOPE_AGENT);
+    return 0;
+  }
+  {
+    constexpr int U = 16;
+    for (int base = 0; base < n; base += U * 256) {
+      double v[U];
+#pragma unroll
+      for (int u = 0; u < U; ++u) {
+        if (base + u * 256 >= n) break;
+        v[u] = pack[min(base + u * 256 + tid, n - 1)];
+      }
+#pragma unroll
+      for (int u = 0; u < U; ++u) {
+        if (base + u * 256 >= n) break;
+        const int i = base + u * 256 + tid;
+        if (i < n) dyn[i] = v[u];
+      }
+    }
+  }
+  __syncthreads();
+  for (int j = b; j < ml.K; j += n_bld) {
+    ws_table_row_block<true>(dyn, ml, j, DP, K4, table, sV2);
+    __builtin_amdgcn_s_waitcnt(0x0F70);
+    __syncthreads();
+    if (tid == 0) __hip_atomic_store(row_flag + j, go_seq, __ATOMIC_RELAXED, __HIP_MEMORY_SCOPE_AGENT);
+  }
+  if (b == 0 && mix_copy != nullptr) {
+    uint64_t ck = 0;
+    for (int i = tid; i < n; i += 256) {
+      const double v = dyn[i];
+      mix_copy[i] = v;
+      ck += pack_ck_term(v, (uint32_t)i);
+    }
+    if (ident_out != nullptr) {
+      if (tid < 16) s_ck[tid] = 0;
+      __syncthreads();
+      __hip_atomic_fetch_add(&s_ck[tid & 15], (unsigned long long)ck, __ATOMIC_RELAXED, __HIP_MEMORY_SCOPE_WORKGROUP);
+      __syncthreads();
+      if (tid == 0) {
+        unsigned long long t = 0;
+        for (int i = 0; i < 16; ++i) t += s_ck[i];
+        *ident_out = t;
+      }
+    }
+  }
+  __syncthreads();
+  return 1;
+}
+
+__device__ __forceinline__ int ws_armed_wait(const uint64_t* flag, uint64_t go_seq, uint64_t go_timeout, uint64_t* go, uint64_t* dead,
+                                          int* s_st) {
+  if (threadIdx.x == 0) {
+    const unsigned long long t0 = wall_clock64();
+    int st = 0;
+    for (;;) {
+      const uint64_t v = __hip_atomic_load(flag, __ATOMIC_RELAXED, __HIP_MEMORY_SCOPE_AGENT);
+      if (v == go_seq) { st = 1; break; }
+      if (v == (go_seq | WS_ROW_CANCEL)) break;
+      if (wall_clock64() - t0 > go_timeout + (go_timeout >> 1)) {
+        __hip_atomic_store(go, ~(uint64_t)0, __ATOMIC_RELAXED, __HIP_MEMORY_SCOPE_SYSTEM);
+        __hip_atomic_store(dead, go_seq, __ATOMIC_RELAXED, __HIP_MEMORY_SCOPE_SYSTEM);
+        break;
+      }
+      __builtin_amdgcn_s_sleep(2);
+    }
+    *s_st = st;
+  }
+  __syncthreads();
+  const int st = *s_st;
+  __builtin_amdgcn_fence(__ATOMIC_ACQUIRE, "agent");
+  __builtin_amdgcn_s_dcache_inv();
+  __syncthreads();
+  return st;
+}
 constexpr int ws_dprev(int dp) { return dp <= 12 ? dp - 2 : dp == 16 ? 12 : dp == 20 ? 16 : dp == 24 ? 20 : 24; }
 template <int DP, int KTMAX, bool GRAD, bool PHILOX, int STAGE = 0>
 __global__ __launch_bounds__(WG, ws_min_waves(DP, KTMAX, GRAD)) void entmc_ws_kernel(
@@ -105,6 +220,7 @@
   __shared__ __attribute__((aligned(16))) double sE[PHILOX ? GB : 2][DP][64];
   __shared__ double sRed[WAVES][2 * DP + 1];
   __shared__ int sSimd[WAVES];
+  __shared__ int sGo;
   extern __shared__ double dyn[];
   constexpr int EPI = ws_epi_doubles(DP, KTMAX, GRAD);
   double* sW = dyn + EPI;
@@ -135,9 +251,19 @@
       return;
     }
   }
-  if (a.cancel != nullptr && __hip_atomic_load(a.cancel, __ATOMIC_RELAXED, __HIP_MEMORY_SCOPE_SYSTEM) == ~(uint64_t)0) return;
-  if (a.gp_items > 0 && (span ? (int)blockIdx.x >= a.sp.n_parts() && (int)blockIdx.x < a.sp.n_parts() + a.gp_wgs : blockIdx.y == gridDim.y - 1)) {
-    const int first = span ? (int)blockIdx.x - a.sp.n_parts() : (int)blockIdx.x, step = span ? a.gp_wgs : (int)gridDim.x;
+  const bool gp_row = a.gp_items > 0 && (span ? (int)blockIdx.x >= a.sp.n_parts() && (int)blockIdx.x < a.sp.n_parts() + a.gp_wgs : (int)blockIdx.y >= (int)gridDim.y - a.gp_rows);
+  constexpr bool ARMED2 = !PHILOX && ws_armed2_built(DP, KTMAX, GRAD);
+  const bool armed2 = ARMED2 && a.row_flag != nullptr;
+  if (a.cancel != nullptr && !(armed2 && gp_row) && __hip_atomic_load(a.cancel, __ATOMIC_RELAXED, __HIP_MEMORY_SCOPE_SYSTEM) == ~(uint64_t)0) return;
+  if (gp_row) {
+    const int first = span ? (int)blockIdx.x - a.sp.n_parts() : ((int)blockIdx.y - ((int)gridDim.y - a.gp_rows)) * (int)gridDim.x + (int)blockIdx.x;
+    const int step = span ? a.gp_wgs : a.gp_rows * (int)gridDim.x;
+    if constexpr (ARMED2) {
+      if (armed2 && !__builtin_amdgcn_readfirstlane(ws_armed_build(a.go, a.go_seq, a.go_timeout, a.dead, a.row_flag, a.pack, a.ml.D, a.ml.K, a.ml.o_mup, a.ml.o_is2,
+                                                                        a.ml.o_w, a.ml.o_lrc, a.ml.total, DP, 4 * KTMAX, a.table_w, a.mix_copy,
+                                                                        a.ident_out, first, step, dyn)))
+        return;
+    }
     if (a.gp.x_lds) {
       if (first < a.gp_items) glj_stage_x(a.gp, dyn);
       for (int it = first; it < a.gp_items; it += step) {
@@ -221,9 +347,8 @@
   }
   const int n_it = g < g_hi ? (int)((g_hi - g < nb - ib0) ? g_hi - g : nb - ib0) : 0;
   const int slot = span ? part - a.sp.part_of((int64_t)j * nbv) : chunk_slot;
-  const double sig_j = a.mix[a.ml.o_sig + j];
-  const double sj2 = sig_j * sig_j;
-  const double two_sj = 2.0 * sig_j;
+  double sig_j = 0.0;
+  if (!armed2) sig_j = a.mix[a.ml.o_sig + j];
   const double* Tj = T + (size_t)j * K4 * TS;
   double slog_acc = 0.0;
   double mu_acc[DP], lam_acc[DP], Wacc[KTMAX];
@@ -274,6 +399,16 @@
     asm volatile("s_waitcnt vmcnt(0)" ::: "memory");
     __syncthreads();
   }
+  if (g == g_lo) WS_STAMP(4);
+  if constexpr (ARMED2) {
+    if (armed2 && n_it > 0) {
+      if (!__builtin_amdgcn_readfirstlane(ws_armed_wait(a.row_flag + j, a.go_seq, a.go_timeout, a.go, a.dead, &sGo))) return;
+      sig_j = a.pack[a.ml.o_sig + j];
+    }
+  }
+  if (g == g_lo) WS_STAMP(5);
+  const double sj2 = sig_j * sig_j;
+  const double two_sj = 2.0 * sig_j;
   constexpr int LOGB = 8;
   double lmant = 1.0;
   int lexp = 0;
@@ -574,7 +709,7 @@
   const bool philox = a.eps_mode == VBMC_EPS_PHILOX;
   const bool extra_row = a.extra != nullptr && a.want_grad && !philox;
   const dim3 grid = a.sp.cus > 0 ? dim3(a.sp.n_parts() + (a.gp_items > 0 ? a.gp_wgs : 0) + (extra_row ? 1 : 0))
-                                 : dim3(a.chunks, K + (extra_row ? 1 : 0) + (a.gp_items > 0 ? 1 : 0));
+                                 : dim3(a.chunks, K + (extra_row ? 1 : 0) + (a.gp_items > 0 ? a.gp_rows : 0));
   const dim3 block(WG);
   if (extra_row && sizeof(double) * (size_t)a.extra_lds > lds) lds = sizeof(double) * (size_t)a.extra_lds;
   if (a.gp_items > 0 && glj_block_lds(a.ml.D, a.gp.N) > lds) lds = glj_block_lds(a.ml.D, a.gp.N);
@@ -585,6 +720,7 @@
     }();
     a.gp.x_lds = (x_lds_on && a.gp_items > 0 && glj_block_lds_x(a.ml.D, a.gp.N) <= lds) ? 1 : 0;
   }
+  if (a.row_flag != nullptr && sizeof(double) * ws_armed_build_doubles(a.ml, DP, K4) > lds) lds = sizeof(double) * ws_armed_build_doubles(a.ml, DP, K4);
   int dev = 0;
   if (lds > 32 * 1024) (void)hipGetDevice(&dev);
 #define VBMC_LAUNCH_WS(G, P, X)                                                                           \
diff --git a/pyvbmc_amd/csrc/ws_table.h b/pyvbmc_amd/csrc/ws_table.h
--- a/pyvbmc_amd/csrc/ws_table.h
+++ b/pyvbmc_amd/csrc/ws_table.h
@@ -1,6 +1,12 @@
 #pragma once
 #include "common.h"
 
+template <bool WT>
+__device__ __forceinline__ void ws_table_put(double* p, double v) {
+  if constexpr (WT) __hip_atomic_store(p, v, __ATOMIC_RELAXED, __HIP_MEMORY_SCOPE_AGENT);
+  else *p = v;
+}
+template <bool WT = false>
 __device__ __forceinline__ void ws_table_row_block(const double* mix, const MixLayout& ml, int j, int DP, int K4,
                                                    double* table, double* lds) {
   const int D = ml.D, K = ml.K, tid = threadIdx.x, TS = DP + 6;
@@ -26,7 +32,7 @@
       const int k = idx / DP, d = idx - k * DP;
       if (idx < K4 * DP) {
         const double v = (d < D && k < K) ? (vj[u] - vk[u]) : 0.0;
-        table[((size_t)j * K4 + k) * TS + d] = v;
+        ws_table_put<WT>(&table[((size_t)j * K4 + k) * TS + d], v);
         sV2[idx] = v * v;
       }
     }
@@ -41,14 +47,17 @@
       const double is2 = pre ? t_is2 : mix[ml.o_is2 + k];
       const double w = pre ? t_w : mix[ml.o_w + k];
       const double ak = -0.5 * 0x1.71547652b82fep+0 * is2;
-      row[DP + 0] = fma(ak, s, pre ? t_lrc : mix[ml.o_lrc + k]);
-      row[DP + 1] = ak;
-      row[DP + 2] = w;
-      row[DP + 3] = w * is2;
+      ws_table_put<WT>(row + DP + 0, fma(ak, s, pre ? t_lrc : mix[ml.o_lrc + k]));
+      ws_table_put<WT>(row + DP + 1, ak);
+      ws_table_put<WT>(row + DP + 2, w);
+      ws_table_put<WT>(row + DP + 3, w * is2);
     } else {
-      row[DP + 0] = -2000.0; row[DP + 1] = 0.0; row[DP + 2] = 0.0; row[DP + 3] = 0.0;
+      ws_table_put<WT>(row + DP + 0, -2000.0);
+      ws_table_put<WT>(row + DP + 1, 0.0);
+      ws_table_put<WT>(row + DP + 2, 0.0);
+      ws_table_put<WT>(row + DP + 3, 0.0);
     }
-    row[DP + 4] = 0.0;
-    row[DP + 5] = 0.0;
+    ws_table_put<WT>(row + DP + 4, 0.0);
+    ws_table_put<WT>(row + DP + 5, 0.0);
   }
 }
```

After: 11040 evals/s. 0.884x the previous value.
